# StephenNG59/ICP-symm

Hardware: AMD Instinct MI355X
Metric: icp_iterations_per_sec (higher is better)
Workload: dtype f32

## Files before the change

### icp-symm_amd/csrc/engine.cpp

```cpp
#include "engine_internal.h"
#include "robust_loss.h"
#include <limits>

void read_switches(Switches &w)
{
    auto flag = [](const char *n) { return std::getenv(n) != nullptr; };
    auto num = [](const char *n, long def) { const char *e = std::getenv(n); return e ? std::atol(e) : def; };
    auto tri = [](const char *n) { const char *e = std::getenv(n); return e ? (e[0] == '1' ? 1 : 0) : -1; };
    w.allow_any_arch = flag("SYMMICP_ALLOW_ANY_ARCH");
    w.debug_host = flag("SYMMICP_DEBUG_HOST");
    w.debug_counters = flag("SYMMICP_DEBUG_COUNTERS");
    if (const char *e = std::getenv("SYMMICP_DEBUG_TRACE")) w.debug_trace = e;
    if (const char *e = std::getenv("SYMMICP_GRID_PPC")) w.grid_ppc = std::atof(e);
    w.grid_maxlevel = (int)num("SYMMICP_GRID_MAXLEVEL", kMortonBits);
    w.grid_level = (int)num("SYMMICP_GRID_LEVEL", -1);
    if (const char *e = std::getenv("SYMMICP_FIRST_PASS")) w.first_pass = (e[0] == 'p') ? 1 : 0;
    w.oct_leaf = (int)num("SYMMICP_OCT_LEAF", 0);
    if (const char *e = std::getenv("SYMMICP_PACKET_ORDER")) w.packet_order = e[0] != '0';
    if (const char *e = std::getenv("SYMMICP_PACKET_JUMP")) w.packet_jump = (float)std::atof(e);
    w.packet_key_bits = (int)num("SYMMICP_PACKET_KEY_BITS", 16);
    w.packet_chunk = (uint32_t)num("SYMMICP_PACKET_CHUNK", 0);
    w.packet_lds_pad = (uint32_t)num("SYMMICP_PACKET_LDS_PAD", 0);
    w.packet_waves = (uint32_t)num("SYMMICP_PACKET_WAVES", 0);
    w.packet_front_cap = (uint32_t)num("SYMMICP_PACKET_FRONT_CAP", 0);
    if (const char *e = std::getenv("SYMMICP_HOOD_FRAC")) w.hood_frac = std::atof(e);
    w.no_hood = flag("SYMMICP_NO_NEIGHBOURHOOD");
    w.no_cert = flag("SYMMICP_NO_CERT");
    w.walk_full_grid = flag("SYMMICP_WALK_FULL_GRID");
    { const char *e = std::getenv("SYMMICP_HOST_LOOP"); w.host_loop = e && e[0] == '1'; }
    w.no_loop_stragglers = flag("SYMMICP_NO_LOOP_STRAGGLERS");
    w.force_comm = flag("SYMMICP_FORCE_COMM");
    if (const char *e = std::getenv("SYMMICP_PACKET_COST_KEY")) w.packet_cost_key = e[0] != '0';
    w.budget_walk = tri("SYMMICP_BUDGET_WALK");
    w.optimistic = tri("SYMMICP_OPTIMISTIC");
    w.compact = tri("SYMMICP_COMPACT");
    w.pass_blocks = (int)num("SYMMICP_PASS_BLOCKS", 2048);
    w.id_blocks = (int)num("SYMMICP_ID_BLOCKS", 2048);
    w.acc_blocks = (int)num("SYMMICP_ACC_BLOCKS", 512);
    w.fused_blocks = (int)num("SYMMICP_FUSED_BLOCKS", 512);
    w.compact_blocks = (int)num("SYMMICP_COMPACT_BLOCKS", 1280);
    w.feature_nn_splits = (int)num("SYMMICP_FEATURE_NN_SPLITS", 0);
    w.feature_nn_queries = (int)num("SYMMICP_FEATURE_NN_QUERIES", 0);
    w.tune.wave_mode_max = (uint32_t)num("SYMMICP_WAVE_MODE_MAX", 20000);
    w.tune.cells_chunk = (uint32_t)num("SYMMICP_CELLS_CHUNK", 16);
    w.tune.cells_queries = (uint32_t)num("SYMMICP_CELLS_QUERIES", 0);
    w.tune.walk_budget = (uint32_t)num("SYMMICP_WALK_BUDGET", 160);
}

void arena_begin(Arena &a, size_t want)
{
    a.off = 0;
    if (a.cap >= want) return;
    if (a.base) hipFree(a.base);
    a.base = nullptr; a.cap = 0;
    const size_t cap = want + want / 4;
    if (hipMalloc((void **)&a.base, cap) == hipSuccess) a.cap = cap;
    else (void)hipGetLastError();
}


extern "C" {

int symmicp_version(void) { return 100; }

void symmicp_config_default(symmicp_config *cfg)
{
    if (!cfg) return;
    std::memset(cfg, 0, sizeof(*cfg));
    cfg->struct_size = (int32_t)sizeof(*cfg);
    cfg->device = -1;
    cfg->mode = SYMMICP_MODE_QUIRKS;
    cfg->corr = SYMMICP_CORR_IDENTITY;
    cfg->apply = SYMMICP_APPLY_DEFAULT;
    cfg->max_iters = 10;
    cfg->diff_threshold = 1.0f;
    cfg->max_corr_dist = 0.f;
    cfg->fixed_iters = 0;
    cfg->sort_source = 1;
    cfg->verbose = 0;
    cfg->min_normal_dot = -2.0f;
    cfg->eps_rotation = 0.f;
    cfg->eps_translation = 0.f;
}

static int check_cfg(const symmicp_config *cfg)
{
    if (!cfg || cfg->struct_size != (int32_t)sizeof(symmicp_config)) return SYMMICP_ERR_ARG;
    if (!mode_known(cfg->mode)) return SYMMICP_ERR_ARG;
    if (cfg->corr < SYMMICP_CORR_IDENTITY || cfg->corr > SYMMICP_CORR_TREE) return SYMMICP_ERR_ARG;
    if (cfg->apply < SYMMICP_APPLY_DEFAULT || cfg->apply > SYMMICP_APPLY_CUMULATIVE) return SYMMICP_ERR_ARG;
    if (cfg->max_iters < 0) return SYMMICP_ERR_ARG;
    return SYMMICP_OK;
}

int symmicp_create(const symmicp_config *cfg, symmicp_ctx **out)
{
    if (!out) return SYMMICP_ERR_ARG;
    *out = nullptr;
    if (check_cfg(cfg) != SYMMICP_OK) return SYMMICP_ERR_ARG;
    int ndev = 0;
    if (hipGetDeviceCount(&ndev) != hipSuccess || ndev <= 0) return SYMMICP_ERR_HIP;
    symmicp_ctx *c = new symmicp_ctx();
    read_switches(c->sw);
    c->cfg = *cfg;
    if (cfg->device >= 0) {
        if (cfg->device >= ndev || hipSetDevice(cfg->device) != hipSuccess) { delete c; return SYMMICP_ERR_HIP; }
        c->device = cfg->device;
    } else if (hipGetDevice(&c->device) != hipSuccess) { delete c; return SYMMICP_ERR_HIP; }
    hipDeviceProp_t prop;
    if (hipGetDeviceProperties(&prop, c->device) != hipSuccess) { delete c; return SYMMICP_ERR_HIP; }
    if (std::strncmp(prop.gcnArchName, "gfx950", 6) != 0 && !c->sw.allow_any_arch) {
        delete c;
        return SYMMICP_ERR_HIP;
    }
    if (hipStreamCreateWithFlags(&c->stream, hipStreamNonBlocking) != hipSuccess) { delete c; return SYMMICP_ERR_HIP; }
    bool ok = hipMalloc((void **)&c->partials, sizeof(double) * kNSum * 8192) == hipSuccess &&
              hipMalloc((void **)&c->d_sums, sizeof(double) * kNSum) == hipSuccess &&
              hipHostMalloc((void **)&c->h_sums, sizeof(double) * (kNSum + 8), hipHostMallocMapped | hipHostMallocCoherent) == hipSuccess &&
              hipMalloc((void **)&c->ticket, 2 * sizeof(uint32_t)) == hipSuccess && hipMemset(c->ticket, 0, 2 * sizeof(uint32_t)) == hipSuccess &&
              hipHostGetDevicePointer((void **)&c->h_sums_dev, c->h_sums, 0) == hipSuccess &&
              std::memset(c->h_sums, 0, sizeof(double) * (kNSum + 8)) != nullptr &&
              hipMalloc((void **)&c->d_loop, sizeof(LoopState)) == hipSuccess &&
              hipHostMalloc((void **)&c->h_loop, sizeof(LoopState), hipHostMallocMapped | hipHostMallocCoherent) == hipSuccess &&
              hipHostGetDevicePointer((void **)&c->h_loop_dev, c->h_loop, 0) == hipSuccess &&
              hipHostMalloc((void **)&c->h_ring, sizeof(LoopRecord) * symmicp_ctx::kRing, hipHostMallocMapped | hipHostMallocCoherent) == hipSuccess &&
              hipHostGetDevicePointer((void **)&c->h_ring_dev, c->h_ring, 0) == hipSuccess &&
              hipHostMalloc((void **)&c->h_done, 64, hipHostMallocMapped | hipHostMallocCoherent) == hipSuccess &&
              hipHostGetDevicePointer((void **)&c->h_done_dev, c->h_done, 0) == hipSuccess &&
              std::memset(c->h_done, 0, 64) != nullptr &&
              true;
    for (int k = 0; ok && k < symmicp_ctx::kEvRing * symmicp_ctx::kEvPer; k++) ok = hipEventCreateWithFlags(&c->ev[k], hipEventDisableSystemFence) == hipSuccess;
    if (!ok) { symmicp_destroy(c); return SYMMICP_ERR_HIP; }
    c->pkt_fallbacks = c->ticket + 1;
    identity16(c->X);
    *out = c;
    return SYMMICP_OK;
}

extern "C++" hipError_t keep_alloc(symmicp_ctx *c, void **out, size_t bytes)
{
    bytes = (bytes + 255) & ~(size_t)255;
    if (!bytes) bytes = 256;
    if (c->keep.base && c->keep.off + bytes <= c->keep.cap) { *out = c->keep.base + c->keep.off; c->keep.off += bytes; return hipSuccess; }
    void *p = nullptr;
    const hipError_t e = hipMalloc(&p, bytes);
    if (e == hipSuccess) { c->keep_extra.push_back(p); *out = p; }
    return e;
}

extern "C++" void free_target(symmicp_ctx *c)
{
    for (void *p : c->keep_extra) hipFree(p);
    c->keep_extra.clear();
    c->keep.off = 0;
    hipFree(c->dbg); hipFree(c->dbg_trace); c->dbg_trace = nullptr;
    c->ctop = nullptr; c->dbg = nullptr; c->ix = TargetIndex{}; c->tgt_block = nullptr; c->tq = nullptr; c->tn = nullptr; c->boxes = nullptr; c->cells = nullptr; c->onodes = nullptr;
    c->have_index = false; c->n_t = 0;
    c->have_tgt_color = false;
    c->notes = IndexNotes{};
}

extern "C++" void forget_source(symmicp_ctx *c)
{
    c->worklist = c->wl_count = nullptr; c->cert = nullptr; c->certk = nullptr; c->hoodr = nullptr; c->pkt_tab = nullptr; c->pkt_count = 0; c->pkt_cost_keyed = false; c->pairrec = nullptr;
    c->src0_block = c->cur_block = nullptr; c->src_order = nullptr; c->pos = nullptr; c->d2 = nullptr; c->best64 = nullptr;
    c->n_loc = c->n_s_total = c->src_off = 0;
    c->src_no_normals = false;
    c->have_src_int = false;
    drop_reverse_index(c->rej.src_ix, false);
}

static void free_source(symmicp_ctx *c)
{
    forget_source(c);
    hipFree(c->src_all);
    c->src_all = nullptr; c->src_all_cap = 0;
}

void symmicp_destroy(symmicp_ctx *c)
{
    if (!c) return;
    if (c->sw.debug_host && c->n_pass_timed)
        std::fprintf(stderr, "[symmicp host] passes %ld: launch %.1f us, spin %.1f us, between passes %.1f us (per pass)\n", c->n_pass_timed, 1e6 * c->t_launch / c->n_pass_timed, 1e6 * c->t_spin / c->n_pass_timed, 1e6 * c->t_between / c->n_pass_timed);
    hipSetDevice(c->device);
    if (c->stream) hipStreamSynchronize(c->stream);
    if (c->comm && g_rccl.CommDestroy) g_rccl.CommDestroy(c->comm);
    shm_close(c);
    free_target(c);
// ... 1494 lines not shown
```

### icp-symm_amd/csrc/engine_internal.h

```cpp
#pragma once
#include <hip/hip_runtime.h>
#include <dlfcn.h>
#include <fcntl.h>
#include <sys/mman.h>
#include <sys/stat.h>
#include <unistd.h>
#include <algorithm>
#include <chrono>
#include <cmath>
#include <cstdio>
#include <cstdlib>
#include <cstring>
#include <mutex>
#include <string>
#include <vector>

#include "symmicp.h"
#include "symmicp_internal.h"
#include "host_solve.h"


namespace symmicp {}
using namespace symmicp;

typedef struct { char internal[128]; } rcclUniqueId;
typedef void *rcclComm_t;
typedef int (*fn_ncclGetUniqueId)(rcclUniqueId *);
typedef int (*fn_ncclCommInitRank)(rcclComm_t *, int, rcclUniqueId, int);
typedef int (*fn_ncclCommDestroy)(rcclComm_t);
typedef int (*fn_ncclAllReduce)(const void *, void *, size_t, int, int, rcclComm_t, hipStream_t);
typedef const char *(*fn_ncclGetErrorString)(int);
constexpr int kNcclFloat64 = 8;
constexpr int kNcclSum = 0;

struct Rccl {
    void *handle = nullptr;
    fn_ncclGetUniqueId GetUniqueId = nullptr;
    fn_ncclCommInitRank CommInitRank = nullptr;
    fn_ncclCommDestroy CommDestroy = nullptr;
    fn_ncclAllReduce AllReduce = nullptr;
    fn_ncclGetErrorString GetErrorString = nullptr;
    std::string err;
    std::mutex mu;
    bool load()
    {
        std::lock_guard<std::mutex> lock(mu);
        if (handle && AllReduce) return true;
        const char *names[] = {"librccl.so.1", "librccl.so"};
        for (const char *nm : names) { handle = dlopen(nm, RTLD_NOW | RTLD_NOLOAD | RTLD_GLOBAL); if (handle) break; }
        if (!handle)
            for (const char *nm : names) { handle = dlopen(nm, RTLD_NOW | RTLD_GLOBAL); if (handle) break; }
        if (!handle) { err = std::string("cannot load librccl: ") + dlerror(); return false; }
        GetUniqueId = (fn_ncclGetUniqueId)dlsym(handle, "ncclGetUniqueId");
        CommInitRank = (fn_ncclCommInitRank)dlsym(handle, "ncclCommInitRank");
        CommDestroy = (fn_ncclCommDestroy)dlsym(handle, "ncclCommDestroy");
        AllReduce = (fn_ncclAllReduce)dlsym(handle, "ncclAllReduce");
        GetErrorString = (fn_ncclGetErrorString)dlsym(handle, "ncclGetErrorString");
        if (!GetUniqueId || !CommInitRank || !CommDestroy || !AllReduce) { err = "librccl misses nccl* symbols"; return false; }
        return true;
    }
};
extern Rccl g_rccl;

inline double now_s()
{
    return std::chrono::duration<double>(std::chrono::steady_clock::now().time_since_epoch()).count();
}

struct Switches {
    bool allow_any_arch = false, debug_host = false, debug_counters = false;
    std::string debug_trace;
    double grid_ppc = 3.0;
    int grid_maxlevel = kMortonBits, grid_level = -1;
    int first_pass = -1;
    int oct_leaf = 0;
    bool packet_order = true;
    bool packet_cost_key = true;
    float packet_jump = -1.0f;
    int packet_key_bits = 16;
    uint32_t packet_chunk = 0, packet_lds_pad = 0, packet_waves = 0, packet_front_cap = 0;
    double hood_frac = 0.8;
    bool no_hood = false, no_cert = false, walk_full_grid = false, host_loop = false, no_loop_stragglers = false, force_comm = false;
    int budget_walk = -1, optimistic = -1, compact = -1;
    int pass_blocks = 2048, id_blocks = 2048, acc_blocks = 512, fused_blocks = 512, compact_blocks = 1280;
    int feature_nn_splits = 0, feature_nn_queries = 0;
    PassTuning tune;
};

void read_switches(Switches &w);

struct Arena {
    char *base = nullptr;
    size_t cap = 0, off = 0;
};

struct ShmSlot {
    volatile unsigned long long seq;
    double s[SYMMICP_NSUM];
    char pad[512 - 8 - 8 * SYMMICP_NSUM];
};
static_assert(sizeof(ShmSlot) == 512, "slot = 4 cache lines");
struct ShmExchange {
    ShmSlot *slots = nullptr;
    size_t bytes = 0;
    unsigned long long count = 0;
    std::string name;
    bool owner = false;
};

struct IndexNotes {
    float origin[3] = {0, 0, 0}, h0 = 0.f;
    uint32_t hist[16] = {};
    uint32_t leaf_max = 0;
    uint32_t nblocks = 0, ctop_len = 0;
};

struct ReverseIndex {
    Arena keep;
    std::vector<void *> extra;
    TargetIndex ix{};
    bool valid = false;
};

struct Rejectors {
    float trim_frac = 1.0f, med_factor = 0.0f;
    bool one_to_one = false, reciprocal = false;
    uint32_t *keys = nullptr, *ws = nullptr;
    unsigned long long *table = nullptr;
    size_t keys_cap = 0, table_cap = 0;
    ReverseIndex src_ix;
    uint64_t src_ix_builds = 0;
    RecipArgs recip_args{};
    enum : uint32_t { kTrim = 1, kMedian = 2, kOneToOne = 4, kReciprocal = 8 };
    uint32_t ran = 0;
    RejectRecord last{};
    void invalidate() { ran = 0; }

    bool trims() const { return trim_frac < 1.0f; }
    bool median() const { return med_factor > 0.0f; }
    bool claims(int corr) const { return (one_to_one || reciprocal) && corr != SYMMICP_CORR_IDENTITY; }
    bool checks_back(int corr) const { return reciprocal && corr != SYMMICP_CORR_IDENTITY; }
    bool rejects(int corr) const { return trims() || median() || claims(corr); }
    uint32_t settings_mask(int corr) const
    {
        if (!rejects(corr)) return 0u;
        return (trims() ? kTrim : 0u) | (median() ? kMedian : 0u) | (one_to_one ? kOneToOne : 0u) | (checks_back(corr) ? kReciprocal : 0u);
    }
    bool keys_valid() const { return ran != 0u; }
    bool trim_state_valid() const { return (ran & kTrim) != 0u; }
    bool rejection_state_valid() const { return (ran & (kMedian | kOneToOne | kReciprocal)) != 0u; }
    bool reciprocal_state_valid() const { return (ran & kReciprocal) != 0u; }
    static size_t table_words(size_t n_t, bool with_recip_tail) { return (n_t ? n_t : 1) + (with_recip_tail ? kRecipTailWords : 0); }
};

struct symmicp_ctx {
    Switches sw;
    Arena arena;
    Arena keep;
    std::vector<void *> keep_extra;
    ShmExchange shm;
    symmicp_config cfg{};
    int loss = SYMMICP_LOSS_NONE;
    float loss_scale = 0.f;
    float gicp_eps = 1e-3f;
    float color_lam = 0.968f;
    float4 *tgt_color = nullptr;
    float *src_int = nullptr;
    size_t tgt_color_cap = 0, src_int_cap = 0;
    bool have_tgt_color = false, have_src_int = false;
    Rejectors rej;
    int device = 0;
    hipStream_t stream = nullptr;
    std::string err;
    int nranks = 1, rank = 0;
    rcclComm_t comm = nullptr;
    bool external_exchange = false;
    bool sums_exchanged = false;
    uint32_t n_t = 0;
    float *tgt_block = nullptr;
    CloudSoA tgt{};
    float4 *tq = nullptr, *tn = nullptr;
    float4 *boxes = nullptr;
    float4 *onodes = nullptr;
    uint2 *cells = nullptr;
    uint32_t *ctop = nullptr;
    unsigned long long *dbg = nullptr;
    unsigned long long *dbg_trace = nullptr;
    TargetIndex ix{};
    bool have_index = false;
    bool target_surface_like = false;
    IndexNotes notes;
    float pivot[3] = {0, 0, 0};
    uint32_t n_s_total = 0, n_loc = 0, src_off = 0;
    bool src_no_normals = false;
    char *src_all = nullptr;
    size_t src_all_cap = 0;
    float *src0_block = nullptr, *cur_block = nullptr;
    CloudSoA src0{}, cur{};
    uint32_t *src_order = nullptr;
    int32_t *pos = nullptr;
    float *d2 = nullptr;
    float4 *pairrec = nullptr;
    float *cert = nullptr;
    uint32_t *certk = nullptr;
    float *hoodr = nullptr;
    uint32_t *pkt_tab = nullptr;
    uint32_t pkt_count = 0;
    bool pkt_cost_keyed = false;
    uint32_t *pkt_fallbacks = nullptr;
    unsigned long long *best64 = nullptr;
    uint32_t *worklist = nullptr, *wl_count = nullptr;
    WorkLists wl{};
    int pass_blocks = 0;
    double *partials = nullptr, *d_sums = nullptr, *h_sums = nullptr, *h_sums_dev = nullptr;
    uint32_t *ticket = nullptr;
    long long last_list_len = -1;
    long long last_uncertified = -1;
    static constexpr int kRing = 65;
    LoopState *d_loop = nullptr, *h_loop = nullptr, *h_loop_dev = nullptr;
    LoopRecord *h_ring = nullptr, *h_ring_dev = nullptr;
    unsigned long long *h_done = nullptr, *h_done_dev = nullptr;
    unsigned long long batch_seq = 0;
    bool loop_log_on = false;
    std::vector<symmicp_loop_log_entry> loop_log;
    int loop_log_batches = 0;
    int host_passes_since_bailout = 1000;
    unsigned long long seq = 0;
    bool begun = false;
    int iters = 0;
    float X[16];
    symmicp_sums last{};
    int timing = 0;
    static constexpr int kEvRing = 64, kEvPer = 8;
    hipEvent_t ev[kEvRing * kEvPer] = {};
    int ev_split[kEvRing] = {};
    int ev_weight[kEvRing] = {};
    int ev_coll[kEvRing] = {};
    int ev_used = 0;
    symmicp_stats st{};
    double t_launch = 0, t_spin = 0, t_between = 0, t_last_done = 0;
    long n_pass_timed = 0;
};

template <typename T>
struct DevBuf {
    T *p = nullptr;
    bool owned = true;
    DevBuf() = default;
    DevBuf(const DevBuf &) = delete;
    DevBuf &operator=(const DevBuf &) = delete;
    ~DevBuf() { if (p && owned) hipFree(p); }
    hipError_t alloc(size_t count) { owned = true; return hipMalloc((void **)&p, sizeof(T) * (count ? count : 1)); }
    hipError_t alloc_temp(Arena &a, size_t count)
    {
        const size_t bytes = ((sizeof(T) * (count ? count : 1)) + 255) & ~(size_t)255;
        if (a.base && a.off + bytes <= a.cap) { p = reinterpret_cast<T *>(a.base + a.off); a.off += bytes; owned = false; return hipSuccess; }
        return alloc(count);
    }
    T *release() { T *q = p; p = nullptr; return q; }
};

template <typename T>
inline hipError_t grow(T *&p, size_t &cap, size_t want)
{
    if (cap >= want) return hipSuccess;
    hipFree(p);
    p = nullptr; cap = 0;
    const hipError_t e = hipMalloc((void **)&p, sizeof(T) * want);
    if (e == hipSuccess) cap = want;
    return e;
}

hipError_t keep_alloc(symmicp_ctx *c, void **out, size_t bytes);
void arena_begin(Arena &a, size_t want);

#define HIP_TRY(ctx, call)                                                                                  \
    do {                                                                                                    \
        hipError_t e__ = (call);                                                                            \
        if (e__ != hipSuccess) {                                                                            \
            (ctx)->err = std::string(#call) + ": " + hipGetErrorString(e__);                                \
            return SYMMICP_ERR_HIP;                                                                         \
        }                                                                                                   \
    } while (0)



inline int fail(symmicp_ctx *c, int code, const std::string &msg)
{
    if (c) c->err = msg;
    return code;
}

inline void soa_from_block(float *block, size_t n, CloudSoA &s)
{
    s.x = block; s.y = block + n; s.z = block + 2 * n; s.nx = block + 3 * n; s.ny = block + 4 * n; s.nz = block + 5 * n;
}

inline void identity16(float X[16])
{
    for (int k = 0; k < 16; k++) X[k] = (k % 5 == 0) ? 1.f : 0.f;
}

inline bool pass_claims(const symmicp_ctx *c) { return c->rej.claims(c->cfg.corr); }
inline bool pass_reciprocal(const symmicp_ctx *c) { return c->rej.checks_back(c->cfg.corr); }
inline bool pass_rejects(const symmicp_ctx *c) { return c->rej.rejects(c->cfg.corr); }

inline int resolved_apply(const symmicp_config &c)
{
    if (c.apply == SYMMICP_APPLY_INCREMENTAL || c.apply == SYMMICP_APPLY_CUMULATIVE) return c.apply;
    return c.mode == SYMMICP_MODE_QUIRKS ? SYMMICP_APPLY_INCREMENTAL : SYMMICP_APPLY_CUMULATIVE;
}


void free_target(symmicp_ctx *c);
void forget_source(symmicp_ctx *c);
void flush_events(symmicp_ctx *c);
int build_reverse_index(symmicp_ctx *c, const CloudSoA &cl, uint32_t n, const uint32_t *labels, ReverseIndex &ri);
void drop_reverse_index(ReverseIndex &ri, bool release);
void shm_close(symmicp_ctx *c);
int shm_exchange(symmicp_ctx *c, double *rec);
void dump_packet_trace(symmicp_ctx *c);
void print_pass_counters(symmicp_ctx *c, bool first, long long list_len);
```

### icp-symm_amd/csrc/engine_loop.cpp

```cpp
#include "engine_internal.h"

extern "C" {

static int prepare_rejectors(symmicp_ctx *c, RejectArgs &r)
{
    Rejectors &j = c->rej;
    r = RejectArgs{};
    if (!pass_rejects(c)) return SYMMICP_OK;
    HIP_TRY(c, grow(j.keys, j.keys_cap, c->n_loc ? c->n_loc : 1));
    if (!j.ws) HIP_TRY(c, hipMalloc((void **)&j.ws, sizeof(uint32_t) * kRejectWsWords));
    r.keys = j.keys; r.ws = j.ws;
    r.host = reinterpret_cast<RejectRecord *>(c->h_sums_dev + kNSum + 1);
    r.rho = j.trim_frac; r.med_f2 = j.median() ? j.med_factor * j.med_factor : 0.0f;
    if (!pass_claims(c)) return SYMMICP_OK;
    HIP_TRY(c, grow(j.table, j.table_cap, Rejectors::table_words(c->n_t, pass_reciprocal(c))));
    r.table = j.table; r.n_t = c->n_t; r.order = c->src_order;
    r.claim = kClaimOneToOne;
    if (!pass_reciprocal(c)) return SYMMICP_OK;
    if (!j.src_ix.valid) {
        const double t0 = now_s();
        if (int st = build_reverse_index(c, c->src0, c->n_loc, c->src_order, j.src_ix)) return st;
        j.src_ix_builds++;
        if (c->sw.debug_host) {
            std::fprintf(stderr, "[symmicp host] source index: %u points, %zu bytes in its arena (+%zu allocations beside it), built in %.3f ms\n", c->n_loc,
// ... 19 lines not shown
        __builtin_ia32_pause();
        if ((++spins & 0xFFFu) == 0) {
            if (hipStreamQuery(c->stream) != hipErrorNotReady) { got = (*flag == seq); break; }
            if (now_s() - t0 > limit_seconds) break;
        }
    }
    __atomic_thread_fence(__ATOMIC_ACQUIRE);
    if (spun) *spun += now_s() - t0;
    if (!got) {
        HIP_TRY(c, hipStreamSynchronize(c->stream));
        HIP_TRY(c, hipGetLastError());
        if (*flag != seq) return fail(c, SYMMICP_ERR_HIP, what);
    }
    return SYMMICP_OK;
}

static void fill_pass_args(symmicp_ctx *c, PassArgs &a, const RejectArgs &rej, const float Xapply[16], bool from_cur, bool writeback, bool first)
{
    a.in = from_cur ? c->cur : c->src0;
    a.out = c->cur;
    a.n = c->n_loc;
    a.tgt_offset = c->src_off;
    for (int k = 0; k < 12; k++) a.X.m[k] = Xapply[k];
    a.X.nrm_w = (c->cfg.mode == SYMMICP_MODE_QUIRKS) ? 1.0f : 0.0f;
    const bool paper = c->cfg.mode != SYMMICP_MODE_QUIRKS;
    for (int k = 0; k < 3; k++) a.pivot[k] = paper ? c->pivot[k] : 0.0f;
    a.p2p = c->cfg.mode == SYMMICP_MODE_P2P ? 1 : 0;
    a.obj = mode_obj(c->cfg.mode);
    a.gicp_k = 1.0f - c->gicp_eps;
    a.tgt_color = c->tgt_color;
    a.src_int = c->src_int;
    a.color_lam = c->color_lam;
    a.color_om = 1.0f - c->color_lam;
    a.max_d2 = c->cfg.max_corr_dist > 0.f ? c->cfg.max_corr_dist * c->cfg.max_corr_dist : 0.f;
    a.min_ndot = c->cfg.min_normal_dot;
    a.writeback = writeback ? 1 : 0;
    a.best64 = c->best64;
    a.pos_prev = first ? nullptr : c->pos;
    a.pos_out = c->pos;
    a.d2_out = (c->cfg.corr == SYMMICP_CORR_IDENTITY) ? nullptr : c->d2;
    a.partials = c->partials;
    a.cert = reinterpret_cast<float4 *>(c->cert);
    a.certk = c->sw.no_hood ? nullptr : reinterpret_cast<uint4 *>(c->certk);
    a.hoodr = reinterpret_cast<float2 *>(c->hoodr);
    a.make_hood = (a.certk && !first && c->last_uncertified >= 0 && (double)c->last_uncertified < c->sw.hood_frac * (double)c->n_s_total) ? 1 : 0;
    a.pairrec = c->pairrec;
    a.budget_walk = c->sw.budget_walk >= 0 ? c->sw.budget_walk : (first && c->nranks > 1 && c->n_loc < 400000u);
    a.use_slack = (!first && c->cert && !c->sw.no_cert) ? 1 : 0;
    a.loop = nullptr;
    a.pkt_tab = reinterpret_cast<const uint2 *>(c->pkt_tab);
    a.pkt_count = c->pkt_count;
    a.pkt_waves = c->sw.packet_waves;
    a.pkt_front_cap = c->sw.packet_front_cap;
    a.pkt_fallbacks = c->pkt_fallbacks;
    a.pkt_chunk = c->sw.packet_chunk;
    a.pkt_lds_pad = c->sw.packet_lds_pad;
    a.loss = c->loss;
    a.loss_scale = c->loss_scale;
    a.rej = rej;
}

static int run_pass(symmicp_ctx *c, const float Xapply[16], bool from_cur, bool writeback, bool first)
{
    PassArgs a{};
    RejectArgs rej;
    if (int st = prepare_rejectors(c, rej)) return st;
    c->rej.invalidate();
    fill_pass_args(c, a, rej, Xapply, from_cur, writeback, first);
    const bool rejecting = pass_rejects(a);
    int blocks = (int)((c->n_loc + kPassThreads - 1) / kPassThreads);
    int cap = c->sw.pass_blocks;
    if (cap > 8192) cap = 8192;
    if (blocks > cap) blocks = cap;
    if (blocks < 1) blocks = 1;
    c->pass_blocks = blocks;
    const double t_l0 = now_s();
    if (c->t_last_done > 0) c->t_between += t_l0 - c->t_last_done;
    hipEvent_t *ev = nullptr;
    uint32_t walk_blocks = 0;
    bool optimistic = false;
    if (c->timing) {
        if (c->ev_used == symmicp_ctx::kEvRing) flush_events(c);
        ev = c->ev + c->ev_used * symmicp_ctx::kEvPer;
        c->ev_split[c->ev_used] = (c->timing == 1 || c->timing == 3) ? 1 : 0;
        c->ev_weight[c->ev_used] = 1;
    }
    if (ev && !(c->timing == 2 && c->cfg.corr == SYMMICP_CORR_TREE)) hipEventRecord(ev[0], c->stream);
    switch (c->cfg.corr) {
    case SYMMICP_CORR_IDENTITY: {
        const bool vec4 = (c->n_loc % 4 == 0) && (c->n_t % 4 == 0) && (c->src_off % 4 == 0);
        if (vec4) {
            const int id_cap = c->sw.id_blocks;
            const int nb4 = (int)((c->n_loc / 4 + kPassThreads - 1) / kPassThreads);
            blocks = nb4 < id_cap ? (nb4 > 0 ? nb4 : 1) : id_cap;
            c->pass_blocks = blocks;
        }
        launch_pass_identity(a, c->tgt, blocks, vec4, c->stream);
        break;
    }
    case SYMMICP_CORR_BRUTE:
        launch_nn_brute(a.in, c->n_loc, a.X, c->tq, c->n_t, c->best64, c->stream);
        launch_pass_indexed(a, c->tn, blocks, c->stream);
        break;
    default:
        {
            const int acc_cap = c->sw.acc_blocks;
            const int nb_all = (int)((c->n_loc + kPassThreads - 1) / kPassThreads);
            int ab = nb_all < acc_cap ? ((nb_all + 7) / 8) * 8 : acc_cap;
            if (ab < 8) ab = 8;
            c->pass_blocks = blocks = ab;
            if (!first && c->last_list_len >= 0 && c->last_list_len <= 50000) {
                walk_blocks = (uint32_t)(2 * c->last_list_len);
                if (walk_blocks < 256u) walk_blocks = 256u;
                if (walk_blocks > 8192u) walk_blocks = 8192u;
            }
            if (!first && c->last_list_len == -2) walk_blocks = 16384u;
            if (c->sw.walk_full_grid) walk_blocks = 0;
            optimistic = c->sw.optimistic >= 0 ? c->sw.optimistic == 1 : (!first && c->last_list_len == 0);
            if (writeback) optimistic = false;
            if (rejecting) optimistic = false;
            if (first && c->target_surface_like) launch_pass_tree_first(a, c->ix, c->wl, ab, c->stream, c->timing == 2 ? ev : nullptr);
            else
            {
                const int cp_blocks = c->sw.compact_blocks;
                const bool compact = a.use_slack && (c->sw.compact >= 0 ? c->sw.compact == 1 : (c->last_uncertified >= 0 && c->last_uncertified < (long long)(c->n_s_total / 10)));
                launch_pass_tree_split(a, c->ix, c->wl, ab, walk_blocks, optimistic ? 1 : 0, compact ? cp_blocks : 0, c->sw.tune, c->stream, c->timing == 2 ? ev : nullptr);
            }
            if (ev && c->timing == 2) c->ev_split[c->ev_used] = 2;
        }
        break;
    }
    if (ev && c->ev_split[c->ev_used] != 2) hipEventRecord(ev[4], c->stream);
    c->t_launch += now_s() - t_l0;
    auto reduce_and_wait = [&](int keep_nonempty) -> int {
        const unsigned long long seq = ++c->seq;
        volatile unsigned long long *flag = reinterpret_cast<volatile unsigned long long *>(c->h_sums + kNSum);
        launch_final_reduce(c->partials, blocks, c->d_sums, c->comm ? nullptr : c->h_sums_dev, c->ticket, seq,
                            c->cfg.corr == SYMMICP_CORR_TREE ? c->wl_count : nullptr, keep_nonempty, c->stream);
        if (c->comm) {
            if (ev) { hipEventRecord(ev[6], c->stream); c->ev_coll[c->ev_used] = 1; }
            int r = g_rccl.AllReduce(c->d_sums, c->d_sums, kNSum, kNcclFloat64, kNcclSum, c->comm, c->stream);
            if (r != 0) return fail(c, SYMMICP_ERR_COMM, std::string("ncclAllReduce: ") + (g_rccl.GetErrorString ? g_rccl.GetErrorString(r) : "?"));
            if (ev) hipEventRecord(ev[7], c->stream);
            launch_publish(c->d_sums, c->h_sums_dev, seq, c->stream);
        }
        if (ev && c->ev_split[c->ev_used] != 1) hipEventRecord(ev[5], c->stream);
        return wait_for_word(c, flag, seq, 30.0, "pass finished without publishing its record", &c->t_spin);
    };
    if (int st = reduce_and_wait(optimistic ? 1 : 0)) return st;
    if (c->shm.slots) { if (int st = shm_exchange(c, c->h_sums)) return st; }
    if (c->cfg.corr == SYMMICP_CORR_TREE && c->h_sums[kNSum - 1] >= kListDropped)
        return fail(c, SYMMICP_ERR_HIP, "a work-list shard overflowed: appends were dropped (internal capacity error)");
    long long list_len = (c->cfg.corr == SYMMICP_CORR_TREE) ? (long long)c->h_sums[kNSum - 1] : -1;
    c->last_uncertified = (c->cfg.corr == SYMMICP_CORR_TREE && !first) ? (long long)c->h_sums[kNSum - 2] : -1;
    if (optimistic && list_len > 0) {
        c->st.kernel_launches[7]++;
        launch_pass_tree_split(a, c->ix, c->wl, blocks, list_len <= 50000 ? 8192u : 0u, 2, 0, c->sw.tune, c->stream, nullptr);
        if (ev && c->ev_split[c->ev_used] != 2) hipEventRecord(ev[4], c->stream);
        if (int st = reduce_and_wait(0)) return st;
        if (c->shm.slots) { if (int st = shm_exchange(c, c->h_sums)) return st; }
    }
    if (rejecting) {
        std::memcpy(&c->rej.last, c->h_sums + kNSum + 1, sizeof(RejectRecord));
        c->rej.ran = c->rej.settings_mask(c->cfg.corr);
    }
    if (ev) c->ev_used++;
    c->t_last_done = now_s(); c->n_pass_timed++;
    if (c->dbg_trace && first) dump_packet_trace(c);
    if (c->ix.dbg) print_pass_counters(c, first, list_len);
    std::memcpy(c->last.s, c->h_sums, sizeof(double) * kNSum);
    if (c->cfg.corr == SYMMICP_CORR_TREE) c->last.s[kNSum - 1] = c->last.s[kNSum - 2] = 0.0;
    c->last_list_len = list_len;
    if (first && c->cfg.corr == SYMMICP_CORR_TREE && c->target_surface_like) c->last_list_len = -2;
    c->st.passes++;
    return SYMMICP_OK;
}

static constexpr uint32_t kLoopListLimit = 8192;
static uint32_t loop_scan_limit(uint32_t n) { const uint32_t f = n / 256; return f < 8192u ? f : 8192u; }
static bool batch_eligible(const symmicp_ctx *c)
{
    if (c->sw.host_loop) return false;
    if (pass_rejects(c)) return false;
    if (c->cfg.mode == SYMMICP_MODE_COLOR) return false;
    if (c->cfg.host_loop) return false;
    if (c->external_exchange || c->shm.slots) return false;
    if (c->timing == 2 || c->ix.dbg) return false;
    if (!mode_device_solves(c->cfg.mode)) return false;
    if (c->n_loc == 0 && !c->comm) return false;
    if (c->host_passes_since_bailout < 2) return false;
    const bool incr = resolved_apply(c->cfg) == SYMMICP_APPLY_INCREMENTAL;
    if (c->cfg.corr == SYMMICP_CORR_IDENTITY) return true;
    if (c->cfg.corr == SYMMICP_CORR_TREE)
        return !incr && c->last_list_len >= 0 && c->last_list_len <= (c->sw.no_loop_stragglers ? 0ll : (long long)kLoopListLimit) && c->last_uncertified >= 0 &&
               c->last_uncertified <= (long long)(loop_scan_limit(c->n_s_total) / (c->last_list_len > 0 ? 2 : 1)) && c->cert && !c->sw.no_cert;
    return false;
}

static constexpr int kListBlocks = 8;
static constexpr int kEvSampleStride = 4;
static int run_batch(symmicp_ctx *c, int want, float *diffs_before, int *n_done, bool *small_step)
{
    *n_done = 0;
    *small_step = false;
    if (want > symmicp_ctx::kRing - 1) want = symmicp_ctx::kRing - 1;
    if (want <= 0) return SYMMICP_OK;
    const bool incr = resolved_apply(c->cfg) == SYMMICP_APPLY_INCREMENTAL;
    const bool tree = c->cfg.corr == SYMMICP_CORR_TREE;
    LoopConfig lc{};
    lc.mode = c->cfg.mode; lc.fixed_iters = c->cfg.fixed_iters; lc.max_iters = c->iters + want; lc.incremental = incr ? 1 : 0; lc.tree = tree ? 1 : 0;
    lc.diff_threshold = c->cfg.diff_threshold; lc.eps_rotation = c->cfg.eps_rotation; lc.eps_translation = c->cfg.eps_translation;
    lc.nrm_w = (c->cfg.mode == SYMMICP_MODE_QUIRKS) ? 1.0f : 0.0f;
    for (int k = 0; k < 3; k++) lc.pivot[k] = c->pivot[k];
    lc.uncertified_limit = 4 * loop_scan_limit(c->n_s_total);
    const bool no_stage = c->sw.no_loop_stragglers;
    bool stragglers = tree && c->last_list_len > 0 && !no_stage;
    lc.list_limit = kLoopListLimit;
    if (lc.max_iters > c->cfg.max_iters) lc.max_iters = c->cfg.max_iters;
    const int it0 = c->iters;
    LoopState ls{};
    std::memcpy(ls.X, c->X, sizeof(ls.X));
    for (int k = 0; k < 12; k++) ls.Xapply.m[k] = c->X[k];
    ls.Xapply.nrm_w = lc.nrm_w;
    ls.iters = it0;
    *c->h_loop = ls;
    symmicp_sums last0{};
    if (c->loop_log_on) {
        last0 = c->last;
        c->h_ring[it0 % symmicp_ctx::kRing].solved = 0;
    }
    HIP_TRY(c, hipMemcpyAsync(c->d_loop, c->h_loop, sizeof(LoopState), hipMemcpyHostToDevice, c->stream));
    PassArgs a{};
    fill_pass_args(c, a, RejectArgs{}, c->X, incr, incr, false);
    a.loop = c->d_loop;
    int blocks;
    bool vec4 = false;
    if (tree) {
        const int fb = c->sw.fused_blocks;
        const int tiles = (int)((c->n_loc + kPassThreads - 1) / kPassThreads);
        blocks = tiles < fb ? tiles : fb;
        if (blocks < 1) blocks = 1;
    } else {
        vec4 = (c->n_loc % 4 == 0) && (c->n_t % 4 == 0) && (c->src_off % 4 == 0);
        const int id_cap = c->sw.id_blocks;
        const int nb = (int)(((vec4 ? c->n_loc / 4 : c->n_loc) + kPassThreads - 1) / kPassThreads);
        blocks = nb < id_cap ? (nb > 0 ? nb : 1) : id_cap;
    }
    const int fused_blocks_full = blocks;
    c->pass_blocks = blocks;
    uint32_t *counters = tree ? c->wl_count : nullptr;
    const bool timed_run = c->timing == 1 || c->timing == 3;
    const int ev_stride = c->timing == 3 ? kEvSampleStride : 1;
    if (timed_run && c->ev_used + want > symmicp_ctx::kEvRing) flush_events(c);
    const bool unstoppable = lc.fixed_iters && !(lc.eps_rotation > 0.f && lc.eps_translation > 0.f) && !stragglers;
    int enq = 0, chunk = unstoppable ? want : 4, n_stage = 0;
    bool first_chunk = true;
    while (enq < want) {
        const int nq = (want - enq < chunk) ? want - enq : chunk;
        const int it_before = first_chunk ? it0 : c->h_loop->iters;
        const int ev_used0 = c->ev_used;
        const int fused_blocks = (stragglers && fused_blocks_full + kListBlocks > 512) ? 512 - kListBlocks : fused_blocks_full;
        blocks = fused_blocks + (stragglers ? kListBlocks : 0);
        a.partial_cols = stragglers ? (uint32_t)blocks : 0u;
        a.partial_col0 = (uint32_t)fused_blocks;
        lc.walk_in_loop = stragglers ? 1 : 0;
        if (first_chunk) launch_reduce_solve(c->partials, blocks, c->d_sums, 2, c->d_loop, lc, c->h_ring_dev, symmicp_ctx::kRing, counters, c->stream);
        for (int p = 0; p < nq; p++) {
            hipEvent_t *ev = nullptr;
            if (timed_run && (enq + p) % ev_stride == 0 && c->ev_used < symmicp_ctx::kEvRing) {
                ev = c->ev + c->ev_used * symmicp_ctx::kEvPer;
                c->ev_split[c->ev_used] = 1;
                c->ev_weight[c->ev_used] = 1;
                hipEventRecord(ev[0], c->stream);
            }
            if (tree) {
                launch_pass_fused(a, c->ix, c->wl, fused_blocks, c->stream);
                if (stragglers) launch_loop_stragglers(a, c->ix, c->wl, kListBlocks, c->sw.tune, c->stream);
            }
            else launch_pass_identity(a, c->tgt, blocks, vec4, c->stream);
            if (ev) { hipEventRecord(ev[4], c->stream); c->ev_used++; }
            if (c->comm || blocks > 512) {
                launch_final_reduce(c->partials, blocks, c->d_sums, nullptr, c->ticket, 0ull, counters, 0, c->stream);
                if (c->comm) {
                    if (ev) { hipEventRecord(ev[6], c->stream); c->ev_coll[c->ev_used - 1] = 1; }
                    int r = g_rccl.AllReduce(c->d_sums, c->d_sums, kNSum, kNcclFloat64, kNcclSum, c->comm, c->stream);
                    if (r != 0) {
                        (void)hipStreamSynchronize(c->stream);
                        c->begun = false;
                        c->ev_used = 0;
                        return fail(c, SYMMICP_ERR_COMM, std::string("ncclAllReduce: ") + (g_rccl.GetErrorString ? g_rccl.GetErrorString(r) : "?"));
                    }
                    if (ev) hipEventRecord(ev[7], c->stream);
                }
                launch_reduce_solve(c->partials, blocks, c->d_sums, 1, c->d_loop, lc, c->h_ring_dev, symmicp_ctx::kRing, counters, c->stream);
            } else {
                launch_reduce_solve(c->partials, blocks, c->d_sums, 0, c->d_loop, lc, c->h_ring_dev, symmicp_ctx::kRing, counters, c->stream);
            }
        }
        const unsigned long long seq = ++c->batch_seq;
        launch_loop_end(c->d_loop, c->h_loop_dev, c->h_done_dev, seq, c->stream);
        if (int st = wait_for_word(c, c->h_done, seq, 60.0, "batch finished without publishing its end flag")) return st;
        enq += nq;
        first_chunk = false;
        const int ran = (c->h_loop->iters - it_before) + (c->h_loop->reason == LOOP_REDO_PASS ? 1 : 0);
        if (timed_run && ran >= 0) {
            int sampled_ran = 0;
            for (int p = 0; p < ran && p < nq; p++) {
                if ((enq - nq + p) % ev_stride != 0) continue;
                if (ev_used0 + sampled_ran < symmicp_ctx::kEvRing) {
                    const int left = (ran < nq ? ran : nq) - p;
                    c->ev_weight[ev_used0 + sampled_ran] = left < ev_stride ? left : ev_stride;
                }
                sampled_ran++;
            }
            if (ev_used0 + sampled_ran < c->ev_used) c->ev_used = ev_used0 + sampled_ran;
        }
        if (stragglers) n_stage += c->h_loop->iters - it_before;
        if (c->h_loop->stop) break;
        if (tree && !no_stage) {
            stragglers = false;
            for (int k = it_before + 1; k <= c->h_loop->iters; k++) stragglers = stragglers || c->h_ring[k % symmicp_ctx::kRing].list_len > 0;
        }
        if (stragglers) chunk = 4;
        else if (lc.fixed_iters && !(lc.eps_rotation > 0.f && lc.eps_translation > 0.f)) chunk = want;
        else chunk *= 2;
    }
    const LoopState &hl = *c->h_loop;
    const int it1 = hl.iters;
    if (it1 < it0 || it1 > it0 + want) return fail(c, SYMMICP_ERR_HIP, "device loop state out of range");
    for (int k = it0; k < it1; k++) diffs_before[k - it0] = (k == it0) ? (float)c->last.s[33] : (float)c->h_ring[k % symmicp_ctx::kRing].sums[33];
    if (it1 > it0) {
        std::memcpy(c->last.s, c->h_ring[it1 % symmicp_ctx::kRing].sums, sizeof(double) * kNSum);
        std::memcpy(c->X, c->h_ring[(it1 - 1) % symmicp_ctx::kRing].X, sizeof(float) * 16);
        c->st.passes += it1 - it0;
        c->st.loop_passes += it1 - it0;
        c->st.loop_straggler_passes += n_stage;
    }
    if (c->loop_log_on) {
        for (int k = it0; k <= it1; k++) {
            const LoopRecord &r = c->h_ring[k % symmicp_ctx::kRing];
            symmicp_loop_log_entry e{};
            std::memcpy(e.sums, k == it0 ? last0.s : r.sums, sizeof(e.sums));
            std::memcpy(e.increment, r.increment, sizeof(e.increment));
            std::memcpy(e.X, r.X, sizeof(e.X));
            e.rcond = r.rcond; e.iter = k; e.status = r.status; e.solved = r.solved; e.list_len = k == it0 ? 0 : r.list_len;
            e.reason = hl.reason; e.batch = c->loop_log_batches;
            if (!e.solved) { std::memset(e.increment, 0, sizeof(e.increment)); std::memset(e.X, 0, sizeof(e.X)); e.rcond = 0.f; e.status = -1; }
            c->loop_log.push_back(e);
        }
        c->loop_log_batches++;
    }
    c->iters = it1;
    c->last_list_len = tree ? (it1 > it0 ? (long long)c->h_ring[it1 % symmicp_ctx::kRing].list_len : c->last_list_len) : -1;
    *n_done = it1 - it0;
    *small_step = hl.reason == LOOP_DONE && hl.small_step != 0;
    if (tree && it1 > it0) c->last_uncertified = c->h_ring[it1 % symmicp_ctx::kRing].pad;
    if (c->sw.debug_host && it1 - it0 >= 2) {
        const double *q = c->h_ring[(it1 - 1) % symmicp_ctx::kRing].sums;
        if (q[37] != 0.0) std::fprintf(stderr, "[symmicp host] k_reduce_solve stamps of pass %d: load + reduce %.2f us (loop state there after %.2f us), bookkeeping + solve %.2f us, publish %.2f us\n", it1 - 1, std::floor(q[37]) * 0.01, (q[37] - std::floor(q[37])) * 1e4 * 0.01, q[38] * 0.01, q[39] * 0.01);
    }
    if (c->sw.debug_host && tree) {
        std::fprintf(stderr, "[symmicp host] batch: work list / searched pairs after each device pass:");
        for (int k = it0 + 1; k <= it1; k++) std::fprintf(stderr, " %d/%d", c->h_ring[k % symmicp_ctx::kRing].list_len, c->h_ring[k % symmicp_ctx::kRing].pad);
        std::fprintf(stderr, "\n");
    }
    if (c->sw.debug_host) std::fprintf(stderr, "[symmicp host] batch: %d of %d passes on the device (%d enqueued), reason %d, %d with the straggler stage, list after %lld\n", it1 - it0, want, enq, hl.reason, n_stage, (long long)c->last_list_len);
    if (hl.reason == LOOP_SLOW) c->host_passes_since_bailout = 1;
    if (hl.reason == LOOP_REDO_PASS || hl.reason == LOOP_HOST_SOLVE) {
        c->host_passes_since_bailout = 0;
        c->last_list_len = -1;
        c->st.kernel_launches[7]++;
    }
    return SYMMICP_OK;
}

static int check_ready(symmicp_ctx *c)
{
    if (!c->tgt_block || !c->src0_block) return fail(c, SYMMICP_ERR_STATE, "source and target must be set first (myicp.cpp:102)");
    if (c->cfg.corr == SYMMICP_CORR_IDENTITY && c->n_s_total != c->n_t)
        return fail(c, SYMMICP_ERR_SIZE, "identity pairing needs N_s == N_t (func.cpp:21)");
    if (c->cfg.corr == SYMMICP_CORR_TREE && !c->have_index) return fail(c, SYMMICP_ERR_STATE, "target index missing");
    if (c->cfg.corr != SYMMICP_CORR_IDENTITY && !c->tq) return fail(c, SYMMICP_ERR_STATE, "target was set under a different corr mode");
    if (c->cfg.mode == SYMMICP_MODE_COLOR) {
        if (c->nranks > 1) return fail(c, SYMMICP_ERR_STATE, "SYMMICP_MODE_COLOR runs on single-rank contexts only");
        if (!c->have_src_int || !c->have_tgt_color)
            return fail(c, SYMMICP_ERR_STATE, "SYMMICP_MODE_COLOR needs symmicp_set_source_intensity and symmicp_set_target_intensity after the clouds");
    }
    return SYMMICP_OK;
}

static void fill_iter(symmicp_ctx *c, symmicp_iter_result *out, int status, float rcond, const float *incr)
{
    if (!out) return;
    out->status = status;
    out->iter = c->iters;
    out->diff = (float)c->last.s[33];
    out->rcond = rcond;
    out->pairs = c->last.s[c->loss != SYMMICP_LOSS_NONE ? 37 : 34];
    if (incr) std::memcpy(out->increment, incr, sizeof(float) * 16); else identity16(out->increment);
    out->sums = c->last;
}

int symmicp_begin(symmicp_ctx *c, const float *guess16, symmicp_iter_result *out)
{
    if (!c) return SYMMICP_ERR_ARG;
    HIP_TRY(c, hipSetDevice(c->device));
    int st = check_ready(c);
    if (st != SYMMICP_OK) return st;
    if (guess16) std::memcpy(c->X, guess16, sizeof(float) * 16); else identity16(c->X);
    c->iters = 0;
    const bool incr = resolved_apply(c->cfg) == SYMMICP_APPLY_INCREMENTAL;
    st = run_pass(c, c->X, false, incr, true);
    if (st != SYMMICP_OK) return st;
    c->begun = true;
    c->sums_exchanged = false;
    fill_iter(c, out, SYMMICP_OK, 1.0f, nullptr);
    return SYMMICP_OK;
}

int symmicp_step(symmicp_ctx *c, symmicp_iter_result *out)
{
    if (!c) return SYMMICP_ERR_ARG;
    if (!c->begun) return fail(c, SYMMICP_ERR_STATE, "symmicp_step before symmicp_begin");
    if (c->external_exchange && !c->sums_exchanged)
        return fail(c, SYMMICP_ERR_STATE, "external exchange: symmicp_set_sums(total over ranks) must follow every pass");
    c->sums_exchanged = false;
    HIP_TRY(c, hipSetDevice(c->device));
    float pbar[3], qbar[3], a[3], t[3], rc = 0.f, Xi[16];
    int st = (c->cfg.mode == SYMMICP_MODE_P2P) ? solve_p2p(c->last, c->pivot, &rc, Xi) : solve_mode(mode_solves_as(c->cfg.mode), c->last, c->pivot, pbar, qbar, a, t, &rc, Xi);
    if (st != SYMMICP_OK) {
        c->err = "degenerate system (rank-deficient normal equations or non-finite transform; func.cpp:70,96)";
        fill_iter(c, out, st, rc, nullptr);
        return st;
    }
    mat4_mul(Xi, c->X, c->X);
    const bool incr = resolved_apply(c->cfg) == SYMMICP_APPLY_INCREMENTAL;
    st = incr ? run_pass(c, Xi, true, true, false) : run_pass(c, c->X, false, false, false);
    if (st != SYMMICP_OK) return st;
    c->iters++;
    fill_iter(c, out, SYMMICP_OK, rc, Xi);
    return SYMMICP_OK;
}

static size_t append_eigen(std::string &out, const float *m, int rows, int cols, int stride)
{
    char cell[16][32];
    size_t width = 0;
    for (int r = 0; r < rows; r++)
        for (int c = 0; c < cols; c++) {
            std::snprintf(cell[r * cols + c], sizeof(cell[0]), "%g", (double)m[r * stride + c]);
            width = std::max(width, std::strlen(cell[r * cols + c]));
        }
    for (int r = 0; r < rows; r++) {
        for (int c = 0; c < cols; c++) {
            if (c) out += ' ';
            const size_t len = std::strlen(cell[r * cols + c]);
            out.append(width - len, ' ');
            out += cell[r * cols + c];
        }
        out += '\n';
    }
    return width;
}

static void polar_rotation(const float X[16], float R[9])
{
    double A[3][3];
    for (int r = 0; r < 3; r++) for (int c = 0; c < 3; c++) A[r][c] = X[4 * r + c];
    for (int it = 0; it < 100; it++) {
        const double det = A[0][0] * (A[1][1] * A[2][2] - A[1][2] * A[2][1]) - A[0][1] * (A[1][0] * A[2][2] - A[1][2] * A[2][0]) + A[0][2] * (A[1][0] * A[2][1] - A[1][1] * A[2][0]);
        if (!(std::fabs(det) > 1e-300) || !std::isfinite(det)) break;
        double inv_t[3][3];
        inv_t[0][0] = (A[1][1] * A[2][2] - A[1][2] * A[2][1]) / det; inv_t[0][1] = (A[1][2] * A[2][0] - A[1][0] * A[2][2]) / det; inv_t[0][2] = (A[1][0] * A[2][1] - A[1][1] * A[2][0]) / det;
        inv_t[1][0] = (A[0][2] * A[2][1] - A[0][1] * A[2][2]) / det; inv_t[1][1] = (A[0][0] * A[2][2] - A[0][2] * A[2][0]) / det; inv_t[1][2] = (A[0][1] * A[2][0] - A[0][0] * A[2][1]) / det;
        inv_t[2][0] = (A[0][1] * A[1][2] - A[0][2] * A[1][1]) / det; inv_t[2][1] = (A[0][2] * A[1][0] - A[0][0] * A[1][2]) / det; inv_t[2][2] = (A[0][0] * A[1][1] - A[0][1] * A[1][0]) / det;
        double change = 0.0;
        for (int r = 0; r < 3; r++)
            for (int c = 0; c < 3; c++) { const double v = 0.5 * (A[r][c] + inv_t[r][c]); change = std::max(change, std::fabs(v - A[r][c])); A[r][c] = v; }
        if (change < 1e-15) break;
    }
    for (int r = 0; r < 3; r++) for (int c = 0; c < 3; c++) R[3 * r + c] = std::isfinite(A[r][c]) ? (float)A[r][c] : X[4 * r + c];
}

size_t symmicp_format_result(const float transform16[16], char *buf, size_t cap)
{
    if (!transform16) return 0;
    std::string out = "Result transform:\n";
    append_eigen(out, transform16, 4, 4, 4);
    out += "  rotation:\n";
    float R[9];
    polar_rotation(transform16, R);
    append_eigen(out, R, 3, 3, 3);
    out += "  translation:\n";
    append_eigen(out, transform16 + 3, 3, 1, 4);
    if (buf && cap) {
        const size_t n = std::min(out.size(), cap - 1);
        std::memcpy(buf, out.data(), n);
        buf[n] = 0;
    }
    return out.size();
}

int symmicp_align(symmicp_ctx *c, const float *guess16, symmicp_result *out)
{
    if (!c || !out) return SYMMICP_ERR_ARG;
    std::memset(out, 0, sizeof(*out));
    if (c->external_exchange) { out->status = SYMMICP_ERR_STATE; return fail(c, SYMMICP_ERR_STATE, "symmicp_align is not available with external exchange: drive begin/set_sums/step"); }
    const double t0 = now_s();
    c->loop_log.clear();
    c->loop_log_batches = 0;
    symmicp_iter_result it;
    int st = symmicp_begin(c, guess16, &it);
    if (st != SYMMICP_OK) { out->status = st; return st; }
    float diff = it.diff;
    out->diff_initial = diff;
    int iters = 0;
    while ((c->cfg.fixed_iters || diff > c->cfg.diff_threshold) && iters < c->cfg.max_iters) {
        if (batch_eligible(c)) {
            float db[symmicp_ctx::kRing];
            int done = 0;
            bool small = false;
            st = run_batch(c, c->cfg.max_iters - iters, db, &done, &small);
            if (st != SYMMICP_OK) break;
            for (int k = 0; k < done; k++) {
                iters++;
                if (c->cfg.verbose) std::printf("iters#%d\ndiff: %g\n", iters, db[k]);
                if (iters <= 64) out->diffs[iters - 1] = db[k];
            }
            diff = (float)c->last.s[33];
            if (small) break;
            if (done > 0 || c->host_passes_since_bailout == 0) continue;
        }
        iters++;
        if (c->cfg.verbose) std::printf("iters#%d\ndiff: %g\n", iters, diff);
        if (iters <= 64) out->diffs[iters - 1] = diff;
        st = symmicp_step(c, &it);
        if (st != SYMMICP_OK) { iters--; break; }
        c->host_passes_since_bailout++;
        diff = it.diff;
        if (c->cfg.eps_rotation > 0.f && c->cfg.eps_translation > 0.f && !c->cfg.fixed_iters) {
            const float *Xi = it.increment;
            const double tr = ((double)Xi[0] + Xi[5] + Xi[10] - 1.0) * 0.5;
            const double ang = std::acos(tr > 1.0 ? 1.0 : (tr < -1.0 ? -1.0 : tr));
            const double tn = std::sqrt((double)Xi[3] * Xi[3] + (double)Xi[7] * Xi[7] + (double)Xi[11] * Xi[11]);
            if (ang < c->cfg.eps_rotation && tn < c->cfg.eps_translation) break;
        }
    }
    out->status = st;
    out->iters = iters;
    out->diff_final = diff;
    std::memcpy(out->transform, c->X, sizeof(float) * 16);
    out->seconds_total = now_s() - t0;
    if (c->cfg.verbose) {
        char buf[1024];
        symmicp_format_result(c->X, buf, sizeof(buf));
        std::fputs(buf, stdout);
    }
    return st;
}

int symmicp_solve(int mode, const symmicp_sums *sums, const float pivot[3], float pbar[3], float qbar[3], float a[3],
                  float t[3], float *rcond, float out16[16])
{
    if (!sums || !pbar || !qbar || !a || !t || !out16) return SYMMICP_ERR_ARG;
    if (mode == SYMMICP_MODE_P2P) {
        for (int k = 0; k < 3; k++) pbar[k] = qbar[k] = a[k] = t[k] = 0.f;
        return solve_p2p(*sums, pivot, rcond, out16);
    }
    mode = mode_solves_as(mode);
    return mode_device_solves(mode) ? solve_mode(mode, *sums, pivot, pbar, qbar, a, t, rcond, out16) : SYMMICP_ERR_ARG;
}

int symmicp_ctx_solve_probe(symmicp_ctx *c, int mode, int exact_rc, const symmicp_sums *sums, size_t n, const float pivot[3], const float *X_in16,
                            int32_t *status, float *pbar, float *qbar, float *a, float *t, float *rcond, float *out16, float *X_out16)
{
    if (!c) return SYMMICP_ERR_ARG;
    if (!mode_device_solves(mode)) return fail(c, SYMMICP_ERR_ARG, "probe: QUIRKS, PAPER, PLANE or GICP");
    if (!sums || n == 0 || n > (1u << 24) || !status || !pbar || !qbar || !a || !t || !rcond || !out16 || (X_in16 && !X_out16))
        return fail(c, SYMMICP_ERR_ARG, "probe: bad arguments");
    HIP_TRY(c, hipSetDevice(c->device));
    const size_t b_sums = sizeof(symmicp_sums) * n, b_f3 = sizeof(float) * 3 * n, b_16 = sizeof(float) * 16 * n;
    const size_t o_piv = b_sums, o_xin = o_piv + 16, o_st = o_xin + b_16, o_pb = o_st + 4 * n, o_qb = o_pb + b_f3, o_a = o_qb + b_f3, o_t = o_a + b_f3,
                 o_rc = o_t + b_f3, o_out = o_rc + 4 * n, o_xo = o_out + b_16, total = o_xo + b_16;
    char *d = nullptr;
    HIP_TRY(c, hipMalloc((void **)&d, total));
    float piv[4] = {0.f, 0.f, 0.f, 0.f};
    if (pivot) for (int k = 0; k < 3; k++) piv[k] = pivot[k];
    int st = SYMMICP_OK;
    if (hipMemcpy(d, sums, b_sums, hipMemcpyHostToDevice) != hipSuccess || hipMemcpy(d + o_piv, piv, 16, hipMemcpyHostToDevice) != hipSuccess ||
        (X_in16 && hipMemcpy(d + o_xin, X_in16, b_16, hipMemcpyHostToDevice) != hipSuccess))
        st = fail(c, SYMMICP_ERR_HIP, "probe: upload");
    if (st == SYMMICP_OK) {
        launch_solve_probe(mode, exact_rc, (const symmicp_sums *)d, (int)n, (const float *)(d + o_piv), X_in16 ? (const float *)(d + o_xin) : nullptr,
                           (int32_t *)(d + o_st), (float *)(d + o_pb), (float *)(d + o_qb), (float *)(d + o_a), (float *)(d + o_t), (float *)(d + o_rc),
                           (float *)(d + o_out), (float *)(d + o_xo), c->stream);
        if (hipGetLastError() != hipSuccess || hipStreamSynchronize(c->stream) != hipSuccess) st = fail(c, SYMMICP_ERR_HIP, "probe: kernel");
    }
    if (st == SYMMICP_OK) {
        const struct { size_t off, bytes; void *dst; } back[] = {{o_st, 4 * n, status}, {o_pb, b_f3, pbar}, {o_qb, b_f3, qbar}, {o_a, b_f3, a}, {o_t, b_f3, t},
                                                              {o_rc, 4 * n, rcond}, {o_out, b_16, out16}, {o_xo, X_in16 ? b_16 : 0, X_out16}};
        for (const auto &b : back)
            if (b.bytes && hipMemcpy(b.dst, d + b.off, b.bytes, hipMemcpyDeviceToHost) != hipSuccess) { st = fail(c, SYMMICP_ERR_HIP, "probe: read back"); break; }
    }
    (void)hipFree(d);
    return st;
}

int symmicp_ctx_loop_solve(symmicp_ctx *c, const symmicp_sums *sums, const float pivot[3], const float X_in16[16], const int32_t in_i[6], const float in_f[3],
                           int32_t state_out[4], float X_out16[16], float Xapply_out12[12], float ring_inc16[16], float ring_X16[16], float *ring_rcond,
                           int32_t ring_i2[2])
{
    if (!c) return SYMMICP_ERR_ARG;
    if (!sums || !X_in16 || !in_i || !in_f || !state_out || !X_out16 || !Xapply_out12 || !ring_inc16 || !ring_X16 || !ring_rcond || !ring_i2)
        return fail(c, SYMMICP_ERR_ARG, "loop_solve: bad arguments");
    const int mode = in_i[0];
    if (!mode_device_solves(mode)) return fail(c, SYMMICP_ERR_ARG, "loop_solve: QUIRKS, PAPER, PLANE or GICP");
    HIP_TRY(c, hipSetDevice(c->device));
    LoopConfig lc{};
    lc.mode = mode; lc.fixed_iters = in_i[1]; lc.max_iters = in_i[2]; lc.incremental = in_i[5] ? 1 : 0; lc.tree = 0;
    lc.diff_threshold = in_f[0]; lc.eps_rotation = in_f[1]; lc.eps_translation = in_f[2];
    lc.nrm_w = (mode == SYMMICP_MODE_QUIRKS) ? 1.0f : 0.0f;
    for (int k = 0; k < 3; k++) lc.pivot[k] = pivot ? pivot[k] : 0.f;
    LoopState ls{};
    std::memcpy(ls.X, X_in16, sizeof(ls.X));
    for (int k = 0; k < 12; k++) ls.Xapply.m[k] = X_in16[k];
    ls.Xapply.nrm_w = lc.nrm_w;
    ls.iters = in_i[3];
    ls.small_step = in_i[4];
    char *d = nullptr;
    const size_t o_loop = 512, o_ring = o_loop + ((sizeof(LoopState) + 255) & ~(size_t)255), total = o_ring + sizeof(LoopRecord);
    HIP_TRY(c, hipMalloc((void **)&d, total));
    int st = SYMMICP_OK;
    if (hipMemcpy(d, sums, sizeof(symmicp_sums), hipMemcpyHostToDevice) != hipSuccess || hipMemcpy(d + o_loop, &ls, sizeof(ls), hipMemcpyHostToDevice) != hipSuccess ||
        hipMemset(d + o_ring, 0xFF, sizeof(LoopRecord)) != hipSuccess)
        st = fail(c, SYMMICP_ERR_HIP, "loop_solve: upload");
    if (st == SYMMICP_OK) {
        launch_reduce_solve(nullptr, 0, (double *)d, 2, (LoopState *)(d + o_loop), lc, (LoopRecord *)(d + o_ring), 1, nullptr, c->stream);
        if (hipGetLastError() != hipSuccess || hipStreamSynchronize(c->stream) != hipSuccess) st = fail(c, SYMMICP_ERR_HIP, "loop_solve: kernel");
    }
    LoopState lo{};
    LoopRecord r{};
    if (st == SYMMICP_OK && (hipMemcpy(&lo, d + o_loop, sizeof(lo), hipMemcpyDeviceToHost) != hipSuccess ||
                             hipMemcpy(&r, d + o_ring, sizeof(r), hipMemcpyDeviceToHost) != hipSuccess))
        st = fail(c, SYMMICP_ERR_HIP, "loop_solve: read back");
    (void)hipFree(d);
    if (st != SYMMICP_OK) return st;
    state_out[0] = lo.stop; state_out[1] = lo.reason; state_out[2] = lo.iters; state_out[3] = lo.small_step;
    std::memcpy(X_out16, lo.X, sizeof(lo.X));
    std::memcpy(Xapply_out12, lo.Xapply.m, sizeof(lo.Xapply.m));
    std::memcpy(ring_inc16, r.increment, sizeof(r.increment));
    std::memcpy(ring_X16, r.X, sizeof(r.X));
    std::memcpy(ring_rcond, &r.rcond, sizeof(float));
    ring_i2[0] = r.status; ring_i2[1] = r.solved;
    return SYMMICP_OK;
}

int symmicp_set_loop_log(symmicp_ctx *c, int on)
{
    if (!c) return SYMMICP_ERR_ARG;
    c->loop_log_on = on != 0;
    if (!c->loop_log_on) { c->loop_log.clear(); c->loop_log.shrink_to_fit(); }
// ... 13 lines not shown
```

### icp-symm_amd/csrc/kernels_pass.hip

```cpp
#include <cstdlib>
#include <type_traits>
#include "symmicp_internal.h"
#include "device_common.h"
#include "oct_walk.h"
#include "solve_core.h"
#include "robust_loss.h"
#include "pass_rows.h"
#pragma clang fp contract(off)

namespace symmicp {

template <int NA>
__device__ __forceinline__ void acc_block_reduce_store(AccN<NA> &a, double *partials, uint32_t col)
{
    __shared__ double red[(kPassThreads / 64) * kNSum];
    acc_wave_reduce(a, red + (threadIdx.x >> 6) * kNSum);
    __syncthreads();
    if (threadIdx.x < kNSum) {
        double s = 0.0;
        if (threadIdx.x < NA) {
#pragma unroll
            for (int w = 0; w < kPassThreads / 64; w++) s += red[w * kNSum + threadIdx.x];
        }
        partials[(size_t)col * kNSum + threadIdx.x] = s;
// ... 3 lines not shown
template <int VEC, bool W, int OBJ, bool T>
__global__ __launch_bounds__(kPassThreads) void k_pass_identity(PassArgs a_in, CloudSoA tgt)
{
    if (a_in.loop && a_in.loop->stop) return;
    PassArgs a = a_in;
    if (a_in.loop) a.X = a_in.loop->Xapply;
    AccT<W> acc; acc_zero(acc);
    const HotParams h = hot_params(a);
    const uint32_t tau = T ? a.rej.ws[kRejectTauWord] : 0u;
    const bool need_n = reads_src_normals<OBJ>(a.writeback, a.min_ndot);
    const uint32_t stride = gridDim.x * blockDim.x * VEC;
    for (uint32_t i0 = (blockIdx.x * blockDim.x + threadIdx.x) * VEC; i0 < a.n; i0 += stride) {
        float x[VEC], y[VEC], z[VEC], nx[VEC], ny[VEC], nz[VEC], qx[VEC], qy[VEC], qz[VEC], qnx[VEC], qny[VEC], qnz[VEC];
        const uint32_t j0 = a.tgt_offset + i0;
        if (VEC == 4) {
            *reinterpret_cast<float4 *>(x) = *reinterpret_cast<const float4 *>(a.in.x + i0);
            *reinterpret_cast<float4 *>(y) = *reinterpret_cast<const float4 *>(a.in.y + i0);
            *reinterpret_cast<float4 *>(z) = *reinterpret_cast<const float4 *>(a.in.z + i0);
            if (need_n) {
                *reinterpret_cast<float4 *>(nx) = *reinterpret_cast<const float4 *>(a.in.nx + i0);
                *reinterpret_cast<float4 *>(ny) = *reinterpret_cast<const float4 *>(a.in.ny + i0);
                *reinterpret_cast<float4 *>(nz) = *reinterpret_cast<const float4 *>(a.in.nz + i0);
            } else {
#pragma unroll
                for (int k = 0; k < VEC; k++) nx[k] = ny[k] = nz[k] = 0.0f;
            }
            *reinterpret_cast<float4 *>(qx) = *reinterpret_cast<const float4 *>(tgt.x + j0);
            *reinterpret_cast<float4 *>(qy) = *reinterpret_cast<const float4 *>(tgt.y + j0);
            *reinterpret_cast<float4 *>(qz) = *reinterpret_cast<const float4 *>(tgt.z + j0);
            *reinterpret_cast<float4 *>(qnx) = *reinterpret_cast<const float4 *>(tgt.nx + j0);
            *reinterpret_cast<float4 *>(qny) = *reinterpret_cast<const float4 *>(tgt.ny + j0);
            *reinterpret_cast<float4 *>(qnz) = *reinterpret_cast<const float4 *>(tgt.nz + j0);
        } else {
            x[0] = a.in.x[i0]; y[0] = a.in.y[i0]; z[0] = a.in.z[i0];
            if (need_n) { nx[0] = a.in.nx[i0]; ny[0] = a.in.ny[i0]; nz[0] = a.in.nz[i0]; }
            else nx[0] = ny[0] = nz[0] = 0.0f;
            qx[0] = tgt.x[j0]; qy[0] = tgt.y[j0]; qz[0] = tgt.z[j0];
            qnx[0] = tgt.nx[j0]; qny[0] = tgt.ny[j0]; qnz[0] = tgt.nz[j0];
        }
        float px[VEC], py[VEC], pz[VEC], npx[VEC], npy[VEC], npz[VEC], d2[VEC];
#pragma unroll
        for (int k = 0; k < VEC; k++) {
            px[k] = xf_row(a.X.m + 0, x[k], y[k], z[k], 1.0f); py[k] = xf_row(a.X.m + 4, x[k], y[k], z[k], 1.0f);
            pz[k] = xf_row(a.X.m + 8, x[k], y[k], z[k], 1.0f);
            npx[k] = xf_row(a.X.m + 0, nx[k], ny[k], nz[k], a.X.nrm_w); npy[k] = xf_row(a.X.m + 4, nx[k], ny[k], nz[k], a.X.nrm_w);
            npz[k] = xf_row(a.X.m + 8, nx[k], ny[k], nz[k], a.X.nrm_w);
            d2[k] = dist2(px[k], py[k], pz[k], qx[k], qy[k], qz[k]);
        }
        if (a.writeback) {
            if (VEC == 4) {
                *reinterpret_cast<float4 *>(a.out.x + i0) = *reinterpret_cast<float4 *>(px);
                *reinterpret_cast<float4 *>(a.out.y + i0) = *reinterpret_cast<float4 *>(py);
                *reinterpret_cast<float4 *>(a.out.z + i0) = *reinterpret_cast<float4 *>(pz);
                *reinterpret_cast<float4 *>(a.out.nx + i0) = *reinterpret_cast<float4 *>(npx);
                *reinterpret_cast<float4 *>(a.out.ny + i0) = *reinterpret_cast<float4 *>(npy);
                *reinterpret_cast<float4 *>(a.out.nz + i0) = *reinterpret_cast<float4 *>(npz);
            } else {
                a.out.x[i0] = px[0]; a.out.y[i0] = py[0]; a.out.z[i0] = pz[0];
                a.out.nx[i0] = npx[0]; a.out.ny[i0] = npy[0]; a.out.nz[i0] = npz[0];
            }
        }
        if (a.d2_out) {
            if (VEC == 4) *reinterpret_cast<float4 *>(a.d2_out + i0) = *reinterpret_cast<float4 *>(d2);
            else a.d2_out[i0] = d2[0];
        }
#pragma unroll
        for (int k = 0; k < VEC; k++) {
            if constexpr (OBJ == kObjColor) {
                const ColorPair cp = color_pair(a, i0 + k, j0 + k);
                pair_step<OBJ, T>(acc, h, nx[k], ny[k], nz[k], px[k], py[k], pz[k], make_float4(qx[k], qy[k], qz[k], 0.0f), make_float4(qnx[k], qny[k], qnz[k], 0.0f), d2[k], tau, &cp);
            } else
            pair_step<OBJ, T>(acc, h, nx[k], ny[k], nz[k], px[k], py[k], pz[k], make_float4(qx[k], qy[k], qz[k], 0.0f), make_float4(qnx[k], qny[k], qnz[k], 0.0f), d2[k], tau);
        }
    }
    acc_block_reduce_store(acc, a.partials, blockIdx.x);
}

template <bool W, int OBJ, bool T>
__global__ __launch_bounds__(kPassThreads) void k_pass_indexed(PassArgs a, const float4 *__restrict__ tn)
{
    AccT<W> acc; acc_zero(acc);
    const HotParams h = hot_params(a);
    const uint32_t tau = T ? a.rej.ws[kRejectTauWord] : 0u;
    const bool need_n = reads_src_normals<OBJ>(a.writeback, a.min_ndot);
    const uint32_t stride = gridDim.x * blockDim.x;
    for (uint32_t i = blockIdx.x * blockDim.x + threadIdx.x; i < a.n; i += stride) {
        float x = a.in.x[i], y = a.in.y[i], z = a.in.z[i];
        float nx = 0.0f, ny = 0.0f, nz = 0.0f;
        if (need_n) { nx = a.in.nx[i]; ny = a.in.ny[i]; nz = a.in.nz[i]; }
        float px = xf_row(a.X.m + 0, x, y, z, 1.0f), py = xf_row(a.X.m + 4, x, y, z, 1.0f), pz = xf_row(a.X.m + 8, x, y, z, 1.0f);
        if (a.writeback) {
            a.out.x[i] = px; a.out.y[i] = py; a.out.z[i] = pz;
            a.out.nx[i] = xf_row(a.X.m + 0, nx, ny, nz, a.X.nrm_w); a.out.ny[i] = xf_row(a.X.m + 4, nx, ny, nz, a.X.nrm_w);
            a.out.nz[i] = xf_row(a.X.m + 8, nx, ny, nz, a.X.nrm_w);
        }
        unsigned long long b = a.best64[i];
        uint32_t j = (uint32_t)(b & 0xFFFFFFFFull);
        float d2 = __uint_as_float((uint32_t)(b >> 32));
        bool ok = (b != ~0ull);
        if (a.pos_out) a.pos_out[i] = ok ? (int32_t)j : -1;
        if (a.d2_out) a.d2_out[i] = ok ? d2 : __int_as_float(0x7f800000);
        if (!ok) continue;
        if (a.max_d2 > 0.0f && d2 > a.max_d2) continue;
        if (T && a.rej.claim != kClaimNone && a.rej.keys[i] == 0xFFFFFFFFu) continue;
        if constexpr (OBJ == kObjColor) {
            const ColorPair cp = color_pair(a, i, j);
            pair_step<OBJ, T>(acc, h, nx, ny, nz, px, py, pz, tn[2 * (size_t)j], tn[2 * (size_t)j + 1], d2, tau, &cp);
        } else
        pair_step<OBJ, T>(acc, h, nx, ny, nz, px, py, pz, tn[2 * (size_t)j], tn[2 * (size_t)j + 1], d2, tau);
    }
    acc_block_reduce_store(acc, a.partials, blockIdx.x);
}

__device__ __forceinline__ uint2 cell_range(const TargetIndex &ix, uint32_t morton)
{
    const uint32_t blk = ix.ctop[morton >> 9];
    if (blk == 0xFFFFFFFFu) return make_uint2(0u, 0u);
    return ix.cells[(size_t)blk * 512u + (morton & 511u)];
}

__device__ __forceinline__ uint32_t spread3(uint32_t v)
{
    v &= 0x3ffu;
    v = (v | (v << 16)) & 0x030000ffu;
    v = (v | (v << 8)) & 0x0300f00fu;
    v = (v | (v << 4)) & 0x030c30c3u;
    v = (v | (v << 2)) & 0x09249249u;
    return v;
}

constexpr int kWaveFrontier = 512;

__device__ __forceinline__ float axis_gap2(float p, float origin, int c, float h, float margin)
{
    const float lo = origin + (float)c * h;
    const float g = fmaxf(fmaxf(lo - p, p - (lo + h)) - margin, 0.0f);
    return g * g;
}

#ifndef SLACK_FRAC
#define SLACK_FRAC 0.0625f
#endif
constexpr float kSlackFrac = SLACK_FRAC;
constexpr int kHoodSlots = 8;
constexpr uint32_t kHoodNone = 0xFFFFFFFFu;

__device__ __forceinline__ float cert_word(float L, bool hood)
{
    const uint32_t u = __float_as_uint(L);
    if (!(L > 0.0f)) return hood ? __uint_as_float(0xBF800001u) : 0.0f;
    return __uint_as_float(hood ? ((u - 1u) | 1u) : (u & ~1u));
}

__device__ __forceinline__ bool hood_test(const PassArgs &a, const TargetIndex &ix, uint32_t i, float px, float py, float pz, float m2,
                                          int32_t pos_a, float d2a, int32_t rowa, int32_t &pos_w, float &d2w)
{
    const uint4 w0 = a.certk[2 * (size_t)i], w1 = a.certk[2 * (size_t)i + 1];
    const float T = a.hoodr[i].x;
    const uint32_t cand[kHoodSlots] = {w0.x, w0.y, w0.z, w0.w, w1.x, w1.y, w1.z, w1.w};
    float4 q[kHoodSlots];
#pragma unroll
    for (int k = 0; k < kHoodSlots; k++) q[k] = ix.tq[min(cand[k], ix.n - 1u)];
    unsigned long long kw = ((unsigned long long)__float_as_uint(d2a) << 32) | (unsigned long long)(uint32_t)rowa;
    uint32_t sec = 0x7f800000u;
    pos_w = pos_a;
#pragma unroll
    for (int k = 0; k < kHoodSlots; k++) {
        const float d2 = dist2(px, py, pz, q[k].x, q[k].y, q[k].z);
        if (cand[k] < ix.n && cand[k] != (uint32_t)pos_a && d2 == d2) {
            const unsigned long long key = ((unsigned long long)__float_as_uint(d2) << 32) | (unsigned long long)(uint32_t)__float_as_int(q[k].w);
            if (key < kw) { sec = (uint32_t)(kw >> 32); kw = key; pos_w = (int32_t)cand[k]; }
            else sec = min(sec, __float_as_uint(d2));
        }
    }
    d2w = __uint_as_float((uint32_t)(kw >> 32));
    const float dl = __builtin_amdgcn_sqrtf(m2);
    if (!((__builtin_amdgcn_sqrtf(d2w) + dl) * 1.000002f < T)) return false;
    if (pos_w != pos_a) {
        a.pos_out[i] = pos_w;
        store_pair_record(a, ix, i, pos_w);
    }
    const float d1 = sqrtf(d2w) * 1.000001f;
    const float Tn = (T - dl * 1.000001f) * 0.999999f;
    const float L = fminf(sqrtf(__uint_as_float(sec)) * 0.999999f, Tn);
    if (Tn > d1 * 1.001f) {
        a.cert[i] = make_float4(px, py, pz, cert_word((L > d1) ? L : 0.0f, true));
        a.hoodr[i].x = Tn;
    } else if (pos_w != pos_a) {
        a.cert[i].w = cert_word(0.0f, true);
    }
    return true;
}

template <bool HOOD>
__device__ __forceinline__ void cells_tile(const PassArgs &a, const TargetIndex &ix, const WorkLists &wl, const Affine &X, const uint32_t i,
                                           const uint32_t shard, const bool from_list)
{
    __shared__ float s_px[kPassThreads], s_py[kPassThreads], s_pz[kPassThreads];
    __shared__ unsigned long long s_key[kPassThreads];
    __shared__ uint32_t s_second[kPassThreads];
    __shared__ int32_t s_pos[kPassThreads];
    __shared__ uint32_t s_cell0[kPassThreads];
    __shared__ __align__(8) uint16_t s_items[kPassThreads * 27];
    __shared__ uint32_t s_wsum[kPassThreads / 64 + 1];
    __shared__ uint32_t s_anyw[kPassThreads / 64];
    __shared__ uint32_t s_nmore;
    constexpr int kHoodLds = HOOD ? kPassThreads : 1;
    __shared__ float s_reach[kHoodLds];
    __shared__ uint32_t s_hcnt[kHoodLds];
    __shared__ uint32_t s_qi[kHoodLds];

    const int tid = threadIdx.x, lane = tid & 63, wave = tid >> 6;
    const bool active = i < a.n;
    const float inf = __int_as_float(0x7f800000);
    const uint32_t push_shard = from_list ? ((i / kPassThreads) & (uint32_t)(kShards - 1)) : shard;

    float px = 0.f, py = 0.f, pz = 0.f;
    Best b;
    b.d2 = inf; b.pos = -1; b.row = 0x7fffffff;
    uint32_t mask = 0;
    uint32_t mask_rest = 0;
    bool defer = false, searched = false, probe = false, uncert = false, hood_ok = false;
    float lim = 0.f, lim_full = 0.f;
    float reach = 0.f;
    if (active) {
        const float x = a.in.x[i], y = a.in.y[i], z = a.in.z[i];
        const int32_t prev = a.pos_prev ? a.pos_prev[i] : -1;
        float clear = 0.0f, rx = 0.0f, ry = 0.0f, rz = 0.0f;
        if (a.use_slack) { const float4 ce = a.cert[i]; rx = ce.x; ry = ce.y; rz = ce.z; clear = ce.w; }
        px = xf_row(X.m + 0, x, y, z, 1.0f); py = xf_row(X.m + 4, x, y, z, 1.0f); pz = xf_row(X.m + 8, x, y, z, 1.0f);
        if (prev >= 0 && (uint32_t)prev < ix.n) {
            const float4 q = ix.tq[prev];
            const float d2 = dist2(px, py, pz, q.x, q.y, q.z);
            const int32_t row = __float_as_int(q.w);
            if (d2 <= inf) { b.d2 = d2; b.pos = prev; b.row = row; }
        }
        bool certified = false;
        if (a.use_slack && b.pos >= 0 && !from_list) {
            const float m2 = dist2(px, py, pz, rx, ry, rz);
            certified = (__builtin_amdgcn_sqrtf(b.d2) + __builtin_amdgcn_sqrtf(m2)) * 1.000002f < clear;
            if (!certified && (__float_as_uint(clear) & 1u) && a.certk) {
                int32_t pw; float d2w;
                if (hood_test(a, ix, i, px, py, pz, m2, b.pos, b.d2, b.row, pw, d2w)) {
                    certified = hood_ok = true; b.pos = pw; b.d2 = d2w;
                }
            }
        }
        if (!certified) {
            uncert = true;
            defer = true;
            if (b.pos >= 0 && ix.glevel > 0) {
                const float margin = 2e-3f * ix.h;
                const float gmax = (float)ix.gdim;
                const float rb = __builtin_amdgcn_sqrtf(b.d2) * 1.00001f;
                lim = rb + kSlackFrac * ix.h;
                const float r = lim + margin;
                const float lx = (px - r - ix.ox) * ix.inv_h, hx = (px + r - ix.ox) * ix.inv_h;
                const float ly = (py - r - ix.oy) * ix.inv_h, hy = (py + r - ix.oy) * ix.inv_h;
                const float lz = (pz - r - ix.oz) * ix.inv_h, hz = (pz + r - ix.oz) * ix.inv_h;
                const int x0 = (int)floorf(fminf(fmaxf(lx, 0.0f), gmax - 1.0f)), x1 = (int)floorf(fminf(fmaxf(hx, 0.0f), gmax - 1.0f));
                const int y0 = (int)floorf(fminf(fmaxf(ly, 0.0f), gmax - 1.0f)), y1 = (int)floorf(fminf(fmaxf(hy, 0.0f), gmax - 1.0f));
                const int z0 = (int)floorf(fminf(fmaxf(lz, 0.0f), gmax - 1.0f)), z1 = (int)floorf(fminf(fmaxf(hz, 0.0f), gmax - 1.0f));
                const int nx = x1 - x0, ny = y1 - y0, nz = z1 - z0;
                if (nx <= 2 && ny <= 2 && nz <= 2) {
                    defer = false;
                    searched = true;
                    const float thr2 = lim * lim * 1.00001f;
                    float gx[3], gy[3], gz[3];
#pragma unroll
                    for (int k = 0; k < 3; k++) {
                        gx[k] = (k <= nx) ? axis_gap2(px, ix.ox, x0 + k, ix.h, margin) : inf;
                        gy[k] = (k <= ny) ? axis_gap2(py, ix.oy, y0 + k, ix.h, margin) : inf;
                        gz[k] = (k <= nz) ? axis_gap2(pz, ix.oz, z0 + k, ix.h, margin) : inf;
                    }
#pragma unroll
                    for (int kz = 0; kz < 3; kz++)
#pragma unroll
                        for (int ky = 0; ky < 3; ky++)
#pragma unroll
                            for (int kx = 0; kx < 3; kx++) {
                                const float g2 = (gx[kx] + gy[ky]) + gz[kz];
                                if (g2 <= thr2) mask |= 1u << (kx + 3 * ky + 9 * kz);
                            }
                    s_cell0[tid] = (uint32_t)x0 | ((uint32_t)y0 << 10) | ((uint32_t)z0 << 20);
                    reach = rb;
                }
            }
            if (defer && b.pos >= 0 && ix.glevel > 0) {
                const float fx = (px - ix.ox) * ix.inv_h, fy = (py - ix.oy) * ix.inv_h, fz = (pz - ix.oz) * ix.inv_h;
                const float gmax = (float)ix.gdim;
                if (fx >= 0.0f && fy >= 0.0f && fz >= 0.0f && fx < gmax && fy < gmax && fz < gmax) {
                    const int cx = (int)fx, cy = (int)fy, cz = (int)fz;
                    const int x0 = max(cx - 1, 0), y0 = max(cy - 1, 0), z0 = max(cz - 1, 0);
                    const int x1 = min(cx + 1, ix.gdim - 1), y1 = min(cy + 1, ix.gdim - 1), z1 = min(cz + 1, ix.gdim - 1);
                    const int ax = max(cx - ((fx - (float)cx) < 0.5f ? 1 : 0), 0), bx = min(ax + 1, ix.gdim - 1);
                    const int ay = max(cy - ((fy - (float)cy) < 0.5f ? 1 : 0), 0), by = min(ay + 1, ix.gdim - 1);
                    const int az = max(cz - ((fz - (float)cz) < 0.5f ? 1 : 0), 0), bz = min(az + 1, ix.gdim - 1);
#pragma unroll
                    for (int kz = 0; kz < 3; kz++)
#pragma unroll
                        for (int ky = 0; ky < 3; ky++)
#pragma unroll
                            for (int kx = 0; kx < 3; kx++) {
                                const int X = x0 + kx, Y = y0 + ky, Z = z0 + kz;
                                const uint32_t bit = 1u << (kx + 3 * ky + 9 * kz);
                                if (X <= x1 && Y <= y1 && Z <= z1) {
                                    if (X >= ax && X <= bx && Y >= ay && Y <= by && Z >= az && Z <= bz) mask |= bit;
                                    else mask_rest |= bit;
                                }
                            }
                    s_cell0[tid] = (uint32_t)x0 | ((uint32_t)y0 << 10) | ((uint32_t)z0 << 20);
                    float face = inf, face8 = inf;
                    if (x0 > 0) face = fminf(face, px - (ix.ox + (float)x0 * ix.h));
                    if (y0 > 0) face = fminf(face, py - (ix.oy + (float)y0 * ix.h));
                    if (z0 > 0) face = fminf(face, pz - (ix.oz + (float)z0 * ix.h));
                    if (x1 < ix.gdim - 1) face = fminf(face, (ix.ox + (float)(x1 + 1) * ix.h) - px);
                    if (y1 < ix.gdim - 1) face = fminf(face, (ix.oy + (float)(y1 + 1) * ix.h) - py);
                    if (z1 < ix.gdim - 1) face = fminf(face, (ix.oz + (float)(z1 + 1) * ix.h) - pz);
                    if (ax > 0) face8 = fminf(face8, px - (ix.ox + (float)ax * ix.h));
                    if (ay > 0) face8 = fminf(face8, py - (ix.oy + (float)ay * ix.h));
                    if (az > 0) face8 = fminf(face8, pz - (ix.oz + (float)az * ix.h));
                    if (bx < ix.gdim - 1) face8 = fminf(face8, (ix.ox + (float)(bx + 1) * ix.h) - px);
                    if (by < ix.gdim - 1) face8 = fminf(face8, (ix.oy + (float)(by + 1) * ix.h) - py);
                    if (bz < ix.gdim - 1) face8 = fminf(face8, (ix.oz + (float)(bz + 1) * ix.h) - pz);
                    lim = face8 - 2e-3f * ix.h;
                    lim_full = face - 2e-3f * ix.h;
                    probe = true;
                    defer = false;
                    reach = __builtin_amdgcn_sqrtf(b.d2) * 1.00001f;
                }
            }
            if (defer) {
                a.pos_out[i] = b.pos;
                a.d2_out[i] = b.d2;
                a.cert[i].w = 0.0f;
                a.pairrec[2 * (size_t)i + 1].w = 2.0f;
                sl_push(wl.work, push_shard, i);
            }
        }
    }
    if (!from_list) {
        const unsigned long long mu = __ballot(uncert);
        if (lane == 0 && mu) atomicAdd(wl.work.counts + shard * kShardStride + 1, (uint32_t)__popcll(mu));
    }
// ... 81 lines not shown
            if (mypos >= 0) {
                const unsigned long long old = atomicMin(&s_key[q], mykey);
                uint32_t offer;
                if (mykey < old) offer = min((uint32_t)(old >> 32), my2nd);
                else if (mykey == old) offer = my2nd;
                else offer = (uint32_t)(mykey >> 32);
                atomicMin(&s_second[q], offer);
            }
        }
        __syncthreads();
        if (mypos >= 0 && s_key[q] == mykey) s_pos[q] = mypos;
    };
    for (uint32_t it0 = 0; it0 < total; it0 += kPassThreads) {
        const uint32_t it = it0 + tid;
        int q = 0;
        uint32_t j0 = 0, j1 = 0;
        if (it < total) {
            const uint32_t item = s_items[it];
            q = (int)(item >> 5);
            const int bit = (int)(item & 31u);
            const int kz = bit / 9, ky = (bit - 9 * kz) / 3, kx = bit - 9 * kz - 3 * ky;
            const uint32_t c0 = s_cell0[q];
            const uint32_t cx = (c0 & 1023u) + (uint32_t)kx, cy = ((c0 >> 10) & 1023u) + (uint32_t)ky, cz = (c0 >> 20) + (uint32_t)kz;
            const uint2 rng = cell_range(ix, (spread3(cz) << 2) | (spread3(cy) << 1) | spread3(cx));
            if (ix.dbg) atomicAdd(ix.dbg + 3, (unsigned long long)(rng.y - rng.x));
            j0 = rng.x; j1 = rng.y;
            while (j1 > j0 && j1 - j0 > kItemMax) {
                const uint32_t js = j0 + ((j1 - j0 - 1u) / kItemMax) * kItemMax;
                const uint32_t e = atomicAdd(&s_nmore, 1u);
                if (e >= more_cap) break;
                s_more[e] = make_uint2((uint32_t)q | ((j1 - js) << 8), js);
                j1 = js;
            }
        }
        scan_merge(it < total && j1 > j0, q, j0, j1);
    }
    __syncthreads();
    {
        const uint32_t nmore = min(s_nmore, more_cap);
        for (uint32_t e0 = 0; e0 < nmore; e0 += kPassThreads) {
            const uint32_t e = e0 + tid;
            int q = 0;
            uint32_t j0 = 0, j1 = 0;
            if (e < nmore) { const uint2 m = s_more[e]; q = (int)(m.x & 255u); j0 = m.y; j1 = m.y + (m.x >> 8); }
            scan_merge(e < nmore && j1 > j0, q, j0, j1);
        }
    }
    __syncthreads();

    bool more = false;
    if (round == 0 && probe) {
        const float d1 = sqrtf(__uint_as_float((uint32_t)(s_key[tid] >> 32))) * 1.00001f;
        if (!(d1 * 1.02f < lim)) { more = (mask_rest != 0); lim = lim_full; }
    }
    mask = more ? mask_rest : 0u;
    if (round == 1) break;
    {
        const unsigned long long anym = __ballot(more);
        if (lane == 0) s_anyw[wave] = (anym != 0ull);
        __syncthreads();
        uint32_t any = 0;
#pragma unroll
        for (int w = 0; w < kPassThreads / 64; w++) any |= s_anyw[w];
        if (!any) break;
    }
    }
    if (ix.dbg) {
        if (tid == 0) atomicAdd(ix.dbg + 0, (unsigned long long)total_all);
        const unsigned long long mc = __ballot(active && !defer && !searched && !probe), ms = __ballot(searched), mp = __ballot(probe), md = __ballot(defer);
        const unsigned long long mh = __ballot(hood_ok);
        if (lane == 0) {
            atomicAdd(ix.dbg + 8, (unsigned long long)__popcll(mh));
            atomicAdd(ix.dbg + 1, (unsigned long long)__popcll(mc)); atomicAdd(ix.dbg + 2, (unsigned long long)__popcll(ms));
            atomicAdd(ix.dbg + 6, (unsigned long long)__popcll(mp)); atomicAdd(ix.dbg + 7, (unsigned long long)__popcll(md));
        }
    }

    if (active && (searched || probe)) {
        const unsigned long long key = s_key[tid];
        const float d1sq = __uint_as_float((uint32_t)(key >> 32));
        const float d1 = sqrtf(d1sq) * 1.000001f;
        a.pos_out[i] = s_pos[tid];
        a.d2_out[i] = d1sq;
        if (probe && !(d1 < lim)) {
            a.cert[i].w = 0.0f;
            a.pairrec[2 * (size_t)i + 1].w = 2.0f;
            sl_push(wl.work, push_shard, i);
        } else {
            const float second = sqrtf(__uint_as_float(s_second[tid])) * 0.999999f;
            const float L = fminf(second, lim * 0.99999f);
            bool hood = false;
            const float Tq = HOOD ? fminf(s_reach[tid], lim) : 0.0f;
            if (Tq > 0.0f) {
                const uint32_t hc = s_hcnt[tid];
                const float T = Tq * 0.99999f;
                hood = T > d1 && hc >= 1u && hc <= (uint32_t)kHoodSlots;
                if (hood) {
                    uint32_t *slots = reinterpret_cast<uint32_t *>(a.certk) + (size_t)i * kHoodSlots;
#pragma unroll
                    for (int k = 1; k < kHoodSlots; k++) if ((uint32_t)k >= hc) slots[k] = kHoodNone;
                }
                const float scale = fminf(fmaxf(__powf(6.5f / ((float)hc + 0.5f), 0.4f), 0.4f), 1.5f);
                a.hoodr[i] = make_float2(hood ? T : 0.0f, Tq * scale);
                if (ix.dbg) atomicAdd(ix.dbg + (hood ? 9 : 10), 1ull);
            }
            const float Lw = cert_word((L > d1) ? L : 0.0f, hood);
            a.cert[i] = make_float4(px, py, pz, Lw);
            store_pair_record(a, ix, i, s_pos[tid]);
        }
    }
}

template <bool HOOD>
__global__ __launch_bounds__(kPassThreads) void k_search_cells(PassArgs a, TargetIndex ix, WorkLists wl, uint32_t chunk, uint32_t qshift)
{
    const uint32_t tile = xcd_remap_chunked(blockIdx.x, chunk);
    const uint32_t i = threadIdx.x < (1u << qshift) ? (tile << qshift) + threadIdx.x : 0xFFFFFFFFu;
    cells_tile<HOOD>(a, ix, wl, a.X, i, tile & (kShards - 1), false);
}

constexpr int kFusedList = 2048;

template <typename T>
__device__ __forceinline__ T in_vgpr(T v)
{
    asm volatile("" : "+v"(v));
    return v;
}
typedef float f32x4_t __attribute__((ext_vector_type(4)));
template <typename T>
__device__ __forceinline__ __attribute__((address_space(1))) T *gcol(unsigned long long base)
{
    return (__attribute__((address_space(1))) T *)base;
}
__device__ __forceinline__ float4 as_float4(f32x4_t v) { return make_float4(v.x, v.y, v.z, v.w); }

#ifndef FUSED_WAVES
#define FUSED_WAVES 2
#endif
#ifndef COMPACT_WAVES
#define COMPACT_WAVES 5
#endif
#ifndef FUSED_PPT
#define FUSED_PPT 1u
#endif
template <bool ACC, bool W, int OBJ>
__global__ __launch_bounds__(kPassThreads, ACC ? FUSED_WAVES : COMPACT_WAVES) void k_pass_fused(PassArgs a, TargetIndex ix, WorkLists wl)
{
    static_assert(ACC || !W, "the search-only form has no sums to weight");
    static_assert(ACC || OBJ == kObjSym, "the search-only form has no rows");
    const bool need_n = reads_src_normals<OBJ>(false, a.min_ndot);
    constexpr int kList = ACC ? kFusedList : kFusedList / 2;
    __shared__ uint32_t s_list[kList];
    __shared__ uint32_t s_cnt, s_total;
    __shared__ unsigned long long s_col[ACC ? 10 : 1];
    AccT<W> acc;
    if (ACC) acc_zero(acc);
    if (threadIdx.x == 0) { s_cnt = 0; s_total = 0; }
    if (ACC && threadIdx.x == 0) {
        s_col[0] = (unsigned long long)a.in.x; s_col[1] = (unsigned long long)a.in.y; s_col[2] = (unsigned long long)a.in.z;
        s_col[3] = (unsigned long long)a.in.nx; s_col[4] = (unsigned long long)a.in.ny; s_col[5] = (unsigned long long)a.in.nz;
        s_col[6] = (unsigned long long)a.pairrec; s_col[7] = (unsigned long long)a.cert;
    }
    __syncthreads();
    int stop = 0;
    HotParams h;
    if (ACC && a.loop) {
        stop = a.loop->stop;
        const float4 *xp = reinterpret_cast<const float4 *>(&in_vgpr(a.loop)->Xapply);
        const float4 r0 = xp[0], r1 = xp[1], r2 = xp[2];
        h.X.m[0] = r0.x; h.X.m[1] = r0.y; h.X.m[2] = r0.z; h.X.m[3] = r0.w;
        h.X.m[4] = r1.x; h.X.m[5] = r1.y; h.X.m[6] = r1.z; h.X.m[7] = r1.w;
        h.X.m[8] = r2.x; h.X.m[9] = r2.y; h.X.m[10] = r2.z; h.X.m[11] = r2.w;
        h.X.nrm_w = reinterpret_cast<const float *>(xp)[12];
    } else if (ACC) {
#pragma unroll
        for (int k = 0; k < 12; k++) h.X.m[k] = in_vgpr(a.X.m[k]);
        h.X.nrm_w = in_vgpr(a.X.nrm_w);
    } else {
        h.X = a.X;
        if (a.loop) { stop = a.loop->stop; h.X = a.loop->Xapply; }
    }
    const Affine &X = h.X;
#pragma unroll
    for (int k = 0; k < 3; k++) h.pivot[k] = ACC ? in_vgpr(a.pivot[k]) : a.pivot[k];
    h.max_d2 = ACC ? in_vgpr(a.max_d2) : a.max_d2; h.min_ndot = ACC ? in_vgpr(a.min_ndot) : a.min_ndot;
    h.p2p = a.p2p;
    if (W) { h.loss = a.loss; h.loss_scale = in_vgpr(a.loss_scale); }
    if (OBJ == kObjGicp) h.gicp_k = in_vgpr(a.gicp_k);
#ifdef RS_STAMPS2
    const unsigned long long fs0 = __builtin_amdgcn_s_memrealtime();
    unsigned long long fs1 = 0;
#endif
    const uint32_t shard = blockIdx.x & (kShards - 1);

    auto flush = [&]() {
        const uint32_t cnt = s_cnt;
        if (ACC && a.certk) {
            for (uint32_t base = 0; base < cnt; base += kPassThreads) {
                const uint32_t e = base + threadIdx.x;
                if (e >= cnt) continue;
                const uint32_t i = s_list[e];
                const float4 ce = a.cert[i];
                if (!(__float_as_uint(ce.w) & 1u)) continue;
                const float4 q = a.pairrec[2 * (size_t)i], nq = a.pairrec[2 * (size_t)i + 1];
                const int32_t pk = a.pos_prev[i];
                if (nq.w != 0.0f || (uint32_t)pk >= ix.n) continue;
                const float x = a.in.x[i], y = a.in.y[i], z = a.in.z[i];
                const float px = xf_row(X.m + 0, x, y, z, 1.0f), py = xf_row(X.m + 4, x, y, z, 1.0f), pz = xf_row(X.m + 8, x, y, z, 1.0f);
                const float d2 = dist2(px, py, pz, q.x, q.y, q.z);
                if (!(d2 <= __int_as_float(0x7f800000))) continue;
                int32_t pw; float d2w;
                if (hood_test(a, ix, i, px, py, pz, dist2(px, py, pz, ce.x, ce.y, ce.z), pk, d2, __float_as_int(q.w), pw, d2w)) {
                    float4 qw = q, nqw = nq;
                    if (pw != pk) { qw = ix.tn[2 * (size_t)pw]; nqw = ix.tn[2 * (size_t)pw + 1]; }
                    float nx = 0.0f, ny = 0.0f, nz = 0.0f;
                    if (need_n) { nx = a.in.nx[i]; ny = a.in.ny[i]; nz = a.in.nz[i]; }
                    pair_step<OBJ>(acc, h, nx, ny, nz, px, py, pz, qw, nqw, d2w);
                    s_list[e] = 0xFFFFFFFFu;
                }
            }
            __syncthreads();
        }
        for (uint32_t base = 0; base < cnt; base += kPassThreads) {
            const uint32_t e = base + threadIdx.x;
            cells_tile<true>(a, ix, wl, X, e < cnt ? s_list[e] : 0xFFFFFFFFu, shard, true);
            __syncthreads();
        }
        if (ACC) {
            for (uint32_t base = 0; base < cnt; base += kPassThreads) {
                const uint32_t e = base + threadIdx.x;
                if (e >= cnt) continue;
                const uint32_t i = s_list[e];
                if (i == 0xFFFFFFFFu) continue;
                const float4 q = a.pairrec[2 * (size_t)i], nq = a.pairrec[2 * (size_t)i + 1];
                if (nq.w != 0.0f) continue;
                const float x = a.in.x[i], y = a.in.y[i], z = a.in.z[i];
                float nx = 0.0f, ny = 0.0f, nz = 0.0f;
                if (need_n) { nx = a.in.nx[i]; ny = a.in.ny[i]; nz = a.in.nz[i]; }
                const float px = xf_row(X.m + 0, x, y, z, 1.0f), py = xf_row(X.m + 4, x, y, z, 1.0f), pz = xf_row(X.m + 8, x, y, z, 1.0f);
                pair_step<OBJ>(acc, h, nx, ny, nz, px, py, pz, q, nq, dist2(px, py, pz, q.x, q.y, q.z));
            }
        }
        __syncthreads();
        if (threadIdx.x == 0) { s_total += cnt; s_cnt = 0; }
        __syncthreads();
    };

    constexpr uint32_t kPpt = ACC ? FUSED_PPT : 1u;
    constexpr uint32_t kTilePts = kPpt * kPassThreads;
    const uint32_t tiles = (a.n + kTilePts - 1) / kTilePts;
    constexpr uint32_t kTileChunk = 16;
    const uint32_t tiles_p = ACC ? ((tiles + 7u) / 8u) * 8u : ((tiles + 8u * kTileChunk - 1u) / (8u * kTileChunk)) * (8u * kTileChunk);
    constexpr int kCheck = ACC ? 1 : 1;
    int since = 0;
    for (uint32_t t = blockIdx.x; t < tiles_p; t += gridDim.x) {
        const uint32_t i0 = (ACC ? xcd_remap(t, tiles_p) : xcd_remap_chunked(t, kTileChunk)) * kTilePts + threadIdx.x;
        if (ACC) asm volatile("" ::: "memory");
        float x[kPpt], y[kPpt], z[kPpt], nx[kPpt], ny[kPpt], nz[kPpt];
        float4 q[kPpt], nq[kPpt], ce[kPpt];
        int32_t pa[kPpt];
#pragma unroll
        for (uint32_t k = 0; k < kPpt; k++) {
            const uint32_t i = i0 + k * kPassThreads;
            nq[k] = make_float4(0.f, 0.f, 0.f, 2.0f);
            pa[k] = -1;
            if (i < a.n) {
                if (ACC) {
                    const size_t o = (size_t)i;
                    x[k] = gcol<float>(s_col[0])[o]; y[k] = gcol<float>(s_col[1])[o]; z[k] = gcol<float>(s_col[2])[o];
                    if (need_n) { nx[k] = gcol<float>(s_col[3])[o]; ny[k] = gcol<float>(s_col[4])[o]; nz[k] = gcol<float>(s_col[5])[o]; }
                    else nx[k] = ny[k] = nz[k] = 0.0f;
                    q[k] = as_float4(gcol<f32x4_t>(s_col[6])[2 * o]); nq[k] = as_float4(gcol<f32x4_t>(s_col[6])[2 * o + 1]);
                    ce[k] = as_float4(gcol<f32x4_t>(s_col[7])[o]);
                } else {
                    x[k] = a.in.x[i]; y[k] = a.in.y[i]; z[k] = a.in.z[i];
                    pa[k] = a.pos_prev[i];
                    if ((uint32_t)pa[k] < ix.n) { q[k] = ix.tq[pa[k]]; nq[k].w = 0.0f; }
                    ce[k] = a.cert[i];
                }
            }
        }
        if (stop) return;
#ifdef RS_STAMPS2
        if (fs1 == 0) fs1 = __builtin_amdgcn_s_memrealtime();
#endif
#pragma unroll
        for (uint32_t k = 0; k < kPpt; k++) {
            const uint32_t i = i0 + k * kPassThreads;
            if (i < a.n) {
                const float px = xf_row(X.m + 0, x[k], y[k], z[k], 1.0f), py = xf_row(X.m + 4, x[k], y[k], z[k], 1.0f), pz = xf_row(X.m + 8, x[k], y[k], z[k], 1.0f);
                bool certified = false;
                float d2 = 0.0f;
                if (nq[k].w == 0.0f) {
                    d2 = dist2(px, py, pz, q[k].x, q[k].y, q[k].z);
                    const float m2 = dist2(px, py, pz, ce[k].x, ce[k].y, ce[k].z);
                    certified = (__builtin_amdgcn_sqrtf(d2) + __builtin_amdgcn_sqrtf(m2)) * 1.000002f < ce[k].w;
                    if (!ACC && !certified && d2 <= __int_as_float(0x7f800000) && (__float_as_uint(ce[k].w) & 1u) && a.certk) {
                        const int32_t pk = pa[k];
                        int32_t pw; float d2w;
                        if ((uint32_t)pk < ix.n && hood_test(a, ix, i, px, py, pz, m2, pk, d2, __float_as_int(q[k].w), pw, d2w)) {
                            certified = true;
                            d2 = d2w;
                        }
                    }
                }
                if (certified) {
                    if (ACC) pair_step<OBJ>(acc, h, nx[k], ny[k], nz[k], px, py, pz, q[k], nq[k], d2);
                } else {
                    s_list[atomicAdd(&s_cnt, 1u)] = i;
                }
            }
        }
        if (++since == kCheck) {
            since = 0;
            __syncthreads();
            if (s_cnt > (uint32_t)(kList - kCheck * (int)kTilePts)) flush();
        }
    }
    __syncthreads();
    flush();
    if (threadIdx.x == 0 && s_total) atomicAdd(wl.work.counts + shard * kShardStride + 1, s_total);
#ifdef RS_STAMPS2
    const unsigned long long fs2 = __builtin_amdgcn_s_memrealtime();
#endif
    if (ACC) acc_block_reduce_store(acc, a.partials, blockIdx.x);
#ifdef RS_STAMPS2
    if (ACC && blockIdx.x == 0 && threadIdx.x == 0) {
        double *dbg = a.partials + (size_t)8191 * kNSum;
        dbg[0] = (double)(fs1 - fs0); dbg[1] = (double)(fs2 - fs1); dbg[2] = (double)(__builtin_amdgcn_s_memrealtime() - fs2);
    }
#endif
}


__device__ __forceinline__ float boxmaxdist2(float px, float py, float pz, const float4 &lo, const float4 &hi)
{
    float dx = fmaxf(fabsf(px - lo.x), fabsf(px - hi.x));
    float dy = fmaxf(fabsf(py - lo.y), fabsf(py - hi.y));
    float dz = fmaxf(fabsf(pz - lo.z), fabsf(pz - hi.z));
    return (dx * dx + dy * dy) + dz * dz;
}

__device__ __forceinline__ unsigned long long wave_min_u64(unsigned long long v)
{
#pragma unroll
    for (int off = 32; off > 0; off >>= 1) {
        unsigned long long o = __shfl_xor(v, off, 64);
        v = o < v ? o : v;
    }
    return v;
}

__device__ __forceinline__ float wave_min_f32(float v)
{
#pragma unroll
    for (int off = 32; off > 0; off >>= 1) v = fminf(v, __shfl_xor(v, off, 64));
    return v;
}

constexpr int kWalkThreads = 64;
constexpr uint32_t kWaveWorkers = 8192;

template <bool BUDGETED>
__global__ __launch_bounds__(kWalkThreads, 6) void k_search_walk(PassArgs a, TargetIndex ix, WorkLists wl, ShardList list, uint32_t kWaveModeMax,
                                                                 uint32_t budget)
{
    if (a.loop) {
        if (a.loop->stop) return;
        a.X = a.loop->Xapply;
    }
    __shared__ uint32_t fr[1][2][kWaveFrontier];
    __shared__ uint32_t pre[kShards + 1];
    sl_prefix(list, pre);
    const float inf = __int_as_float(0x7f800000);
    if (pre[kShards] > kWaveModeMax) {
        for (uint32_t g = blockIdx.x * kWalkThreads + threadIdx.x; ; g += gridDim.x * kWalkThreads) {
            uint32_t i;
            if (!sl_locate(list, pre, g, i)) break;
            const float x = a.in.x[i], y = a.in.y[i], z = a.in.z[i];
            const float px = xf_row(a.X.m + 0, x, y, z, 1.0f), py = xf_row(a.X.m + 4, x, y, z, 1.0f), pz = xf_row(a.X.m + 8, x, y, z, 1.0f);
            Best b;
            b.pos = a.pos_out[i]; b.d2 = a.d2_out[i]; b.row = 0x7fffffff;
            if (b.pos >= 0) b.row = __float_as_int(ix.tq[b.pos].w);
            const uint32_t visits = oct_walk<BUDGETED>(ix, px, py, pz, b, budget);
            a.pos_out[i] = b.pos;
            a.d2_out[i] = b.d2;
            if (BUDGETED && visits > budget) sl_push(wl.retry, blockIdx.x & (kShards - 1), i);
            if (ix.dbg) {
                uint32_t mx = visits;
                for (int off = 32; off > 0; off >>= 1) mx = max(mx, (uint32_t)__shfl_xor((int)mx, off, 64));
                atomicAdd(ix.dbg + 4, (unsigned long long)visits);
                if ((threadIdx.x & 63) == 0) atomicAdd(ix.dbg + 5, (unsigned long long)mx * 64ull);
            }
        }
        return;
    }
    if (blockIdx.x >= kWaveWorkers) return;
    const int lane = threadIdx.x, wave = 0;
    const uint32_t nwaves = min(gridDim.x, kWaveWorkers);
    for (uint32_t w = blockIdx.x; ; w += nwaves) {
        uint32_t i;
        if (!sl_locate(list, pre, w, i)) break;
        const float x = a.in.x[i], y = a.in.y[i], z = a.in.z[i];
        const float px = xf_row(a.X.m + 0, x, y, z, 1.0f), py = xf_row(a.X.m + 4, x, y, z, 1.0f), pz = xf_row(a.X.m + 8, x, y, z, 1.0f);
        int32_t bpos = a.pos_out[i];
        float bd2 = a.d2_out[i];
        unsigned long long bkey = ~0ull;
        if (bpos >= 0) bkey = ((unsigned long long)__float_as_uint(bd2) << 32) | (unsigned long long)(uint32_t)__float_as_int(ix.tq[bpos].w);
        else bd2 = inf;
        float radius2 = bd2;
        const float pad = kSlackFrac * ix.h;
        bool overflowed = false;
        uint32_t nf = 0;
        {
            float mind = inf, maxd = inf;
            if (lane < (int)ix.ntop) {
                const float4 *bx = ix.boxes + 2 * ((size_t)ix.level_off[ix.top] + lane);
                const float4 lo = bx[0], hi = bx[1];
                if (lo.x <= hi.x) { mind = boxdist2(px, py, pz, lo, hi); maxd = boxmaxdist2(px, py, pz, lo, hi); }
            }
            radius2 = fminf(radius2, wave_min_f32(maxd));
            const float rp = __builtin_amdgcn_sqrtf(radius2) * 1.00001f + pad;
            const bool keep = mind <= rp * rp * 1.00001f && mind < inf;
            const unsigned long long m = __ballot(keep);
            if (keep) fr[wave][0][__popcll(m & ((1ull << lane) - 1ull))] = (uint32_t)lane;
            nf = (uint32_t)__popcll(m);
            __builtin_amdgcn_wave_barrier();
        }
        int cur = 0;
        for (int L = ix.top; L >= 1 && !overflowed; L--) {
            uint32_t nn = 0;
            for (uint32_t f0 = 0; f0 < nf; f0 += 8) {
                const uint32_t f = f0 + (uint32_t)(lane >> 3);
                float mind = inf, maxd = inf;
                uint32_t child = 0;
                if (f < nf) {
                    child = (fr[wave][cur][f] << 3) + (uint32_t)(lane & 7);
                    const float4 *bx = ix.boxes + 2 * ((size_t)ix.level_off[L - 1] + child);
                    const float4 lo = bx[0], hi = bx[1];
                    if (lo.x <= hi.x) { mind = boxdist2(px, py, pz, lo, hi); maxd = boxmaxdist2(px, py, pz, lo, hi); }
                }
                radius2 = fminf(radius2, wave_min_f32(maxd));
                const float rp = __builtin_amdgcn_sqrtf(radius2) * 1.00001f + pad;
                const bool keep = mind <= rp * rp * 1.00001f && mind < inf;
                const unsigned long long m = __ballot(keep);
                const uint32_t slot = nn + (uint32_t)__popcll(m & ((1ull << lane) - 1ull));
                if (keep && slot < (uint32_t)kWaveFrontier) fr[wave][cur ^ 1][slot] = child;
                nn += (uint32_t)__popcll(m);
            }
            if (nn > (uint32_t)kWaveFrontier) { overflowed = true; break; }
            nf = nn;
            cur ^= 1;
            __builtin_amdgcn_wave_barrier();
        }
        if (overflowed) {
            if (lane == 0) {
                Best b;
                b.pos = bpos; b.d2 = bd2; b.row = (bkey == ~0ull) ? 0x7fffffff : (int32_t)(uint32_t)(bkey & 0xFFFFFFFFull);
                oct_walk(ix, px, py, pz, b);
                a.pos_out[i] = b.pos;
                a.d2_out[i] = b.d2;
            }
            continue;
        }
        uint32_t second = 0x7f800000u;
        for (uint32_t f0 = 0; f0 < nf; f0 += 8) {
            const uint32_t f = f0 + (uint32_t)(lane >> 3);
            unsigned long long key = ~0ull;
            uint32_t j = 0;
            if (f < nf) {
                j = fr[wave][cur][f] * kLeaf + (uint32_t)(lane & 7);
                if (j < ix.n) {
                    const float4 q = ix.tq[j];
                    const float d2 = dist2(px, py, pz, q.x, q.y, q.z);
                    if (d2 == d2) key = ((unsigned long long)__float_as_uint(d2) << 32) | (unsigned long long)(uint32_t)__float_as_int(q.w);
                }
            }
            const unsigned long long best = wave_min_u64(key);
            const unsigned long long runner = wave_min_u64(key == best ? ~0ull : key);
            if (best < bkey) {
                second = min(second, min((uint32_t)(bkey >> 32), (uint32_t)(runner >> 32)));
                bkey = best;
                const unsigned long long who = __ballot(key == best);
                bpos = (int32_t)__shfl((int)j, __ffsll((long long)who) - 1, 64);
            } else if (best == bkey) {
                second = min(second, (uint32_t)(runner >> 32));
            } else {
                second = min(second, (uint32_t)(best >> 32));
            }
        }
        if (lane == 0 && bkey != ~0ull) {
            const float d1 = sqrtf(__uint_as_float((uint32_t)(bkey >> 32)));
            const float L = fminf(sqrtf(__uint_as_float(second)) * 0.999999f, (d1 + pad) * 0.99999f);
            a.cert[i] = make_float4(px, py, pz, cert_word((L > d1 * 1.000001f) ? L : 0.0f, false));
        }
        if (lane == 0) {
            a.pos_out[i] = bpos;
            a.d2_out[i] = (bkey == ~0ull) ? inf : __uint_as_float((uint32_t)(bkey >> 32));
        }
    }
}

template <bool W, int OBJ, bool T>
__global__ __launch_bounds__(kPassThreads) void k_accumulate(PassArgs a, const float4 *__restrict__ tn)
{
    AccT<W> acc; acc_zero(acc);
    const HotParams h = hot_params(a);
    const uint32_t tau = T ? a.rej.ws[kRejectTauWord] : 0u;
    const bool need_n = reads_src_normals<OBJ>(a.writeback, a.min_ndot);
    const uint32_t nbp = gridDim.x;
    const uint32_t total_blocks = (a.n + kPassThreads - 1) / kPassThreads;
    for (uint32_t lb = xcd_remap(blockIdx.x, nbp); lb < total_blocks; lb += nbp) {
        const uint32_t i = lb * kPassThreads + threadIdx.x;
        if (i >= a.n) continue;
        const float x = a.in.x[i], y = a.in.y[i], z = a.in.z[i];
        float nx = 0.0f, ny = 0.0f, nz = 0.0f;
        if (need_n) { nx = a.in.nx[i]; ny = a.in.ny[i]; nz = a.in.nz[i]; }
        float4 q = a.pairrec[2 * (size_t)i], nq = a.pairrec[2 * (size_t)i + 1];
        if (nq.w == 2.0f) {
            const int32_t pos = a.pos_out[i];
            if (pos >= 0) { q = tn[2 * (size_t)pos]; nq = tn[2 * (size_t)pos + 1]; }
            else nq = make_float4(0.f, 0.f, 0.f, 1.f);
            if (a.refresh_records) { a.pairrec[2 * (size_t)i] = q; a.pairrec[2 * (size_t)i + 1] = nq; }
        }
        const float px = xf_row(a.X.m + 0, x, y, z, 1.0f), py = xf_row(a.X.m + 4, x, y, z, 1.0f), pz = xf_row(a.X.m + 8, x, y, z, 1.0f);
        if (a.writeback) {
            a.out.x[i] = px; a.out.y[i] = py; a.out.z[i] = pz;
            a.out.nx[i] = xf_row(a.X.m + 0, nx, ny, nz, a.X.nrm_w); a.out.ny[i] = xf_row(a.X.m + 4, nx, ny, nz, a.X.nrm_w);
            a.out.nz[i] = xf_row(a.X.m + 8, nx, ny, nz, a.X.nrm_w);
        }
        if (nq.w != 0.0f) continue;
        if (T && a.rej.claim != kClaimNone && a.rej.keys[i] == 0xFFFFFFFFu) continue;
        if constexpr (OBJ == kObjColor) {
            const ColorPair cp = color_pair(a, i, (uint32_t)a.pos_out[i]);
            pair_step<OBJ, T>(acc, h, nx, ny, nz, px, py, pz, q, nq, dist2(px, py, pz, q.x, q.y, q.z), tau, &cp);
        } else
        pair_step<OBJ, T>(acc, h, nx, ny, nz, px, py, pz, q, nq, dist2(px, py, pz, q.x, q.y, q.z), tau);
    }
    acc_block_reduce_store(acc, a.partials, blockIdx.x);
}

template <bool W, int OBJ>
__global__ __launch_bounds__(kPassThreads) void k_accumulate_list(PassArgs a, const float4 *__restrict__ tn, ShardList list)
{
    if (a.loop) {
        if (a.loop->stop) return;
        a.X = a.loop->Xapply;
    }
    AccT<W> acc; acc_zero(acc);
    const HotParams h = hot_params(a);
    const bool need_n = reads_src_normals<OBJ>(false, a.min_ndot);
    const int wave = threadIdx.x >> 6, lane = threadIdx.x & 63;
    for (uint32_t shard = blockIdx.x + gridDim.x * wave; shard < (uint32_t)kShards; shard += gridDim.x * (kPassThreads / 64)) {
        const uint32_t cnt = min(list.counts[shard * kShardStride], list.cap);
        for (uint32_t e = lane; e < cnt; e += 64) {
            const uint32_t i = list.items[(size_t)shard * list.cap + e];
            const float x = a.in.x[i], y = a.in.y[i], z = a.in.z[i];
            float nx = 0.0f, ny = 0.0f, nz = 0.0f;
            if (need_n) { nx = a.in.nx[i]; ny = a.in.ny[i]; nz = a.in.nz[i]; }
            const int32_t pos = a.pos_out[i];
            float4 q = make_float4(0.f, 0.f, 0.f, 0.f), nq = make_float4(0.f, 0.f, 0.f, 1.f);
            if (pos >= 0) { q = tn[2 * (size_t)pos]; nq = tn[2 * (size_t)pos + 1]; }
            a.pairrec[2 * (size_t)i] = q; a.pairrec[2 * (size_t)i + 1] = nq;
            if (nq.w != 0.0f) continue;
            const float px = xf_row(a.X.m + 0, x, y, z, 1.0f), py = xf_row(a.X.m + 4, x, y, z, 1.0f), pz = xf_row(a.X.m + 8, x, y, z, 1.0f);
            pair_step<OBJ>(acc, h, nx, ny, nz, px, py, pz, q, nq, dist2(px, py, pz, q.x, q.y, q.z));
        }
    }
    acc_block_reduce_store(acc, a.partials, a.partial_col0 + blockIdx.x);
}

__device__ __forceinline__ void read_list_words(const uint32_t *cnt, int t, uint32_t &len, uint32_t &searched, uint32_t &dropped)
{
    uint32_t v = cnt[t * kShardStride], u = cnt[t * kShardStride + 1];
    uint32_t d = (t < 2) ? cnt[t * kShards * kShardStride + 2] : 0u;
#pragma unroll
    for (int off = 32; off > 0; off >>= 1) {
        v += (uint32_t)__shfl_xor((int)v, off, 64);
        u += (uint32_t)__shfl_xor((int)u, off, 64);
        d += (uint32_t)__shfl_xor((int)d, off, 64);
    }
    len = v; searched = u; dropped = d;
}

__global__ __launch_bounds__(256) void k_final_reduce(const double *__restrict__ partials, int nblocks,
                                                      double *out_dev, double *out_mapped, uint32_t *ticket,
                                                      unsigned long long seq, uint32_t *counters_to_clear, int keep_nonempty)
{
    __shared__ double red[256];
    const int k = blockIdx.x, t = threadIdx.x;
    double s = 0.0;
    for (int j = t; j < nblocks; j += 256) s += partials[(size_t)j * kNSum + k];
    red[t] = s;
    __syncthreads();
#pragma unroll
    for (int off = 128; off > 0; off >>= 1) {
        if (t < off) red[t] += red[t + off];
        __syncthreads();
    }
    __shared__ int last;
    if (t == 0) {
        out_dev[k] = red[0];
        if (out_mapped) out_mapped[k] = red[0];
        __threadfence_system();
        last = (atomicAdd(ticket, 1u) == gridDim.x - 1);
    }
    __syncthreads();
    if (last) {
        if (counters_to_clear) {
            __shared__ uint32_t s_len;
            if (t < 64) {
                uint32_t len, searched, dropped;
                read_list_words(counters_to_clear, t, len, searched, dropped);
                if (t == 0) {
                    s_len = len;
                    const double lenw = (double)len + (dropped ? kListDropped : 0.0);
                    out_dev[kNSum - 1] = lenw; out_dev[kNSum - 2] = (double)searched;
                    if (out_mapped) { out_mapped[kNSum - 1] = lenw; out_mapped[kNSum - 2] = (double)searched; }
                }
            }
            __syncthreads();
            if (t < 2) counters_to_clear[t * kShards * kShardStride + 2] = 0;
            if (t < kShards) counters_to_clear[t * kShardStride + 1] = 0;
            if (!(keep_nonempty && s_len > 0u))
                for (int c = t; c < 2 * kShards; c += 256) counters_to_clear[c * kShardStride] = 0;
        }
        if (t == 0) {
            *ticket = 0;
            if (out_mapped) {
                __threadfence_system();
                reinterpret_cast<volatile unsigned long long *>(out_mapped)[kNSum] = seq;
            }
        }
    }
}

template <bool REDUCE>
__global__ __launch_bounds__(512) void k_reduce_solve(const double *__restrict__ partials, int nblocks, double *out_dev, int solve_only, LoopState *loop,
                                                       LoopConfig cfg, LoopRecord *ring, int ring_len, uint32_t *counters_to_clear)
{
    __shared__ double s_sum[kNSum];
    __shared__ uint32_t s_len, s_unc;
    const int t = threadIdx.x, lane = t & 63, wave = t >> 6;
#ifdef RS_STAMPS
    const unsigned long long ts0 = __builtin_amdgcn_s_memrealtime();
#endif
    const LoopState ls = *loop;
    uint32_t cw0 = 0, cw1 = 0, cw2 = 0;
    const bool want_counters = !solve_only && REDUCE && counters_to_clear && t < 64;
    if (want_counters) {
        cw0 = counters_to_clear[t * kShardStride]; cw1 = counters_to_clear[t * kShardStride + 1];
        cw2 = (t < 2) ? counters_to_clear[t * kShards * kShardStride + 2] : 0u;
    }
    __shared__ double s_part[8][kNSum];
    double accw = 0.0;
    if (!solve_only && REDUCE && lane < kNSum) {
        if (nblocks <= 512) {
            double c[64];
#pragma unroll
            for (int j = 0; j < 64; j++) { const int b = wave + 8 * j; c[j] = (b < nblocks) ? partials[(size_t)b * kNSum + lane] : 0.0; }
#pragma unroll
            for (int j = 0; j < 64; j++) accw += c[j];
        } else {
            for (int b = wave; b < nblocks; b += 8) accw += partials[(size_t)b * kNSum + lane];
        }
    }
    double rec = 0.0;
    if ((solve_only || !REDUCE) && t < kNSum) rec = out_dev[t];
    if (ls.stop) return;
#ifdef RS_STAMPS
    const unsigned long long tsA = __builtin_amdgcn_s_memrealtime();
#endif
    if (t == 0) { s_len = 0; s_unc = 0; }
    if (!solve_only && REDUCE) {
        if (lane < kNSum) s_part[wave][lane] = accw;
        __syncthreads();
        if (t < kNSum) {
            double x = 0.0;
#pragma unroll
            for (int w = 0; w < 8; w++) x += s_part[w][t];
            s_sum[t] = (t < kNAccW) ? x : 0.0;
        }
    } else if (t < kNSum) s_sum[t] = rec;
    __syncthreads();
    if (!solve_only && counters_to_clear) {
        if (REDUCE) {
            if (t < 64) {
#pragma unroll
                for (int off = 32; off > 0; off >>= 1) {
                    cw0 += (uint32_t)__shfl_xor((int)cw0, off, 64);
                    cw1 += (uint32_t)__shfl_xor((int)cw1, off, 64);
                    cw2 += (uint32_t)__shfl_xor((int)cw2, off, 64);
                }
                if (t == 0) { s_len = cw2 ? 0xFFFFFFFFu : cw0; s_unc = cw1; }
            }
            if (t < kShards) counters_to_clear[t * kShardStride + 1] = 0;
            for (int c = t; c < 2 * kShards; c += 512) counters_to_clear[c * kShardStride] = 0;
        } else if (t == 0) {
            s_len = (s_sum[kNSum - 1] >= kListDropped) ? 0xFFFFFFFFu : (uint32_t)s_sum[kNSum - 1];
            s_unc = (uint32_t)s_sum[kNSum - 2];
        }
    }
    __syncthreads();
#ifdef RS_STAMPS
    const unsigned long long ts1 = __builtin_amdgcn_s_memrealtime();
#endif
    int it = ls.iters;
    if (!solve_only) {
        const uint32_t len = s_len, unc = s_unc;
        if (cfg.tree && len > 0u && (!cfg.walk_in_loop || len == 0xFFFFFFFFu)) { if (t == 0) { loop->stop = 1; loop->reason = LOOP_REDO_PASS; } return; }
        it += 1;
        LoopRecord &r = ring[it % ring_len];
        if (t < kNSum) { const double v = (t >= kNAccW) ? 0.0 : s_sum[t]; r.sums[t] = v; if (REDUCE) out_dev[t] = v; }
        if (t == 0) {
            loop->iters = it;
            r.solved = 0;
            r.pad = (int32_t)unc;
            r.list_len = (int32_t)len; r.reserved = 0;
        }
        if (cfg.tree && (unc > cfg.uncertified_limit || (cfg.walk_in_loop && len > cfg.list_limit))) { if (t == 0) { loop->stop = 1; loop->reason = LOOP_SLOW; } return; }
    }
    if (t != 0) return;
    const float diff = (float)s_sum[33];
    if (ls.small_step || !((cfg.fixed_iters || diff > cfg.diff_threshold) && it < cfg.max_iters)) {
        loop->stop = 1; loop->reason = LOOP_DONE;
        return;
    }
    symmicp_sums S;
    for (int k = 0; k < kNSum; k++) S.s[k] = (k >= kNAccW) ? 0.0 : s_sum[k];
    float pbar[3], qbar[3], av[3], tv[3], rc = 0.f, Xi[16];
    const int st = solve::solve_mode(cfg.mode, S, cfg.pivot, pbar, qbar, av, tv, &rc, Xi, false);
    if (st != SYMMICP_OK || !(rc > 1e-6f)) { loop->stop = 1; loop->reason = LOOP_HOST_SOLVE; return; }
#ifdef RS_STAMPS
    const unsigned long long ts2 = __builtin_amdgcn_s_memrealtime();
#endif
    float Xn[16];
    solve::mat4_mul(Xi, ls.X, Xn);
    for (int k = 0; k < 16; k++) loop->X[k] = Xn[k];
    const float *ap = cfg.incremental ? Xi : Xn;
    for (int k = 0; k < 12; k++) loop->Xapply.m[k] = ap[k];
    loop->Xapply.nrm_w = cfg.nrm_w;
    LoopRecord &r = ring[it % ring_len];
    for (int k = 0; k < 16; k++) { r.increment[k] = Xi[k]; r.X[k] = Xn[k]; }
    r.rcond = rc; r.status = st; r.solved = 1;
#ifdef RS_STAMPS2
    r.sums[37] = partials[(size_t)8191 * kNSum]; r.sums[38] = partials[(size_t)8191 * kNSum + 1]; r.sums[39] = partials[(size_t)8191 * kNSum + 2];
#elif defined(RS_STAMPS)
    r.sums[37] = (double)(ts1 - ts0) + 1e-4 * (double)(tsA - ts0); r.sums[38] = (double)(ts2 - ts1); r.sums[39] = (double)(__builtin_amdgcn_s_memrealtime() - ts2);
#endif
    if (cfg.eps_rotation > 0.f && cfg.eps_translation > 0.f && !cfg.fixed_iters) {
        const double tr = ((double)Xi[0] + Xi[5] + Xi[10] - 1.0) * 0.5;
        const double ang = acos(tr > 1.0 ? 1.0 : (tr < -1.0 ? -1.0 : tr));
        const double tn = sqrt((double)Xi[3] * Xi[3] + (double)Xi[7] * Xi[7] + (double)Xi[11] * Xi[11]);
        if (ang < cfg.eps_rotation && tn < cfg.eps_translation) loop->small_step = 1;
    }
}

__global__ __launch_bounds__(64) void k_solve_probe(int mode, int exact_rc, const symmicp_sums *__restrict__ sums, int n, const float *pivot,
                                                    const float *__restrict__ X_in, int32_t *status, float *pbar, float *qbar, float *a, float *t,
                                                    float *rcond, float *out16, float *X_out)
{
    const int i = blockIdx.x * blockDim.x + threadIdx.x;
    if (i >= n) return;
    const symmicp_sums S = sums[i];
    float pb[3] = {0.f, 0.f, 0.f}, qb[3] = {0.f, 0.f, 0.f}, av[3] = {0.f, 0.f, 0.f}, tv[3] = {0.f, 0.f, 0.f}, rc = 0.f, Xi[16], Xn[16];
    for (int k = 0; k < 16; k++) Xi[k] = 0.f;
    const bool ex = exact_rc != 0;
    const int st = solve::solve_mode(mode, S, pivot, pb, qb, av, tv, &rc, Xi, ex);
    status[i] = st;
    rcond[i] = rc;
    for (int k = 0; k < 3; k++) { pbar[3 * i + k] = pb[k]; qbar[3 * i + k] = qb[k]; a[3 * i + k] = av[k]; t[3 * i + k] = tv[k]; }
    for (int k = 0; k < 16; k++) out16[16 * (size_t)i + k] = Xi[k];
    if (X_in) {
        solve::mat4_mul(Xi, X_in + 16 * (size_t)i, Xn);
        for (int k = 0; k < 16; k++) X_out[16 * (size_t)i + k] = Xn[k];
    }
}

void launch_solve_probe(int mode, int exact_rc, const symmicp_sums *sums, int n, const float *pivot, const float *X_in, int32_t *status, float *pbar,
                        float *qbar, float *a, float *t, float *rcond, float *out16, float *X_out, hipStream_t s)
{
    if (n > 0) hipLaunchKernelGGL(k_solve_probe, dim3((n + 63) / 64), dim3(64), 0, s, mode, exact_rc, sums, n, pivot, X_in, status, pbar, qbar, a, t, rcond, out16, X_out);
}

__global__ __launch_bounds__(64) void k_loop_end(const LoopState *loop, LoopState *host_copy, unsigned long long *done_flag, unsigned long long seq)
{
    if (threadIdx.x == 0) {
        *host_copy = *loop;
        __threadfence_system();
        *reinterpret_cast<volatile unsigned long long *>(done_flag) = seq;
    }
}

__global__ __launch_bounds__(64) void k_publish(const double *__restrict__ sums_dev, double *out_mapped, unsigned long long seq)
{
    if (threadIdx.x < kNSum) out_mapped[threadIdx.x] = sums_dev[threadIdx.x];
    __threadfence_system();
    __syncthreads();
    if (threadIdx.x == 0) {
        __threadfence_system();
        reinterpret_cast<volatile unsigned long long *>(out_mapped)[kNSum] = seq;
    }
}

__global__ __launch_bounds__(kPassThreads) void k_nn_brute(CloudSoA src, uint32_t n_s, Affine X,
                                                          const float4 *__restrict__ tq, uint32_t n_t,
                                                          uint32_t tiles_per_split, unsigned long long *best64)
{
    __shared__ float4 tile[kBruteTile];
    float px[kBruteQ], py[kBruteQ], pz[kBruteQ], bd[kBruteQ];
    uint32_t bj[kBruteQ];
    const uint32_t q0 = blockIdx.x * (kPassThreads * kBruteQ) + threadIdx.x;
#pragma unroll
    for (int k = 0; k < kBruteQ; k++) {
        uint32_t i = q0 + k * kPassThreads;
        float x = 0.f, y = 0.f, z = 0.f;
        if (i < n_s) { x = src.x[i]; y = src.y[i]; z = src.z[i]; }
        px[k] = xf_row(X.m + 0, x, y, z, 1.0f); py[k] = xf_row(X.m + 4, x, y, z, 1.0f); pz[k] = xf_row(X.m + 8, x, y, z, 1.0f);
        bd[k] = __int_as_float(0x7f800000); bj[k] = 0xFFFFFFFFu;
    }
    const uint32_t tile0 = blockIdx.y * tiles_per_split;
    const uint32_t ntiles = (n_t + kBruteTile - 1) / kBruteTile;
    const uint32_t tile1 = min(tile0 + tiles_per_split, ntiles);
    for (uint32_t t = tile0; t < tile1; t++) {
        const uint32_t base = t * kBruteTile;
        __syncthreads();
#pragma unroll
        for (int k = 0; k < kBruteTile / kPassThreads; k++) {
            uint32_t j = base + k * kPassThreads + threadIdx.x;
            tile[k * kPassThreads + threadIdx.x] = (j < n_t) ? tq[j] : make_float4(__int_as_float(0x7fc00000), 0.f, 0.f, 0.f);
        }
        __syncthreads();
#pragma unroll 4
        for (int j = 0; j < kBruteTile; j++) {
            float4 q = tile[j];
#pragma unroll
            for (int k = 0; k < kBruteQ; k++) {
                float d2 = dist2(px[k], py[k], pz[k], q.x, q.y, q.z);
                if (d2 < bd[k]) { bd[k] = d2; bj[k] = base + j; }
            }
        }
    }
#pragma unroll
    for (int k = 0; k < kBruteQ; k++) {
        uint32_t i = q0 + k * kPassThreads;
        if (i < n_s && bj[k] != 0xFFFFFFFFu) {
            unsigned long long key = ((unsigned long long)__float_as_uint(bd[k]) << 32) | (unsigned long long)bj[k];
            atomicMin(best64 + i, key);
        }
    }
}

__global__ __launch_bounds__(256) void k_identity_d2(CloudSoA in, Affine X, CloudSoA tgt, uint32_t tgt_offset, uint32_t n, float *d2)
{
    const uint32_t i = blockIdx.x * blockDim.x + threadIdx.x;
    if (i >= n) return;
    const float x = in.x[i], y = in.y[i], z = in.z[i];
    const float px = xf_row(X.m + 0, x, y, z, 1.0f), py = xf_row(X.m + 4, x, y, z, 1.0f), pz = xf_row(X.m + 8, x, y, z, 1.0f);
    const uint32_t j = tgt_offset + i;
    d2[i] = dist2(px, py, pz, tgt.x[j], tgt.y[j], tgt.z[j]);
}

__global__ __launch_bounds__(256) void k_pairs_d2(CloudSoA in, Affine X, const int32_t *__restrict__ pos, const float4 *__restrict__ tq, uint32_t n_t, uint32_t n, float *d2)
{
    const uint32_t i = blockIdx.x * blockDim.x + threadIdx.x;
    if (i >= n) return;
    const int32_t p = pos[i];
    float v = __int_as_float(0x7f800000);
    if (p >= 0 && (uint32_t)p < n_t) {
        const float x = in.x[i], y = in.y[i], z = in.z[i];
        const float px = xf_row(X.m + 0, x, y, z, 1.0f), py = xf_row(X.m + 4, x, y, z, 1.0f), pz = xf_row(X.m + 8, x, y, z, 1.0f);
        const float4 q = tq[p];
        v = dist2(px, py, pz, q.x, q.y, q.z);
    }
    d2[i] = v;
}

void launch_pairs_d2(const CloudSoA &in, const Affine &X, const int32_t *pos, const float4 *tq, uint32_t n_t, uint32_t n, float *d2, hipStream_t s)
{
    if (n) hipLaunchKernelGGL(k_pairs_d2, dim3((n + 255) / 256), dim3(256), 0, s, in, X, pos, tq, n_t, n, d2);
}

void launch_identity_d2(const CloudSoA &in, const Affine &X, const CloudSoA &tgt, uint32_t tgt_offset, uint32_t n, float *d2, hipStream_t s)
{
    hipLaunchKernelGGL(k_identity_d2, dim3((n + 255) / 256), dim3(256), 0, s, in, X, tgt, tgt_offset, n, d2);
}

template <typename F>
static void with_instantiation(const PassArgs &a, F &&f)
{
    auto obj = [&](auto W) {
        if (a.obj == kObjGicp) f(W, std::integral_constant<int, kObjGicp>());
        else if (a.obj == kObjPlane) f(W, std::integral_constant<int, kObjPlane>());
        else f(W, std::integral_constant<int, kObjSym>());
    };
    if (a.loss != SYMMICP_LOSS_NONE) obj(std::true_type());
    else obj(std::false_type());
}

template <typename F>
static void with_trim(const PassArgs &a, F &&f)
{
    if (a.obj == kObjColor) {
        auto trim = [&](auto W) {
            if (pass_rejects(a)) f(W, std::integral_constant<int, kObjColor>(), std::true_type());
            else f(W, std::integral_constant<int, kObjColor>(), std::false_type());
        };
        if (a.loss != SYMMICP_LOSS_NONE) trim(std::true_type());
        else trim(std::false_type());
        return;
    }
    with_instantiation(a, [&](auto W, auto OBJ) {
        if (pass_rejects(a)) f(W, OBJ, std::true_type());
        else f(W, OBJ, std::false_type());
    });
}

void launch_pass_identity(const PassArgs &a, CloudSoA tgt, int blocks, bool vec4_ok, hipStream_t s)
{
    if (pass_rejects(a)) launch_reject(a, SYMMICP_CORR_IDENTITY, tgt, nullptr, s);
    with_trim(a, [&](auto W, auto OBJ, auto T) {
        if (vec4_ok) hipLaunchKernelGGL((k_pass_identity<4, W, OBJ, T>), dim3(blocks), dim3(kPassThreads), 0, s, a, tgt);
        else hipLaunchKernelGGL((k_pass_identity<1, W, OBJ, T>), dim3(blocks), dim3(kPassThreads), 0, s, a, tgt);
    });
}

void launch_pass_indexed(const PassArgs &a, const float4 *tn, int blocks, hipStream_t s)
{
    if (pass_rejects(a)) launch_reject(a, SYMMICP_CORR_BRUTE, CloudSoA{}, tn, s);
    with_trim(a, [&](auto W, auto OBJ, auto T) { hipLaunchKernelGGL((k_pass_indexed<W, OBJ, T>), dim3(blocks), dim3(kPassThreads), 0, s, a, tn); });
}

void launch_accumulate(const PassArgs &a, const float4 *tn, int blocks, hipStream_t s)
{
    if (pass_rejects(a)) launch_reject(a, SYMMICP_CORR_TREE, CloudSoA{}, tn, s);
    with_trim(a, [&](auto W, auto OBJ, auto T) { hipLaunchKernelGGL((k_accumulate<W, OBJ, T>), dim3(blocks), dim3(kPassThreads), 0, s, a, tn); });
}

uint32_t shard_capacity(uint32_t n_points)
{
    const uint32_t nb = (n_points + kPassThreads - 1) / kPassThreads;
    const uint32_t nbp = ((nb + 7u) / 8u) * 8u;
    return ((nbp + kShards - 1) / kShards) * kPassThreads;
}

uint32_t walk_blocks_full(const WorkLists &wl)
{
    return kShards * (wl.work.cap / kWalkThreads);
}

void launch_pass_tree_split(const PassArgs &a_in, const TargetIndex &ix, const WorkLists &wl, int acc_blocks, uint32_t walk_blocks,
                            int stage, int compact_blocks, const PassTuning &tune, hipStream_t s, hipEvent_t *ev)
{
    PassArgs a = a_in;
    a.refresh_records = (stage != 1) ? 1 : 0;
    const uint32_t wave_mode_max = tune.wave_mode_max;
    const uint32_t nb = (a.n + kPassThreads - 1) / kPassThreads;
    const uint32_t nbp = ((nb + 7u) / 8u) * 8u;
    if (ev) hipEventRecord(ev[0], s);
    if (stage != 2 && nbp) {
        if (compact_blocks > 0) hipLaunchKernelGGL((k_pass_fused<false, false, kObjSym>), dim3(min((uint32_t)compact_blocks, nbp)), dim3(kPassThreads), 0, s, a, ix, wl);
        else {
            const uint32_t chunk = tune.cells_chunk ? tune.cells_chunk : 16u;
            uint32_t qshift = nb >= 3072u ? 8u : (nb >= 1536u ? 7u : 6u);
            if (tune.cells_queries == 64u) qshift = 6u; else if (tune.cells_queries == 128u) qshift = 7u; else if (tune.cells_queries == 256u) qshift = 8u;
            const uint32_t nq = (a.n + (1u << qshift) - 1u) >> qshift;
            const uint32_t nbc = ((nq + 8u * chunk - 1u) / (8u * chunk)) * (8u * chunk);
            if (a.make_hood) hipLaunchKernelGGL(k_search_cells<true>, dim3(nbc), dim3(kPassThreads), 0, s, a, ix, wl, chunk, qshift);
            else hipLaunchKernelGGL(k_search_cells<false>, dim3(nbc), dim3(kPassThreads), 0, s, a, ix, wl, chunk, qshift);
        }
    }
    if (ev) hipEventRecord(ev[1], s);
    if (ev) hipEventRecord(ev[2], s);
    if (stage != 1 && nbp) {
        if (walk_blocks == 0 || walk_blocks > walk_blocks_full(wl)) walk_blocks = walk_blocks_full(wl);
        const uint32_t wmm = a.pos_prev ? wave_mode_max : 0u;
        if (a.budget_walk) {
            const uint32_t budget = tune.walk_budget;
            hipLaunchKernelGGL(k_search_walk<true>, dim3(walk_blocks), dim3(kWalkThreads), 0, s, a, ix, wl, wl.work, wmm, budget);
            hipLaunchKernelGGL(k_search_walk<false>, dim3(8192), dim3(kWalkThreads), 0, s, a, ix, wl, wl.retry, 0xFFFFFFFFu, 0xFFFFFFFFu);
        } else {
            hipLaunchKernelGGL(k_search_walk<false>, dim3(walk_blocks), dim3(kWalkThreads), 0, s, a, ix, wl, wl.work, wmm, 0xFFFFFFFFu);
        }
    }
    if (ev) hipEventRecord(ev[3], s);
    launch_accumulate(a, ix.tn, acc_blocks, s);
    if (ev) hipEventRecord(ev[4], s);
}

void launch_final_reduce(const double *partials, int blocks, double *out_dev, double *out_host_mapped, uint32_t *ticket,
                         unsigned long long seq, uint32_t *counters_to_clear, int keep_nonempty, hipStream_t s)
{
    hipLaunchKernelGGL(k_final_reduce, dim3(kNSum), dim3(256), 0, s, partials, blocks, out_dev, out_host_mapped, ticket, seq,
                       counters_to_clear, keep_nonempty);
}

void launch_pass_fused(const PassArgs &a, const TargetIndex &ix, const WorkLists &wl, int blocks, hipStream_t s)
{
    with_instantiation(a, [&](auto W, auto OBJ) { hipLaunchKernelGGL((k_pass_fused<true, W, OBJ>), dim3(blocks), dim3(kPassThreads), 0, s, a, ix, wl); });
}

void launch_loop_stragglers(const PassArgs &a, const TargetIndex &ix, const WorkLists &wl, int list_blocks, const PassTuning &tune, hipStream_t s)
{
    const uint32_t wave_mode_max = tune.wave_mode_max;
    hipLaunchKernelGGL(k_search_walk<false>, dim3(512), dim3(kWalkThreads), 0, s, a, ix, wl, wl.work, wave_mode_max, 0xFFFFFFFFu);
    with_instantiation(a, [&](auto W, auto OBJ) {
        hipLaunchKernelGGL((k_accumulate_list<W, OBJ>), dim3(list_blocks), dim3(kPassThreads), 0, s, a, ix.tn, wl.work);
    });
}

void launch_reduce_solve(const double *partials, int blocks, double *out_dev, int mode, LoopState *loop, LoopConfig cfg, LoopRecord *ring, int ring_len,
                         uint32_t *counters_to_clear, hipStream_t s)
{
    if (mode == 0) hipLaunchKernelGGL(k_reduce_solve<true>, dim3(1), dim3(512), 0, s, partials, blocks, out_dev, 0, loop, cfg, ring, ring_len, counters_to_clear);
    else hipLaunchKernelGGL(k_reduce_solve<false>, dim3(1), dim3(512), 0, s, partials, blocks, out_dev, mode == 2 ? 1 : 0, loop, cfg, ring, ring_len, counters_to_clear);
}

void launch_loop_end(const LoopState *loop, LoopState *host_copy, unsigned long long *done_flag, unsigned long long seq, hipStream_t s)
{
    hipLaunchKernelGGL(k_loop_end, dim3(1), dim3(64), 0, s, loop, host_copy, done_flag, seq);
}

void launch_publish(const double *sums_dev, double *out_host_mapped, unsigned long long seq, hipStream_t s)
{
    hipLaunchKernelGGL(k_publish, dim3(1), dim3(64), 0, s, sums_dev, out_host_mapped, seq);
}

void launch_nn_brute(const CloudSoA &src, uint32_t n_s, const Affine &X, const float4 *tq, uint32_t n_t,
                     unsigned long long *best64, hipStream_t s)
{
    const uint32_t qblocks = (n_s + kPassThreads * kBruteQ - 1) / (kPassThreads * kBruteQ);
    const uint32_t ntiles = (n_t + kBruteTile - 1) / kBruteTile;
    uint32_t splits = 1;
    if (qblocks < 2048) splits = (2048 + qblocks - 1) / qblocks;
    if (splits > ntiles) splits = ntiles;
    if (splits < 1) splits = 1;
    if (splits > 65535) splits = 65535;
    const uint32_t tiles_per_split = (ntiles + splits - 1) / splits;
    splits = (ntiles + tiles_per_split - 1) / tiles_per_split;
    hipMemsetAsync(best64, 0xFF, sizeof(unsigned long long) * (size_t)n_s, s);
    hipLaunchKernelGGL(k_nn_brute, dim3(qblocks, splits), dim3(kPassThreads), 0, s, src, n_s, X, tq, n_t, tiles_per_split, best64);
}

}
```

### icp-symm_amd/csrc/symmicp_internal.h

```cpp
#pragma once
#include <hip/hip_runtime.h>
#include <stdint.h>
#include <stddef.h>
#include "symmicp.h"

namespace symmicp {

constexpr int kNSum = SYMMICP_NSUM;
constexpr int kNAcc = 37;
constexpr int kNAccW = 38;
constexpr double kListDropped = 4294967296.0;
constexpr int kLeaf = 8;
constexpr int kFan = 8;
constexpr int kMaxTreeLevels = 12;
constexpr int kMortonBits = 10;
constexpr int kPassThreads = 256;
constexpr int kBruteTile = 1024;
constexpr int kBruteQ = 4;

constexpr bool mode_device_solves(int mode)
{
    return mode == SYMMICP_MODE_QUIRKS || mode == SYMMICP_MODE_PAPER || mode == SYMMICP_MODE_PLANE || mode == SYMMICP_MODE_GICP;
}
constexpr bool mode_known(int mode) { return mode_device_solves(mode) || mode == SYMMICP_MODE_P2P || mode == SYMMICP_MODE_COLOR; }
constexpr int mode_solves_as(int mode) { return mode == SYMMICP_MODE_COLOR ? SYMMICP_MODE_PLANE : mode; }

constexpr int kObjSym = 0, kObjPlane = 1, kObjGicp = 2, kObjColor = 3;
constexpr int mode_obj(int mode)
{
    return mode == SYMMICP_MODE_PLANE ? kObjPlane : mode == SYMMICP_MODE_GICP ? kObjGicp : mode == SYMMICP_MODE_COLOR ? kObjColor : kObjSym;
}

struct Affine {
    float m[12];
    float nrm_w;
};

struct CloudSoA {
    float *x, *y, *z, *nx, *ny, *nz;
};

struct TargetIndex {
    const float4 *tq;
    const float4 *tn;
    uint32_t n;
    const float4 *boxes;
    uint32_t level_off[kMaxTreeLevels];
    int32_t top;
    uint32_t ntop;
    const uint32_t *ctop;
    const uint2 *cells;
    int32_t glevel;
    int32_t gdim;
    float ox, oy, oz;
    float h, inv_h;
    unsigned long long *dbg;
    unsigned long long *dbg_trace;
    const float4 *onodes;
    uint32_t olevel_off[kMortonBits + 2];
};

constexpr uint32_t kOctCfMask = 0x0FFFFFFFu;
__host__ __device__ inline uint32_t oct_nch(uint32_t packed) { return packed >> 28; }
__host__ __device__ inline uint32_t oct_cf(uint32_t packed) { return packed & kOctCfMask; }

constexpr int kShards = 64;
constexpr int kShardStride = 16;
struct ShardList {
    uint32_t *items;
    uint32_t *counts;
    uint32_t cap;
};
struct WorkLists {
    ShardList work;
    ShardList retry;
};

struct LoopState {
    float X[16];
    Affine Xapply;
    int32_t stop;
    int32_t reason;
    int32_t iters;
    int32_t small_step;
};
enum { LOOP_RUNNING = 0, LOOP_DONE = 1, LOOP_REDO_PASS = 2, LOOP_HOST_SOLVE = 3, LOOP_SLOW = 4 };
struct LoopConfig {
    int32_t mode, fixed_iters, max_iters, incremental, tree;
    float diff_threshold, eps_rotation, eps_translation, nrm_w;
    float pivot[3];
    uint32_t uncertified_limit;
    int32_t walk_in_loop;
    uint32_t list_limit;
};
struct LoopRecord {
    double sums[SYMMICP_NSUM];
    float increment[16], X[16];
    float rcond;
    int32_t status;
    int32_t solved;
    int32_t pad;
    int32_t list_len, reserved;
};

struct RecipArgs {
    TargetIndex six;
    Affine inv;
};
constexpr size_t kRecipTailWords = (sizeof(RecipArgs) + 7) / 8;
constexpr uint32_t kRejectWsWords = 16 + 3 * 2048;
constexpr uint32_t kRejectTauWord = 3;
struct RejectRecord {
    uint32_t population;
    uint32_t kept, tau_bits;
    uint32_t gated;
    uint32_t claimed, reciprocal;
};
enum RejectClaim : int32_t { kClaimNone = 0, kClaimOneToOne = 1, kClaimReciprocal = 2 };
struct RejectArgs {
    uint32_t *keys;
    uint32_t *ws;
    RejectRecord *host;
    unsigned long long *table;
    const uint32_t *order;
    const RecipArgs *recip;
    uint32_t n_t;
    int32_t claim;
    float rho;
    float med_f2;
};
static_assert(sizeof(RejectArgs) == 64 && sizeof(RejectRecord) == 24, "RejectArgs takes the room of the nine fields it replaced");

struct PassArgs {
    CloudSoA in, out;
    uint32_t n;
    uint32_t tgt_offset;
    Affine X;
    float pivot[3];
    float max_d2;
    float min_ndot;
    int32_t p2p;
    int32_t writeback;
    const unsigned long long *best64;
    int32_t *pos_prev;
    float *d2_out;
    int32_t *pos_out;
    double *partials;
    float4 *pairrec;
    int32_t budget_walk;
    int32_t refresh_records;
    float4 *cert;
    uint4 *certk;
    float2 *hoodr;
    int32_t make_hood;
    int32_t use_slack;
    const LoopState *loop;
    uint32_t partial_cols, partial_col0;
    const uint2 *pkt_tab;
    uint32_t pkt_count;
    uint32_t pkt_waves;
    uint32_t pkt_front_cap;
    uint32_t *pkt_fallbacks;
    uint32_t pkt_chunk, pkt_lds_pad;
    int32_t loss;
    float loss_scale;
    int32_t obj;
    float gicp_k;
    RejectArgs rej;
    const float4 *tgt_color;
    const float *src_int;
    float color_lam, color_om;
};
static_assert(sizeof(PassArgs) == 432 && offsetof(PassArgs, rej) == 344 && offsetof(PassArgs, tgt_color) == 408 && offsetof(PassArgs, src_int) == 416,
              "PassArgs keeps its layout");
__host__ __device__ inline bool pass_rejects(const PassArgs &a) { return a.rej.keys != nullptr; }

struct PassTuning {
    uint32_t wave_mode_max = 20000u;
    uint32_t cells_chunk = 16u;
    uint32_t cells_queries = 0u;
    uint32_t walk_budget = 160u;
};

constexpr int kBatchThreads = 512;
constexpr int kBatchQ = 4;
constexpr int kBatchChunk = kBatchThreads * kBatchQ;
constexpr int kBatchTile = SYMMICP_BATCH_MAX_POINTS;
constexpr int kBatchMerge = 1024;
__host__ __device__ constexpr uint32_t batch_splits(uint32_t n) { return n <= 256u ? 8u : n <= 512u ? 4u : n <= 1024u ? 2u : 1u; }
static_assert(kBatchThreads / 8 >= 64 && (kBatchThreads / 2) * kBatchQ == kBatchMerge, "a split is at least one wave; two splits cover kBatchMerge rows");
struct BatchProblem {
    uint32_t src_first, src_count, tgt_first, tgt_count;
    float pivot[3];
    uint32_t slot;
};
struct BatchArgs {
    const float *src_xyz, *src_nrm, *tgt_xyz, *tgt_nrm;
    const BatchProblem *problems;
    const float *guess;
    symmicp_batch_result *out;
    float *trace_X;
    double *trace_sums;
    int32_t mode, max_iters, fixed_iters;
    float diff_threshold, max_d2, min_ndot, eps_rotation, eps_translation;
};
void launch_batch_align(const BatchArgs &a, uint32_t n_problems, hipStream_t s);

void launch_pass_identity(const PassArgs &a, CloudSoA tgt, int blocks, bool vec4_ok, hipStream_t s);
void launch_pass_indexed(const PassArgs &a, const float4 *tn , int blocks, hipStream_t s);
void launch_pass_tree_split(const PassArgs &a, const TargetIndex &ix, const WorkLists &wl, int acc_blocks, uint32_t walk_blocks,
                            int stage, int compact_blocks, const PassTuning &tune, hipStream_t s, hipEvent_t *ev);
void launch_pass_tree_first(const PassArgs &a, const TargetIndex &ix, const WorkLists &wl, int acc_blocks, hipStream_t s, hipEvent_t *ev);
uint32_t walk_blocks_full(const WorkLists &wl);
uint32_t shard_capacity(uint32_t n_points);
void launch_final_reduce(const double *partials, int blocks, double *out_dev, double *out_host_mapped, uint32_t *ticket,
                         unsigned long long seq, uint32_t *counters_to_clear, int keep_nonempty, hipStream_t s);
void launch_pass_fused(const PassArgs &a, const TargetIndex &ix, const WorkLists &wl, int blocks, hipStream_t s);
void launch_loop_stragglers(const PassArgs &a, const TargetIndex &ix, const WorkLists &wl, int list_blocks, const PassTuning &tune, hipStream_t s);
void launch_reduce_solve(const double *partials, int blocks, double *out_dev, int mode, LoopState *loop, LoopConfig cfg, LoopRecord *ring, int ring_len,
                         uint32_t *counters_to_clear, hipStream_t s);
void launch_solve_probe(int mode, int exact_rc, const symmicp_sums *sums, int n, const float *pivot, const float *X_in, int32_t *status, float *pbar,
                        float *qbar, float *a, float *t, float *rcond, float *out16, float *X_out, hipStream_t s);
void launch_loop_end(const LoopState *loop, LoopState *host_copy, unsigned long long *done_flag, unsigned long long seq, hipStream_t s);
void launch_publish(const double *sums_dev, double *out_host_mapped, unsigned long long seq, hipStream_t s);
void launch_nn_brute(const CloudSoA &src, uint32_t n_s, const Affine &X, const float4 *tq, uint32_t n_t,
                     unsigned long long *best64, hipStream_t s);

void launch_bbox(const float *x, const float *y, const float *z, uint32_t n, uint32_t *bbox_ord6, hipStream_t s);
void launch_morton(const float *x, const float *y, const float *z, uint32_t n, float ox, float oy, float oz,
                   float inv_h0, uint32_t *keys, uint32_t *vals, hipStream_t s);
void radix_sort_pairs(uint32_t *keys, uint32_t *vals, uint32_t *keys_tmp, uint32_t *vals_tmp, uint32_t n,
                      int key_bits, uint32_t *hist_ws, size_t hist_ws_elems, hipStream_t s);
size_t radix_sort_ws_elems(uint32_t n);
void launch_gather_f4(const float *x, const float *y, const float *z, const float *nx, const float *ny, const float *nz,
                      const uint32_t *order, uint32_t n, float4 *tq, float4 *tn, hipStream_t s);
void launch_gather_soa(const CloudSoA &src, const uint32_t *order, uint32_t n, CloudSoA dst, hipStream_t s);
void launch_offset_u32(const uint32_t *in, uint32_t off, uint32_t n, uint32_t *out, hipStream_t s);
void launch_packet_runs(const CloudSoA &src, uint32_t n, float jump_factor, uint2 *runs, uint32_t *keys, uint32_t *vals, uint32_t *count, int key_bits, hipStream_t s);
void launch_packet_cost(const CloudSoA &src, const uint2 *runs, uint32_t npk, const TargetIndex &ix, uint32_t *keys, int key_bits, hipStream_t s);
void launch_packet_table(const uint32_t *order, const uint2 *runs, uint32_t npk, uint2 *tab, hipStream_t s);
void launch_deinterleave3(const float *raw, size_t row_stride, size_t offset, uint32_t n, float *x, float *y, float *z, hipStream_t s);
void launch_level_hist(const uint32_t *keys, uint32_t n, uint32_t *hist16, hipStream_t s);
void launch_cell_table(const uint32_t *keys, uint32_t n, int glevel, const uint32_t *nid_top, uint32_t *ctop, uint2 *cells, hipStream_t s);
void launch_oct_flags(const uint32_t *keys, uint32_t n, int level, uint32_t *nid, hipStream_t s);
void launch_exclusive_scan(uint32_t *data, uint32_t n, uint32_t *tile_ws , hipStream_t s);
void launch_oct_first(const uint32_t *keys, uint32_t n, int level, const uint32_t *nid, uint32_t *first, hipStream_t s);
void launch_oct_nodes(int level, const float4 *tq, uint32_t n, const uint32_t *first, uint32_t n_nodes, const uint32_t *nid_next,
                      uint32_t n_nodes_next, const float4 *nodes_next, float4 *nodes, uint32_t leaf_max, hipStream_t s);
void launch_leaf_boxes(const float4 *tq, uint32_t n, float4 *boxes, uint32_t nleaf_padded, hipStream_t s);
void launch_node_boxes(const float4 *child, uint32_t nchild_padded, float4 *parent, uint32_t nparent_padded, hipStream_t s);
void launch_iota_f4(const float *x, const float *y, const float *z, const float *nx, const float *ny, const float *nz,
                    uint32_t n, float4 *tq, float4 *tn, hipStream_t s);
void launch_unpermute(const CloudSoA &cur, const uint32_t *order, uint32_t n, float *xyz_aos, float *nrm_aos, hipStream_t s);
void launch_corr_out(const int32_t *pos, const unsigned long long *best64, const float *d2, const float4 *tq,
                     const uint32_t *src_order, uint32_t n, int mode, uint32_t tgt_offset, int32_t *idx_out, float *d2_out,
                     const uint32_t *rej_keys , uint32_t rej_tau, hipStream_t s);

void launch_reject(const PassArgs &a, int corr, CloudSoA tgt, const float4 *tn, hipStream_t s);
void launch_select_probe(const uint32_t *keys, uint32_t n, uint32_t k, uint32_t *ws, hipStream_t s);
void launch_unique_probe(const int32_t *tgt_row, const uint32_t *d2_bits, uint32_t n, unsigned long long *table, uint32_t n_t,
                         uint8_t *winner_out, hipStream_t s);

void launch_relabel_tq(float4 *tq, uint32_t n, const uint32_t *labels, hipStream_t s);
void launch_reverse_nn_probe(const TargetIndex &six, const Affine &inv, const float *q_xyz, uint32_t n_q, int32_t *label_out, float *d2_out, hipStream_t s);

void launch_identity_d2(const CloudSoA &in, const Affine &X, const CloudSoA &tgt, uint32_t tgt_offset, uint32_t n, float *d2, hipStream_t s);
void launch_pairs_d2(const CloudSoA &in, const Affine &X, const int32_t *pos, const float4 *tq, uint32_t n_t, uint32_t n, float *d2, hipStream_t s);
void launch_normals_knn(const TargetIndex &ix, int k, const float vp[3], float *nrm_out, float *curv_out, hipStream_t s);
void launch_knn(const TargetIndex &ix, int k, int32_t *rows_out, float *d2_out, hipStream_t s);

void launch_color_permute_target(const float *intensity, const float *grad3, const float4 *tq, uint32_t n, float4 *dst, hipStream_t s);
void launch_color_permute_source(const float *intensity, const uint32_t *order, uint32_t off, uint32_t n, float *dst, hipStream_t s);
void launch_color_unpermute_source(const float *src_int, const uint32_t *order, uint32_t n, float *out_rows, hipStream_t s);
void launch_color_gradient(const TargetIndex &ix, const float *intensity_rows, const int32_t *knn_rows, int k, float4 *rec_rows, float *grad_rows,
                           hipStream_t s);

void launch_voxel_keys(const CloudSoA &cl, uint32_t n, float inv, const int lo[3], uint64_t nx, uint64_t ny, uint32_t *keys, uint32_t *vals,
                       hipStream_t s);
void launch_voxel_segments(const uint32_t *keys, uint32_t n, uint32_t *vid_excl, uint32_t *first, uint32_t *scan_ws, uint32_t *m0_out,
                           hipStream_t s);
void launch_voxel_keep(const uint32_t *first, uint32_t m0, uint32_t min_points, uint32_t *kid_excl, uint32_t *scan_ws, uint32_t *kfirst,
                       uint32_t *kcount, uint32_t *m_out, hipStream_t s);
void launch_voxel_mean(const CloudSoA &sorted, const uint32_t *kfirst, const uint32_t *kcount, uint32_t m, int with_normals, float *xyz_out,
                       float *nrm_out, int32_t *count_out, hipStream_t s);
void launch_voxel_of(const uint32_t *keys, const uint32_t *rows, const uint32_t *vid_excl, const uint32_t *first, const uint32_t *kid_excl,
                     uint32_t n, uint32_t min_points, int32_t *voxel_of, hipStream_t s);

void launch_radius_count(const TargetIndex &ix, float r2, int32_t *count_rows, hipStream_t s);
void launch_radius_fill(const TargetIndex &ix, float r2, const uint32_t *offs_rows, int32_t *rows_out, float *d2_out, hipStream_t s);
void launch_spfh(const TargetIndex &ix, float r2, float *spfh_sorted, float *spfh_rows , int32_t *count_rows, hipStream_t s);
void launch_fpfh(const TargetIndex &ix, float r2, const float *spfh_sorted, float *fpfh_rows, hipStream_t s);

void launch_iss_saliency(const TargetIndex &ix, float r2, int32_t min_neighbors, float gamma21, float gamma32, float *s_sorted, float *s_rows,
                         int32_t *k_rows, hipStream_t s);
void launch_iss_nms(const TargetIndex &ix, float r2, int32_t min_neighbors, const float *s_sorted, uint32_t *flag_rows, hipStream_t s);
void launch_iss_scatter(const uint32_t *flag_rows, const uint32_t *pos_rows, uint32_t n, int32_t *rows_out, hipStream_t s);

void launch_feature_nn(const float *fa, uint32_t na, const float *fb, uint32_t nb, int queries_per_thread, uint32_t splits, void *partial,
                       int32_t *nn_out, float *d2_out, float *second_out, hipStream_t s);
size_t feature_nn_partial_bytes(uint32_t na, uint32_t splits);
void launch_ransac_hyp(const float *pq8, uint32_t m, uint32_t H, unsigned long long base, float max_dist2, float edge2, float *hyp,
                       uint8_t *status, int32_t *inliers, uint32_t *surv, uint32_t *n_surv, hipStream_t s);
void launch_ransac_eval(const float *pq8, uint32_t m, const float *hyp, const uint32_t *surv, const uint32_t *n_surv, uint32_t n_surv_host,
                        float max_dist2, int32_t *inliers, hipStream_t s);
void launch_ransac_argmax(const uint8_t *status, const int32_t *inliers, uint32_t H, unsigned long long *best, hipStream_t s);

}
```

### icp-symm_amd/py/symmicp/__init__.py

```python
import ctypes as C
import os
import sys

import numpy as np

_PKG = os.path.dirname(os.path.abspath(__file__))
_ROOT = os.path.dirname(os.path.dirname(_PKG))
LIB_PATH = os.environ.get("SYMMICP_LIB") or os.path.join(_ROOT, "lib", "libsymmicp.so")

NSUM = 40
UNIQUE_ID_BYTES = 128
OK, ERR_ARG, ERR_SIZE, ERR_DEGENERATE, ERR_IO, ERR_HIP, ERR_STATE, ERR_COMM = range(8)
ERR_NO_CONSENSUS = 8
RANSAC_EVALUATED, RANSAC_REPEATED, RANSAC_EDGE, RANSAC_DEGENERATE, RANSAC_FAR = range(5)
MODE_QUIRKS, MODE_PAPER, MODE_P2P, MODE_PLANE, MODE_GICP, MODE_COLOR = 0, 1, 2, 3, 5, 7
CORR_IDENTITY, CORR_BRUTE, CORR_TREE = 0, 1, 2
APPLY_DEFAULT, APPLY_INCREMENTAL, APPLY_CUMULATIVE = 0, 1, 2
LOSS_NONE, LOSS_HUBER, LOSS_TUKEY, LOSS_CAUCHY, LOSS_GEMAN_MCCLURE = range(5)
_LOSS_NAMES = {"none": LOSS_NONE, "huber": LOSS_HUBER, "tukey": LOSS_TUKEY, "cauchy": LOSS_CAUCHY,
               "geman_mcclure": LOSS_GEMAN_MCCLURE}

_STATUS_NAMES = {0: "OK", 1: "ERR_ARG", 2: "ERR_SIZE", 3: "ERR_DEGENERATE", 4: "ERR_IO", 5: "ERR_HIP",
                 6: "ERR_STATE", 7: "ERR_COMM", 8: "ERR_NO_CONSENSUS"}

# ... 1050 lines not shown
    def batch_align_raw(self, src, src_n, tgt, tgt_n, problems, guesses, cfg, trace=False):
        return _batch_call(self._L.symmicp_ctx_batch_align, (self._h,), src, src_n, tgt, tgt_n, problems, guesses, cfg, trace)

    def align_multistart(self, src, src_n, tgt, tgt_n, guesses, **cfg):
        g = np.ascontiguousarray(guesses, np.float32).reshape(-1, 16)
        return self.batch_align(src, src_n, tgt, tgt_n, [(0, len(src), 0, len(tgt))] * len(g), g, **cfg)

    def enable_timing(self, on=True):
        self._chk(self._L.symmicp_enable_timing(self._h, int(on)))

    def reset_stats(self):
        self._chk(self._L.symmicp_reset_stats(self._h))

    def stats(self):
        s = Stats()
        self._chk(self._L.symmicp_get_stats(self._h, C.byref(s)))
        d = {k: getattr(s, k) for k, _ in Stats._fields_}
        d["kernel_ms"] = list(s.kernel_ms)
        d["kernel_launches"] = list(s.kernel_launches)
        d["pass_ms_head"] = list(s.pass_ms_head)
        return d

    def solve_probe(self, mode, sums, exact_rc, pivot=None, X_in=None):
        S = np.ascontiguousarray(np.asarray(sums, np.float64).reshape(-1, NSUM))
        n = S.shape[0]
        o = dict(status=np.zeros(n, np.int32), pbar=np.zeros((n, 3), np.float32), qbar=np.zeros((n, 3), np.float32),
                 a=np.zeros((n, 3), np.float32), t=np.zeros((n, 3), np.float32), rcond=np.zeros(n, np.float32),
                 out16=np.zeros((n, 4, 4), np.float32))
        pv = None if pivot is None else _fptr(np.ascontiguousarray(pivot, np.float32))
        xin = xout = None
        if X_in is not None:
            X_in = np.ascontiguousarray(np.asarray(X_in, np.float32).reshape(n, 4, 4))
            o["X_out"] = np.zeros((n, 4, 4), np.float32)
            xin, xout = _fptr(X_in), _fptr(o["X_out"])
        self._chk(self._L.symmicp_ctx_solve_probe(self._h, int(mode), int(bool(exact_rc)), S.ctypes.data_as(C.POINTER(Sums)), n, pv, xin,
                                                  o["status"].ctypes.data_as(C.POINTER(C.c_int32)), _fptr(o["pbar"]), _fptr(o["qbar"]),
                                                  _fptr(o["a"]), _fptr(o["t"]), _fptr(o["rcond"]), _fptr(o["out16"]), xout))
        return o

    def loop_solve(self, mode, sums, X_in=None, pivot=None, diff_threshold=1.0, fixed_iters=0, max_iters=10, iters=0, small_step=0,
                   eps_rotation=0.0, eps_translation=0.0, incremental=0):
        S = Sums()
        for k, v in enumerate(np.asarray(sums, np.float64).reshape(NSUM)):
            S.s[k] = v
        X_in = np.ascontiguousarray(np.eye(4, dtype=np.float32) if X_in is None else np.asarray(X_in, np.float32).reshape(16))
        pv = None if pivot is None else _fptr(np.ascontiguousarray(pivot, np.float32))
        ii = np.array([mode, fixed_iters, max_iters, iters, small_step, incremental], np.int32)
        ff = np.array([diff_threshold, eps_rotation, eps_translation], np.float32)
        st = np.zeros(4, np.int32); X = np.zeros(16, np.float32); Xa = np.zeros(12, np.float32)
        ri = np.zeros(16, np.float32); rX = np.zeros(16, np.float32); rrc = np.zeros(1, np.float32); r2 = np.zeros(2, np.int32)
        i32 = lambda a: a.ctypes.data_as(C.POINTER(C.c_int32))
        self._chk(self._L.symmicp_ctx_loop_solve(self._h, C.byref(S), pv, _fptr(X_in), i32(ii), _fptr(ff), i32(st), _fptr(X), _fptr(Xa),
                                                 _fptr(ri), _fptr(rX), _fptr(rrc), i32(r2)))
        return dict(stop=int(st[0]), reason=int(st[1]), iters=int(st[2]), small_step=int(st[3]), X=X.reshape(4, 4), Xapply=Xa.reshape(3, 4),
                    ring_increment=ri.reshape(4, 4), ring_X=rX.reshape(4, 4), ring_rcond=float(rrc[0]), ring_status=int(r2[0]), ring_solved=int(r2[1]))

    def index_info(self):
        o = IndexInfo()
        o.struct_size = C.sizeof(IndexInfo)
        self._chk(self._L.symmicp_ctx_index_info(self._h, C.byref(o)))
        d = {k: getattr(o, k) for k, _ in IndexInfo._fields_ if k != "struct_size"}
        d["origin"] = np.array(o.origin, np.float32)
        for k in ("h0", "h", "inv_h"):
            d[k] = np.float32(d[k])
        d["level_off"] = np.array(o.level_off, np.uint32)
        d["olevel_off"] = np.array(o.olevel_off, np.uint32)
        d["level_hist"] = np.array(o.level_hist, np.uint32)
        d["surface_like"] = bool(o.surface_like)
        return d

    def index_arrays(self):
        d = self.index_info()
        gl = d["grid_level"] > 0
        d["tq"] = np.zeros((d["n"], 4), np.float32)
        d["tn"] = np.zeros((d["n"], 2, 4), np.float32)
        d["boxes"] = np.zeros((d["n_boxes"], 2, 4), np.float32)
        d["ctop"] = np.zeros(d["ctop_len"] if gl else 0, np.uint32)
        d["cells"] = np.zeros(((d["n_blocks"] if gl else 0) * 512, 2), np.uint32)
        d["onodes"] = np.zeros((d["n_onodes"], 2, 4), np.float32)
        u32 = lambda a: a.ctypes.data_as(C.POINTER(C.c_uint32)) if a.size else None
        self._chk(self._L.symmicp_ctx_index_arrays(self._h, _fptr(d["tq"]), _fptr(d["tn"]), _fptr(d["boxes"]), u32(d["ctop"]), u32(d["cells"]),
                                                   _fptr(d["onodes"])))
        return d

    def source_share(self):
        nl, npk, so, ck = C.c_size_t(0), C.c_size_t(0), C.c_int32(0), C.c_int32(0)
        self._chk(self._L.symmicp_ctx_source_share(self._h, C.byref(nl), C.byref(npk), C.byref(so), C.byref(ck), None, None))
        order = np.zeros(nl.value, np.uint32) if so.value else None
        tab = np.zeros((npk.value, 2), np.uint32)
        u32 = lambda a: a.ctypes.data_as(C.POINTER(C.c_uint32)) if a is not None and a.size else None
        self._chk(self._L.symmicp_ctx_source_share(self._h, None, None, None, None, u32(order), u32(tab)))
        return dict(n_local=nl.value, pkt_count=npk.value, sorted=bool(so.value), cost_keyed=bool(ck.value), order=order, pkt_tab=tab)

    def radix_sort_probe(self, keys, vals, key_bits):
        k = np.array(keys, np.uint32).reshape(-1)
        v = np.array(vals, np.uint32).reshape(-1)
        if k.shape != v.shape:
            raise ValueError("keys and vals differ in length")
        u32 = lambda a: a.ctypes.data_as(C.POINTER(C.c_uint32))
        self._chk(self._L.symmicp_ctx_radix_sort_probe(self._h, u32(k), u32(v), k.size, int(key_bits)))
        return k, v

    def select_probe(self, keys, k):
        a = np.ascontiguousarray(np.asarray(keys, np.uint32).reshape(-1))
        kth, nle = C.c_uint32(0), C.c_uint64(0)
        self._chk(self._L.symmicp_ctx_select_probe(self._h, a.ctypes.data_as(C.POINTER(C.c_uint32)), a.size, int(k), C.byref(kth), C.byref(nle)))
        return kth.value, nle.value

    def unique_probe(self, tgt_row, d2_bits, n_t):
        r = np.ascontiguousarray(np.asarray(tgt_row, np.int32).reshape(-1))
        d = np.ascontiguousarray(np.asarray(d2_bits, np.uint32).reshape(-1))
        if r.size != d.size:
            raise ValueError("unique_probe: tgt_row and d2_bits differ in length")
        w = np.zeros(r.size, np.uint8)
        self._chk(self._L.symmicp_ctx_unique_probe(self._h, r.ctypes.data_as(C.POINTER(C.c_int32)), d.ctypes.data_as(C.POINTER(C.c_uint32)),
                                                   r.size, int(n_t), w.ctypes.data_as(C.POINTER(C.c_uint8))))
        return w.astype(bool)

    def reverse_nn_probe(self, db, queries, labels=None, X=None):
        d, q = _cloud(db), _cloud(queries)
        lab = None if labels is None else np.ascontiguousarray(np.asarray(labels, np.int32).reshape(-1))
        if lab is not None and lab.size != d.shape[0]:
            raise ValueError("reverse_nn_probe: one label per db point")
        Xa = None if X is None else np.ascontiguousarray(np.asarray(X, np.float32).reshape(16))
        out = np.zeros(q.shape[0], np.int32)
        d2 = np.zeros(q.shape[0], np.float32)
        self._chk(self._L.symmicp_ctx_reverse_nn_probe(self._h, _fptr(d), None if lab is None else lab.ctypes.data_as(C.POINTER(C.c_int32)), d.shape[0],
                                                       _fptr(q), q.shape[0], None if Xa is None else _fptr(Xa),
                                                       out.ctypes.data_as(C.POINTER(C.c_int32)), _fptr(d2)))
        return out, d2

    def reciprocal_info(self):
        v, b, n, t = C.c_int32(0), C.c_uint64(0), C.c_uint64(0), C.c_uint64(0)
        self._chk(self._L.symmicp_ctx_reciprocal_info(self._h, C.byref(v), C.byref(b), C.byref(n), C.byref(t)))
        return dict(index_valid=bool(v.value), index_bytes=b.value, index_builds=n.value, table_words=t.value)

    def scan_probe(self, data):
        d = np.array(data, np.uint32).reshape(-1)
        self._chk(self._L.symmicp_ctx_scan_probe(self._h, d.ctypes.data_as(C.POINTER(C.c_uint32)), d.size))
        return d

    def set_loop_log(self, on=True):
        self._chk(self._L.symmicp_set_loop_log(self._h, int(bool(on))))

    def loop_log(self):
        n = C.c_size_t(0)
        self._chk(self._L.symmicp_get_loop_log(self._h, None, 0, C.byref(n)))
        buf = (LoopLogEntry * max(1, n.value))()
        self._chk(self._L.symmicp_get_loop_log(self._h, buf, n.value, C.byref(n)))
        out = []
        for e in buf[:n.value]:
            out.append(dict(sums=np.array(e.sums[:], np.float64), increment=np.array(e.increment[:], np.float32).reshape(4, 4),
                            X=np.array(e.X[:], np.float32).reshape(4, 4), rcond=e.rcond, iter=e.iter, status=e.status, solved=e.solved,
                            list_len=e.list_len, reason=e.reason, batch=e.batch))
        return out


class MyICP:

    def __init__(self, mode=MODE_QUIRKS, corr=CORR_IDENTITY, max_iters=10, diff_threshold=1.0, verbose=True, **extra):
        self._cfg = dict(mode=mode, corr=corr, max_iters=max_iters, diff_threshold=diff_threshold,
                         verbose=int(bool(verbose)), **extra)
        self.cloud_src = self.cloud_tgt = None
        self.normals_src = self.normals_tgt = None
        self._final = np.eye(4, dtype=np.float32)
        self.last_result = None
        self._loss = (LOSS_NONE, 0.0)
        self._gicp_eps = None
        self._trim = 1.0
        self._one_to_one = False
        self._reciprocal = False
        self._median = 0.0
        self._color_weight = None
        self.intensity_src = self.intensity_tgt = None
        self._levels = []
        self.level_results = []
        self._global = None
        self.global_result = None
        self._have_src = self._have_tgt = False
        self.multistart_results = []

    def alignMultiStart(self, guesses):
        assert self.cloud_src is not None and self.cloud_tgt is not None
        keys = ("mode", "max_iters", "diff_threshold", "max_corr_dist", "fixed_iters", "min_normal_dot", "eps_rotation", "eps_translation")
        cfg = {k: self._cfg[k] for k in keys if k in self._cfg}
        batch_config(**cfg)
        g = np.ascontiguousarray(guesses, np.float32).reshape(-1, 16)
        if self._cfg["mode"] in (MODE_PAPER, MODE_P2P, MODE_PLANE) and max(len(self.cloud_src), len(self.cloud_tgt)) <= BATCH_MAX_POINTS and len(g):
            self.estimateNormals()
        else:
            z = np.zeros_like
            st, _ = _batch_align(lib().symmicp_batch_align, (int(self._cfg.get("device", -1)),), self.cloud_src, z(self.cloud_src), self.cloud_tgt,
                                 z(self.cloud_tgt), [(0, len(self.cloud_src), 0, len(self.cloud_tgt))] * len(g), g if len(g) else None, False, cfg)
            raise SymmIcpError(st if st != OK else ERR_ARG, "alignMultiStart")
        with Engine(**dict(self._cfg, verbose=0)) as e:
            self.multistart_results = e.align_multistart(self.cloud_src, self.normals_src, self.cloud_tgt, self.normals_tgt, g, **cfg)
        best = -1
        for k, r in enumerate(self.multistart_results):
            if r["status"] == OK and (best < 0 or (r["pairs"], -r["diff_final"]) > (self.multistart_results[best]["pairs"],
                                                                                   -self.multistart_results[best]["diff_final"])):
                best = k
        if best >= 0:
            self.last_result = self.multistart_results[best]
            self._final = self.last_result["transform"]
            if self._cfg["verbose"]:
                print(format_result(self._final), end="", flush=True)
        return best

    def multiStartResults(self):
        return self.multistart_results

    def setMaxCorrespondenceDistance(self, d):
        self._cfg["max_corr_dist"] = float(d)

    def setVoxelLevels(self, levels):
        levels = [(float(l), int(i), float(d)) for l, i, d in levels]
        if levels and self._cfg["mode"] == MODE_COLOR:
            raise SymmIcpError(ERR_ARG, "MODE_COLOR does not run voxel levels (intensities are not averaged per voxel yet)")
        self._levels = levels

    def setGlobalInit(self, fpfh_radius, max_dist, voxel_leaf=0.0, normal_k=10, hypotheses=100000, seed=0, mutual=True, max_ratio=0.0,
                      edge_ratio=0.9, refits=1, iss=False, iss_salient_radius=0.0, iss_non_max_radius=0.0, iss_gamma21=0.975, iss_gamma32=0.975,
                      iss_min_neighbors=5):
        self._global = dict(fpfh_radius=float(fpfh_radius), max_dist=float(max_dist), voxel_leaf=float(voxel_leaf), normal_k=int(normal_k),
                            hypotheses=int(hypotheses), seed=int(seed), mutual=bool(mutual), max_ratio=float(max_ratio),
                            edge_ratio=float(edge_ratio), refits=int(refits), iss=bool(iss), iss_salient_radius=float(iss_salient_radius),
                            iss_non_max_radius=float(iss_non_max_radius), iss_gamma21=float(iss_gamma21), iss_gamma32=float(iss_gamma32),
                            iss_min_neighbors=int(iss_min_neighbors))

    def clearGlobalInit(self):
        self._global = None

    def globalResult(self):
        return self.global_result

    def _global_init(self, e):
        g = self._global
        clouds = []
        for xyz, nrm in ((self.cloud_src, self.normals_src if self._have_src else None),
                         (self.cloud_tgt, self.normals_tgt if self._have_tgt else None)):
            if g["voxel_leaf"] > 0:
                d = e.voxel_downsample(xyz, g["voxel_leaf"], nrm)
                xyz, nrm = d["xyz"], d["nrm"]
            if nrm is None:
                nrm, _ = e.estimate_normals(xyz, g["normal_k"])
            clouds.append((xyz, e.fpfh(xyz, nrm, g["fpfh_radius"])))
        (src, fs), (tgt, ft) = clouds
        kp = None
        if g["iss"]:
            try:
                kp = [e.iss_keypoints(x, g["iss_salient_radius"], g["iss_non_max_radius"], g["iss_gamma21"], g["iss_gamma32"], g["iss_min_neighbors"])
                      for x in (src, tgt)]
            except SymmIcpError as err:
                raise SymmIcpError(err.status, "global initialisation: ISS keypoints: " + (e._L.symmicp_last_error(e._h) or b"").decode())
            if min(len(kp[0]), len(kp[1])) < 3:
                raise SymmIcpError(ERR_NO_CONSENSUS, "global initialisation: ISS keypoints: fewer than 3 keypoints (%d in the source, %d in the target)"
                                   % (len(kp[0]), len(kp[1])))
            pairs, _ = e.feature_correspondences(fs[kp[0]], ft[kp[1]], g["mutual"], g["max_ratio"])
            pairs = np.stack([kp[0][pairs[:, 0]], kp[1][pairs[:, 1]]], 1).astype(np.int32)
        else:
            pairs, _ = e.feature_correspondences(fs, ft, g["mutual"], g["max_ratio"])
        if len(pairs) < 3:
            raise SymmIcpError(ERR_NO_CONSENSUS, "global initialisation: fewer than 3 feature correspondences")
        r = e.ransac(src, tgt, pairs, g["max_dist"], g["hypotheses"], g["seed"], g["edge_ratio"], g["refits"], check=False)
        r.update(correspondences=len(pairs), source_points=len(src), target_points=len(tgt),
                 source_keypoints=0 if kp is None else len(kp[0]), target_keypoints=0 if kp is None else len(kp[1]))
        self.global_result = r
        if self._cfg["verbose"] and kp is not None:
            print("global init: %d -> %d source and %d -> %d target points, %d and %d ISS keypoints, %d correspondences, %d of %d hypotheses evaluated, "
                  "%d -> %d inliers" % (len(self.cloud_src), len(src), len(self.cloud_tgt), len(tgt), len(kp[0]), len(kp[1]), len(pairs), r["evaluated"],
                                        g["hypotheses"], r["inliers_ransac"], r["inliers_final"]), flush=True)
        elif self._cfg["verbose"]:
            print("global init: %d -> %d source and %d -> %d target points, %d correspondences, %d of %d hypotheses evaluated, %d -> %d inliers"
                  % (len(self.cloud_src), len(src), len(self.cloud_tgt), len(tgt), len(pairs), r["evaluated"], g["hypotheses"],
                     r["inliers_ransac"], r["inliers_final"]), flush=True)
        if r["status"] != OK:
            raise SymmIcpError(r["status"], "global initialisation: RANSAC: " + (e._L.symmicp_last_error(e._h) or b"").decode())
        return r["transform"]

    def levelResults(self):
        return self.level_results
    def setGicpEpsilon(self, eps):
        self._gicp_eps = float(eps)

    def setColorWeight(self, lam):
        self._color_weight = float(lam)

    def setTrimFraction(self, fraction):
        self._trim = float(fraction)

    def setOneToOne(self, on):
        self._one_to_one = bool(on)

    def setReciprocalCorrespondences(self, on):
        self._reciprocal = bool(on)

    def setMedianFactor(self, factor):
        self._median = float(factor)

    def setRobustLoss(self, loss, scale):
        self._loss = (loss_code(loss), float(scale))

    def LoadCloud(self, src_path, tgt_path):
        self.cloud_src, _ = pcd_read(src_path)
        self.cloud_tgt, _ = pcd_read(tgt_path)
        self.intensity_src, _ = pcd_read_intensity(src_path)
        self.intensity_tgt, _ = pcd_read_intensity(tgt_path)
# ... 123 lines not shown
```

Before: 30650.

## Add certified-only pass kernel for tree correspondence when no search was needed

Adds a lightweight pass kernel that checks each point's certificate and accumulates the pair directly. Uncertified points are resolved by a per-block neighbourhood test, so the full fused pass with its work list is not run. The kernel is chosen per chunk once the previous pass reported an empty work list and zero scanned pairs, and the loop is split into short head chunks so the host can switch to it early. A new scan counter is packed into the searched-pairs slot. If a certified pass ever comes back incomplete, the path is disabled for the rest of the alignment, which costs a redo pass.

```diff
diff --git a/icp-symm_amd/csrc/engine.cpp b/icp-symm_amd/csrc/engine.cpp
--- a/icp-symm_amd/csrc/engine.cpp
+++ b/icp-symm_amd/csrc/engine.cpp
@@ -34,6 +34,8 @@
     w.budget_walk = tri("SYMMICP_BUDGET_WALK");
     w.optimistic = tri("SYMMICP_OPTIMISTIC");
     w.compact = tri("SYMMICP_COMPACT");
+    w.cert_pass = (int)num("SYMMICP_CERT_PASS", 1);
+    w.cert_head = (int)num("SYMMICP_CERT_HEAD", 4);
     w.pass_blocks = (int)num("SYMMICP_PASS_BLOCKS", 2048);
     w.id_blocks = (int)num("SYMMICP_ID_BLOCKS", 2048);
     w.acc_blocks = (int)num("SYMMICP_ACC_BLOCKS", 512);
diff --git a/icp-symm_amd/csrc/engine_internal.h b/icp-symm_amd/csrc/engine_internal.h
--- a/icp-symm_amd/csrc/engine_internal.h
+++ b/icp-symm_amd/csrc/engine_internal.h
@@ -82,6 +82,8 @@
     double hood_frac = 0.8;
     bool no_hood = false, no_cert = false, walk_full_grid = false, host_loop = false, no_loop_stragglers = false, force_comm = false;
     int budget_walk = -1, optimistic = -1, compact = -1;
+    int cert_pass = 1;
+    int cert_head = 4;
     int pass_blocks = 2048, id_blocks = 2048, acc_blocks = 512, fused_blocks = 512, compact_blocks = 1280;
     int feature_nn_splits = 0, feature_nn_queries = 0;
     PassTuning tune;
@@ -216,6 +218,8 @@
     uint32_t *ticket = nullptr;
     long long last_list_len = -1;
     long long last_uncertified = -1;
+    long long last_scans = -1;
+    bool cert_pass_failed = false;
     static constexpr int kRing = 65;
     LoopState *d_loop = nullptr, *h_loop = nullptr, *h_loop_dev = nullptr;
     LoopRecord *h_ring = nullptr, *h_ring_dev = nullptr;
diff --git a/icp-symm_amd/csrc/engine_loop.cpp b/icp-symm_amd/csrc/engine_loop.cpp
--- a/icp-symm_amd/csrc/engine_loop.cpp
+++ b/icp-symm_amd/csrc/engine_loop.cpp
@@ -195,7 +195,12 @@
     if (c->cfg.corr == SYMMICP_CORR_TREE && c->h_sums[kNSum - 1] >= kListDropped)
         return fail(c, SYMMICP_ERR_HIP, "a work-list shard overflowed: appends were dropped (internal capacity error)");
     long long list_len = (c->cfg.corr == SYMMICP_CORR_TREE) ? (long long)c->h_sums[kNSum - 1] : -1;
-    c->last_uncertified = (c->cfg.corr == SYMMICP_CORR_TREE && !first) ? (long long)c->h_sums[kNSum - 2] : -1;
+    c->last_uncertified = c->last_scans = -1;
+    if (c->cfg.corr == SYMMICP_CORR_TREE && !first) {
+        const double sr = c->h_sums[kNSum - 2], sc = std::floor(sr / kScanUnit);
+        c->last_uncertified = (long long)(sr - sc * kScanUnit);
+        c->last_scans = (long long)sc;
+    }
     if (optimistic && list_len > 0) {
         c->st.kernel_launches[7]++;
         launch_pass_tree_split(a, c->ix, c->wl, blocks, list_len <= 50000 ? 8192u : 0u, 2, 0, c->sw.tune, c->stream, nullptr);
@@ -259,8 +264,13 @@
     const bool no_stage = c->sw.no_loop_stragglers;
     bool stragglers = tree && c->last_list_len > 0 && !no_stage;
     lc.list_limit = kLoopListLimit;
+    const int cert_mode = (tree && c->cert && !c->sw.no_cert && !c->cert_pass_failed) ? c->sw.cert_pass : 0;
+    if (cert_mode == 2) stragglers = false;
+    bool cert_chunk = false;
+    uint8_t pass_kernel[symmicp_ctx::kRing] = {};
     if (lc.max_iters > c->cfg.max_iters) lc.max_iters = c->cfg.max_iters;
     const int it0 = c->iters;
+    const long long list0 = c->last_list_len, scans0 = c->last_scans;
     LoopState ls{};
     std::memcpy(ls.X, c->X, sizeof(ls.X));
     for (int k = 0; k < 12; k++) ls.Xapply.m[k] = c->X[k];
@@ -295,8 +305,18 @@
     const bool timed_run = c->timing == 1 || c->timing == 3;
     const int ev_stride = c->timing == 3 ? kEvSampleStride : 1;
     if (timed_run && c->ev_used + want > symmicp_ctx::kEvRing) flush_events(c);
-    const bool unstoppable = lc.fixed_iters && !(lc.eps_rotation > 0.f && lc.eps_translation > 0.f) && !stragglers;
-    int enq = 0, chunk = unstoppable ? want : 4, n_stage = 0;
+    const bool one_piece = lc.fixed_iters && !(lc.eps_rotation > 0.f && lc.eps_translation > 0.f);
+    int enq = 0, n_stage = 0;
+    constexpr int kCertHeads = 3;
+    int heads_left = (one_piece && !stragglers && cert_mode == 1 && c->sw.cert_head > 0) ? kCertHeads : 0;
+    auto plan_chunk = [&](long long list_len, long long scans, int left, int prev) -> int {
+        cert_chunk = cert_mode == 2 || (cert_mode == 1 && !stragglers && list_len == 0 && scans == 0);
+        if (stragglers) return 4;
+        if (!one_piece) return prev ? 2 * prev : 4;
+        if (!cert_chunk && heads_left > 0 && left > c->sw.cert_head) { heads_left--; return c->sw.cert_head; }
+        return left;
+    };
+    int chunk = plan_chunk(c->last_list_len, c->last_scans, want, 0);
     bool first_chunk = true;
     while (enq < want) {
         const int nq = (want - enq < chunk) ? want - enq : chunk;
@@ -317,7 +337,9 @@
                 hipEventRecord(ev[0], c->stream);
             }
             if (tree) {
-                launch_pass_fused(a, c->ix, c->wl, fused_blocks, c->stream);
+                pass_kernel[(it_before + 1 + p) % symmicp_ctx::kRing] = cert_chunk ? 1 : 0;
+                if (cert_chunk) launch_pass_certified(a, c->ix, c->wl, fused_blocks, c->stream);
+                else launch_pass_fused(a, c->ix, c->wl, fused_blocks, c->stream);
                 if (stragglers) launch_loop_stragglers(a, c->ix, c->wl, kListBlocks, c->sw.tune, c->stream);
             }
             else launch_pass_identity(a, c->tgt, blocks, vec4, c->stream);
@@ -364,9 +386,9 @@
             stragglers = false;
             for (int k = it_before + 1; k <= c->h_loop->iters; k++) stragglers = stragglers || c->h_ring[k % symmicp_ctx::kRing].list_len > 0;
         }
-        if (stragglers) chunk = 4;
-        else if (lc.fixed_iters && !(lc.eps_rotation > 0.f && lc.eps_translation > 0.f)) chunk = want;
-        else chunk *= 2;
+        if (cert_mode == 2) stragglers = false;
+        const LoopRecord &lr = c->h_ring[c->h_loop->iters % symmicp_ctx::kRing];
+        chunk = plan_chunk(lr.list_len, lr.reserved, want - enq, chunk);
     }
     const LoopState &hl = *c->h_loop;
     const int it1 = hl.iters;
@@ -388,6 +410,8 @@
             std::memcpy(e.X, r.X, sizeof(e.X));
             e.rcond = r.rcond; e.iter = k; e.status = r.status; e.solved = r.solved; e.list_len = k == it0 ? 0 : r.list_len;
             e.reason = hl.reason; e.batch = c->loop_log_batches;
+            e.reserved = k == it0 ? 0 : pass_kernel[k % symmicp_ctx::kRing];
+            if (k == it1 && hl.reason == LOOP_REDO_PASS && pass_kernel[(it1 + 1) % symmicp_ctx::kRing]) e.reserved |= 0x100;
             if (!e.solved) { std::memset(e.increment, 0, sizeof(e.increment)); std::memset(e.X, 0, sizeof(e.X)); e.rcond = 0.f; e.status = -1; }
             c->loop_log.push_back(e);
         }
@@ -397,17 +421,23 @@
     c->last_list_len = tree ? (it1 > it0 ? (long long)c->h_ring[it1 % symmicp_ctx::kRing].list_len : c->last_list_len) : -1;
     *n_done = it1 - it0;
     *small_step = hl.reason == LOOP_DONE && hl.small_step != 0;
-    if (tree && it1 > it0) c->last_uncertified = c->h_ring[it1 % symmicp_ctx::kRing].pad;
+    if (tree && it1 > it0) { c->last_uncertified = c->h_ring[it1 % symmicp_ctx::kRing].pad; c->last_scans = c->h_ring[it1 % symmicp_ctx::kRing].reserved; }
+    int n_cert = 0;
+    for (int k = it0 + 1; k <= it1; k++) n_cert += pass_kernel[k % symmicp_ctx::kRing];
+    if (hl.reason == LOOP_REDO_PASS && pass_kernel[(it1 + 1) % symmicp_ctx::kRing]) c->cert_pass_failed = true;
     if (c->sw.debug_host && it1 - it0 >= 2) {
         const double *q = c->h_ring[(it1 - 1) % symmicp_ctx::kRing].sums;
         if (q[37] != 0.0) std::fprintf(stderr, "[symmicp host] k_reduce_solve stamps of pass %d: load + reduce %.2f us (loop state there after %.2f us), bookkeeping + solve %.2f us, publish %.2f us\n", it1 - 1, std::floor(q[37]) * 0.01, (q[37] - std::floor(q[37])) * 1e4 * 0.01, q[38] * 0.01, q[39] * 0.01);
     }
     if (c->sw.debug_host && tree) {
-        std::fprintf(stderr, "[symmicp host] batch: work list / searched pairs after each device pass:");
-        for (int k = it0 + 1; k <= it1; k++) std::fprintf(stderr, " %d/%d", c->h_ring[k % symmicp_ctx::kRing].list_len, c->h_ring[k % symmicp_ctx::kRing].pad);
+        std::fprintf(stderr, "[symmicp host] batch: work list / searched pairs / scanned pairs after each device pass (c: certified-only kernel):");
+        for (int k = it0 + 1; k <= it1; k++) {
+            const LoopRecord &r = c->h_ring[k % symmicp_ctx::kRing];
+            std::fprintf(stderr, " %d/%d/%d%s", r.list_len, r.pad, r.reserved, pass_kernel[k % symmicp_ctx::kRing] ? "c" : "");
+        }
         std::fprintf(stderr, "\n");
     }
-    if (c->sw.debug_host) std::fprintf(stderr, "[symmicp host] batch: %d of %d passes on the device (%d enqueued), reason %d, %d with the straggler stage, list after %lld\n", it1 - it0, want, enq, hl.reason, n_stage, (long long)c->last_list_len);
+    if (c->sw.debug_host) std::fprintf(stderr, "[symmicp host] batch: %d of %d passes on the device (%d enqueued), reason %d, %d with the straggler stage, %d certified-only%s, list after %lld (host pass before: list %lld, scanned %lld)\n", it1 - it0, want, enq, hl.reason, n_stage, n_cert, c->cert_pass_failed ? " (now off: a pass came back incomplete)" : "", (long long)c->last_list_len, list0, scans0);
     if (hl.reason == LOOP_SLOW) c->host_passes_since_bailout = 1;
     if (hl.reason == LOOP_REDO_PASS || hl.reason == LOOP_HOST_SOLVE) {
         c->host_passes_since_bailout = 0;
@@ -550,6 +580,7 @@
     std::memset(out, 0, sizeof(*out));
     if (c->external_exchange) { out->status = SYMMICP_ERR_STATE; return fail(c, SYMMICP_ERR_STATE, "symmicp_align is not available with external exchange: drive begin/set_sums/step"); }
     const double t0 = now_s();
+    c->cert_pass_failed = false;
     c->loop_log.clear();
     c->loop_log_batches = 0;
     symmicp_iter_result it;
diff --git a/icp-symm_amd/csrc/kernels_pass.hip b/icp-symm_amd/csrc/kernels_pass.hip
--- a/icp-symm_amd/csrc/kernels_pass.hip
+++ b/icp-symm_amd/csrc/kernels_pass.hip
@@ -179,11 +179,10 @@
     return __uint_as_float(hood ? ((u - 1u) | 1u) : (u & ~1u));
 }
 
-__device__ __forceinline__ bool hood_test(const PassArgs &a, const TargetIndex &ix, uint32_t i, float px, float py, float pz, float m2,
-                                          int32_t pos_a, float d2a, int32_t rowa, int32_t &pos_w, float &d2w)
-{
-    const uint4 w0 = a.certk[2 * (size_t)i], w1 = a.certk[2 * (size_t)i + 1];
-    const float T = a.hoodr[i].x;
+__device__ __forceinline__ bool hood_test_set(const PassArgs &a, const TargetIndex &ix, uint32_t i, float px, float py, float pz, float m2,
+                                              int32_t pos_a, float d2a, int32_t rowa, const uint4 &w0, const uint4 &w1, const float T,
+                                              int32_t &pos_w, float &d2w)
+{
     const uint32_t cand[kHoodSlots] = {w0.x, w0.y, w0.z, w0.w, w1.x, w1.y, w1.z, w1.w};
     float4 q[kHoodSlots];
 #pragma unroll
@@ -217,6 +216,14 @@
         a.cert[i].w = cert_word(0.0f, true);
     }
     return true;
+}
+
+__device__ __forceinline__ bool hood_test(const PassArgs &a, const TargetIndex &ix, uint32_t i, float px, float py, float pz, float m2,
+                                          int32_t pos_a, float d2a, int32_t rowa, int32_t &pos_w, float &d2w)
+{
+    const uint4 w0 = a.certk[2 * (size_t)i], w1 = a.certk[2 * (size_t)i + 1];
+    const float T = a.hoodr[i].x;
+    return hood_test_set(a, ix, i, px, py, pz, m2, pos_a, d2a, rowa, w0, w1, T, pos_w, d2w);
 }
 
 template <bool HOOD>
@@ -604,11 +611,11 @@
     const bool need_n = reads_src_normals<OBJ>(false, a.min_ndot);
     constexpr int kList = ACC ? kFusedList : kFusedList / 2;
     __shared__ uint32_t s_list[kList];
-    __shared__ uint32_t s_cnt, s_total;
+    __shared__ uint32_t s_cnt, s_total, s_hood;
     __shared__ unsigned long long s_col[ACC ? 10 : 1];
     AccT<W> acc;
     if (ACC) acc_zero(acc);
-    if (threadIdx.x == 0) { s_cnt = 0; s_total = 0; }
+    if (threadIdx.x == 0) { s_cnt = 0; s_total = 0; s_hood = 0; }
     if (ACC && threadIdx.x == 0) {
         s_col[0] = (unsigned long long)a.in.x; s_col[1] = (unsigned long long)a.in.y; s_col[2] = (unsigned long long)a.in.z;
         s_col[3] = (unsigned long long)a.in.nx; s_col[4] = (unsigned long long)a.in.ny; s_col[5] = (unsigned long long)a.in.nz;
@@ -670,6 +677,7 @@
                     if (need_n) { nx = a.in.nx[i]; ny = a.in.ny[i]; nz = a.in.nz[i]; }
                     pair_step<OBJ>(acc, h, nx, ny, nz, px, py, pz, qw, nqw, d2w);
                     s_list[e] = 0xFFFFFFFFu;
+                    atomicAdd(&s_hood, 1u);
                 }
             }
             __syncthreads();
@@ -773,6 +781,7 @@
     __syncthreads();
     flush();
     if (threadIdx.x == 0 && s_total) atomicAdd(wl.work.counts + shard * kShardStride + 1, s_total);
+    if (ACC && threadIdx.x == 0 && s_hood) atomicAdd(wl.work.counts + shard * kShardStride + 3, s_hood);
 #ifdef RS_STAMPS2
     const unsigned long long fs2 = __builtin_amdgcn_s_memrealtime();
 #endif
@@ -783,6 +792,102 @@
         dbg[0] = (double)(fs1 - fs0); dbg[1] = (double)(fs2 - fs1); dbg[2] = (double)(__builtin_amdgcn_s_memrealtime() - fs2);
     }
 #endif
+}
+
+constexpr uint32_t kCertList = kPassThreads;
+
+template <bool W, int OBJ>
+__global__ __launch_bounds__(kPassThreads) void k_pass_certified(PassArgs a, TargetIndex ix, WorkLists wl)
+{
+    const bool need_n = reads_src_normals<OBJ>(false, a.min_ndot);
+    __shared__ uint32_t s_list[kCertList];
+    __shared__ uint32_t s_cnt, s_bad;
+    AccT<W> acc; acc_zero(acc);
+    if (threadIdx.x == 0) { s_cnt = 0; s_bad = 0; }
+    __syncthreads();
+    int stop = 0;
+    HotParams h = hot_params(a);
+    if (a.loop) {
+        stop = a.loop->stop;
+        const float4 *xp = reinterpret_cast<const float4 *>(&in_vgpr(a.loop)->Xapply);
+        const float4 r0 = xp[0], r1 = xp[1], r2 = xp[2];
+        h.X.m[0] = r0.x; h.X.m[1] = r0.y; h.X.m[2] = r0.z; h.X.m[3] = r0.w;
+        h.X.m[4] = r1.x; h.X.m[5] = r1.y; h.X.m[6] = r1.z; h.X.m[7] = r1.w;
+        h.X.m[8] = r2.x; h.X.m[9] = r2.y; h.X.m[10] = r2.z; h.X.m[11] = r2.w;
+        h.X.nrm_w = reinterpret_cast<const float *>(xp)[12];
+    }
+    const Affine &X = h.X;
+    const uint32_t tiles = (a.n + kPassThreads - 1) / kPassThreads;
+    const uint32_t tiles_p = ((tiles + 7u) / 8u) * 8u;
+    for (uint32_t t = blockIdx.x; t < tiles_p; t += gridDim.x) {
+        const uint32_t i = xcd_remap(t, tiles_p) * kPassThreads + threadIdx.x;
+        const bool live = i < a.n;
+        float x = 0.f, y = 0.f, z = 0.f, nx = 0.f, ny = 0.f, nz = 0.f;
+        float4 q = make_float4(0.f, 0.f, 0.f, 0.f), nq = make_float4(0.f, 0.f, 0.f, 2.0f), ce = make_float4(0.f, 0.f, 0.f, 0.f);
+        if (live) {
+            x = a.in.x[i]; y = a.in.y[i]; z = a.in.z[i];
+            if (need_n) { nx = a.in.nx[i]; ny = a.in.ny[i]; nz = a.in.nz[i]; }
+            q = a.pairrec[2 * (size_t)i]; nq = a.pairrec[2 * (size_t)i + 1];
+            ce = a.cert[i];
+        }
+        if (stop) return;
+        if (!live) continue;
+        const float px = xf_row(X.m + 0, x, y, z, 1.0f), py = xf_row(X.m + 4, x, y, z, 1.0f), pz = xf_row(X.m + 8, x, y, z, 1.0f);
+        bool certified = false;
+        float d2 = 0.0f;
+        if (nq.w == 0.0f) {
+            d2 = dist2(px, py, pz, q.x, q.y, q.z);
+            const float m2 = dist2(px, py, pz, ce.x, ce.y, ce.z);
+            certified = (__builtin_amdgcn_sqrtf(d2) + __builtin_amdgcn_sqrtf(m2)) * 1.000002f < ce.w;
+        }
+        if (certified) pair_step<OBJ>(acc, h, nx, ny, nz, px, py, pz, q, nq, d2);
+        else {
+            const uint32_t e = atomicAdd(&s_cnt, 1u);
+            if (e < kCertList) s_list[e] = i;
+        }
+    }
+    __syncthreads();
+    const uint32_t cnt = s_cnt;
+    if (cnt) {
+        const uint32_t m = min(cnt, kCertList);
+        if (threadIdx.x < m) {
+            const uint32_t i = s_list[threadIdx.x];
+            bool settled = false;
+            const float4 ce = a.cert[i];
+            const float4 q = a.pairrec[2 * (size_t)i], nq = a.pairrec[2 * (size_t)i + 1];
+            const int32_t pk = a.pos_prev[i];
+            const float x = a.in.x[i], y = a.in.y[i], z = a.in.z[i];
+            float nx = 0.0f, ny = 0.0f, nz = 0.0f;
+            if (need_n) { nx = a.in.nx[i]; ny = a.in.ny[i]; nz = a.in.nz[i]; }
+            uint4 w0 = make_uint4(kHoodNone, kHoodNone, kHoodNone, kHoodNone), w1 = w0;
+            float T = 0.0f;
+            if (a.certk) { w0 = a.certk[2 * (size_t)i]; w1 = a.certk[2 * (size_t)i + 1]; T = a.hoodr[i].x; }
+            if (a.certk && (__float_as_uint(ce.w) & 1u)) {
+                if (nq.w == 0.0f && (uint32_t)pk < ix.n) {
+                    const float px = xf_row(X.m + 0, x, y, z, 1.0f), py = xf_row(X.m + 4, x, y, z, 1.0f), pz = xf_row(X.m + 8, x, y, z, 1.0f);
+                    const float d2 = dist2(px, py, pz, q.x, q.y, q.z);
+                    int32_t pw; float d2w;
+                    if (d2 <= __int_as_float(0x7f800000) &&
+                        hood_test_set(a, ix, i, px, py, pz, dist2(px, py, pz, ce.x, ce.y, ce.z), pk, d2, __float_as_int(q.w), w0, w1, T, pw, d2w)) {
+                        float4 qw = q, nqw = nq;
+                        if (pw != pk) { qw = ix.tn[2 * (size_t)pw]; nqw = ix.tn[2 * (size_t)pw + 1]; }
+                        pair_step<OBJ>(acc, h, nx, ny, nz, px, py, pz, qw, nqw, d2w);
+                        settled = true;
+                    }
+                }
+            }
+            if (!settled) atomicAdd(&s_bad, 1u);
+        }
+        __syncthreads();
+        if (threadIdx.x == 0) {
+            const uint32_t shard = blockIdx.x & (kShards - 1);
+            const uint32_t bad = s_bad + (cnt - m);
+            if (bad) atomicAdd(wl.work.counts + shard * kShardStride, bad);
+            atomicAdd(wl.work.counts + shard * kShardStride + 1, cnt);
+            atomicAdd(wl.work.counts + shard * kShardStride + 3, cnt - bad);
+        }
+    }
+    acc_block_reduce_store(acc, a.partials, blockIdx.x);
 }
 
 
@@ -1023,17 +1128,18 @@
     acc_block_reduce_store(acc, a.partials, a.partial_col0 + blockIdx.x);
 }
 
-__device__ __forceinline__ void read_list_words(const uint32_t *cnt, int t, uint32_t &len, uint32_t &searched, uint32_t &dropped)
-{
-    uint32_t v = cnt[t * kShardStride], u = cnt[t * kShardStride + 1];
+__device__ __forceinline__ void read_list_words(const uint32_t *cnt, int t, uint32_t &len, uint32_t &searched, uint32_t &dropped, uint32_t &scans)
+{
+    uint32_t v = cnt[t * kShardStride], u = cnt[t * kShardStride + 1], sc = cnt[t * kShardStride + 3];
     uint32_t d = (t < 2) ? cnt[t * kShards * kShardStride + 2] : 0u;
 #pragma unroll
     for (int off = 32; off > 0; off >>= 1) {
         v += (uint32_t)__shfl_xor((int)v, off, 64);
         u += (uint32_t)__shfl_xor((int)u, off, 64);
         d += (uint32_t)__shfl_xor((int)d, off, 64);
-    }
-    len = v; searched = u; dropped = d;
+        sc += (uint32_t)__shfl_xor((int)sc, off, 64);
+    }
+    len = v; searched = u; dropped = d; scans = u > sc ? u - sc : 0u;
 }
 
 __global__ __launch_bounds__(256) void k_final_reduce(const double *__restrict__ partials, int nblocks,
@@ -1063,18 +1169,18 @@
         if (counters_to_clear) {
             __shared__ uint32_t s_len;
             if (t < 64) {
-                uint32_t len, searched, dropped;
-                read_list_words(counters_to_clear, t, len, searched, dropped);
+                uint32_t len, searched, dropped, scans;
+                read_list_words(counters_to_clear, t, len, searched, dropped, scans);
                 if (t == 0) {
                     s_len = len;
-                    const double lenw = (double)len + (dropped ? kListDropped : 0.0);
-                    out_dev[kNSum - 1] = lenw; out_dev[kNSum - 2] = (double)searched;
-                    if (out_mapped) { out_mapped[kNSum - 1] = lenw; out_mapped[kNSum - 2] = (double)searched; }
+                    const double lenw = (double)len + (dropped ? kListDropped : 0.0), srw = (double)searched + (double)scans * kScanUnit;
+                    out_dev[kNSum - 1] = lenw; out_dev[kNSum - 2] = srw;
+                    if (out_mapped) { out_mapped[kNSum - 1] = lenw; out_mapped[kNSum - 2] = srw; }
                 }
             }
             __syncthreads();
             if (t < 2) counters_to_clear[t * kShards * kShardStride + 2] = 0;
-            if (t < kShards) counters_to_clear[t * kShardStride + 1] = 0;
+            if (t < kShards) { counters_to_clear[t * kShardStride + 1] = 0; counters_to_clear[t * kShardStride + 3] = 0; }
             if (!(keep_nonempty && s_len > 0u))
                 for (int c = t; c < 2 * kShards; c += 256) counters_to_clear[c * kShardStride] = 0;
         }
@@ -1093,17 +1199,18 @@
                                                        LoopConfig cfg, LoopRecord *ring, int ring_len, uint32_t *counters_to_clear)
 {
     __shared__ double s_sum[kNSum];
-    __shared__ uint32_t s_len, s_unc;
+    __shared__ uint32_t s_len, s_unc, s_scan;
     const int t = threadIdx.x, lane = t & 63, wave = t >> 6;
 #ifdef RS_STAMPS
     const unsigned long long ts0 = __builtin_amdgcn_s_memrealtime();
 #endif
     const LoopState ls = *loop;
-    uint32_t cw0 = 0, cw1 = 0, cw2 = 0;
+    uint32_t cw0 = 0, cw1 = 0, cw2 = 0, cw3 = 0;
     const bool want_counters = !solve_only && REDUCE && counters_to_clear && t < 64;
     if (want_counters) {
         cw0 = counters_to_clear[t * kShardStride]; cw1 = counters_to_clear[t * kShardStride + 1];
         cw2 = (t < 2) ? counters_to_clear[t * kShards * kShardStride + 2] : 0u;
+        cw3 = counters_to_clear[t * kShardStride + 3];
     }
     __shared__ double s_part[8][kNSum];
     double accw = 0.0;
@@ -1124,7 +1231,7 @@
 #ifdef RS_STAMPS
     const unsigned long long tsA = __builtin_amdgcn_s_memrealtime();
 #endif
-    if (t == 0) { s_len = 0; s_unc = 0; }
+    if (t == 0) { s_len = 0; s_unc = 0; s_scan = 0; }
     if (!solve_only && REDUCE) {
         if (lane < kNSum) s_part[wave][lane] = accw;
         __syncthreads();
@@ -1144,14 +1251,16 @@
                     cw0 += (uint32_t)__shfl_xor((int)cw0, off, 64);
                     cw1 += (uint32_t)__shfl_xor((int)cw1, off, 64);
                     cw2 += (uint32_t)__shfl_xor((int)cw2, off, 64);
+                    cw3 += (uint32_t)__shfl_xor((int)cw3, off, 64);
                 }
-                if (t == 0) { s_len = cw2 ? 0xFFFFFFFFu : cw0; s_unc = cw1; }
-            }
-            if (t < kShards) counters_to_clear[t * kShardStride + 1] = 0;
+                if (t == 0) { s_len = cw2 ? 0xFFFFFFFFu : cw0; s_unc = cw1; s_scan = cw1 > cw3 ? cw1 - cw3 : 0u; }
+            }
+            if (t < kShards) { counters_to_clear[t * kShardStride + 1] = 0; counters_to_clear[t * kShardStride + 3] = 0; }
             for (int c = t; c < 2 * kShards; c += 512) counters_to_clear[c * kShardStride] = 0;
         } else if (t == 0) {
             s_len = (s_sum[kNSum - 1] >= kListDropped) ? 0xFFFFFFFFu : (uint32_t)s_sum[kNSum - 1];
-            s_unc = (uint32_t)s_sum[kNSum - 2];
+            const double sr = s_sum[kNSum - 2], sc = floor(sr / kScanUnit);
+            s_unc = (uint32_t)(sr - sc * kScanUnit); s_scan = (uint32_t)sc;
         }
     }
     __syncthreads();
@@ -1160,7 +1269,7 @@
 #endif
     int it = ls.iters;
     if (!solve_only) {
-        const uint32_t len = s_len, unc = s_unc;
+        const uint32_t len = s_len, unc = s_unc, scans = s_scan;
         if (cfg.tree && len > 0u && (!cfg.walk_in_loop || len == 0xFFFFFFFFu)) { if (t == 0) { loop->stop = 1; loop->reason = LOOP_REDO_PASS; } return; }
         it += 1;
         LoopRecord &r = ring[it % ring_len];
@@ -1169,7 +1278,7 @@
             loop->iters = it;
             r.solved = 0;
             r.pad = (int32_t)unc;
-            r.list_len = (int32_t)len; r.reserved = 0;
+            r.list_len = (int32_t)len; r.reserved = (int32_t)scans;
         }
         if (cfg.tree && (unc > cfg.uncertified_limit || (cfg.walk_in_loop && len > cfg.list_limit))) { if (t == 0) { loop->stop = 1; loop->reason = LOOP_SLOW; } return; }
     }
@@ -1453,6 +1562,11 @@
     with_instantiation(a, [&](auto W, auto OBJ) { hipLaunchKernelGGL((k_pass_fused<true, W, OBJ>), dim3(blocks), dim3(kPassThreads), 0, s, a, ix, wl); });
 }
 
+void launch_pass_certified(const PassArgs &a, const TargetIndex &ix, const WorkLists &wl, int blocks, hipStream_t s)
+{
+    with_instantiation(a, [&](auto W, auto OBJ) { hipLaunchKernelGGL((k_pass_certified<W, OBJ>), dim3(blocks), dim3(kPassThreads), 0, s, a, ix, wl); });
+}
+
 void launch_loop_stragglers(const PassArgs &a, const TargetIndex &ix, const WorkLists &wl, int list_blocks, const PassTuning &tune, hipStream_t s)
 {
     const uint32_t wave_mode_max = tune.wave_mode_max;
diff --git a/icp-symm_amd/csrc/symmicp_internal.h b/icp-symm_amd/csrc/symmicp_internal.h
--- a/icp-symm_amd/csrc/symmicp_internal.h
+++ b/icp-symm_amd/csrc/symmicp_internal.h
@@ -10,6 +10,7 @@
 constexpr int kNAcc = 37;
 constexpr int kNAccW = 38;
 constexpr double kListDropped = 4294967296.0;
+constexpr double kScanUnit = 4294967296.0;
 constexpr int kLeaf = 8;
 constexpr int kFan = 8;
 constexpr int kMaxTreeLevels = 12;
@@ -216,6 +217,7 @@
 void launch_final_reduce(const double *partials, int blocks, double *out_dev, double *out_host_mapped, uint32_t *ticket,
                          unsigned long long seq, uint32_t *counters_to_clear, int keep_nonempty, hipStream_t s);
 void launch_pass_fused(const PassArgs &a, const TargetIndex &ix, const WorkLists &wl, int blocks, hipStream_t s);
+void launch_pass_certified(const PassArgs &a, const TargetIndex &ix, const WorkLists &wl, int blocks, hipStream_t s);
 void launch_loop_stragglers(const PassArgs &a, const TargetIndex &ix, const WorkLists &wl, int list_blocks, const PassTuning &tune, hipStream_t s);
 void launch_reduce_solve(const double *partials, int blocks, double *out_dev, int mode, LoopState *loop, LoopConfig cfg, LoopRecord *ring, int ring_len,
                          uint32_t *counters_to_clear, hipStream_t s);
diff --git a/icp-symm_amd/py/symmicp/__init__.py b/icp-symm_amd/py/symmicp/__init__.py
--- a/icp-symm_amd/py/symmicp/__init__.py
+++ b/icp-symm_amd/py/symmicp/__init__.py
@@ -1226,7 +1226,8 @@
         for e in buf[:n.value]:
             out.append(dict(sums=np.array(e.sums[:], np.float64), increment=np.array(e.increment[:], np.float32).reshape(4, 4),
                             X=np.array(e.X[:], np.float32).reshape(4, 4), rcond=e.rcond, iter=e.iter, status=e.status, solved=e.solved,
-                            list_len=e.list_len, reason=e.reason, batch=e.batch))
+                            list_len=e.list_len, reason=e.reason, batch=e.batch,
+                            kernel=e.reserved & 0xff, redo_certified=bool(e.reserved & 0x100)))
         return out
 
 
```

Result: faster. 33180 (median of 6 runs) (+8.2%).
